# fnothaft/adam

Hardware: AMD Instinct MI355X
Metric: BQSR bases/sec (observe+apply) at 1/2/4/8 MI355X; % HBM roofline (higher is better)
Workload: dtype u8 in, int64 counts, f64 recalibration; 1 GPU; cfg2: synthetic 10M x 100 bp reads, 1 read group, no known sites (per GPU); reads_per_gpu=10000000, bases_per_gpu=1000000000, reads_total=10000000, read_groups=1, known_sites=0, parallelism=dp1: read shards per GPU, RCCL int64 table all-reduce

## Files before the change

adam_amd/csrc/bqsr_capi.cpp:

```cpp
#include <hip/hip_runtime.h>

#include <algorithm>
#include <array>
#include <atomic>
#include <chrono>
#include <cmath>
#include <cstdio>
#include <cstdlib>
#include <cstring>
#include <dlfcn.h>
#include <memory>
#include <mutex>
#include <new>
#include <string>
#include <thread>
#include <vector>

#include <rocprim/rocprim.hpp>

#include "bqsr_internal.h"

using namespace bqsr;

#include "bqsr_kernels.hip"
// ... 129 lines not shown
  return K + 2 * K * cells;
}
TableGeom geom(const bqsr_dims& d) {
  TableGeom g;
  g.K = 60 * (d.n_rg - 1) + 128;
  g.L = d.max_len;
  g.C = 2 * d.max_len + 1;
  g.cells = g.C + kCtxSlots;
  return g;
}

constexpr size_t kLdsMax = 163840;
size_t observe_lds(int qw, int wcells, bool table) {
  return (table ? (size_t)kCtxTabBytes : 0) + (size_t)qw * wcells * 8 + (size_t)qw * 4 + kQBins * 4 +
         (size_t)kMkWords * 4;
}
int64_t piece_bytes(int qw, int cw) { return ((int64_t)qw * cw * kCtxSlots + 15) & ~(int64_t)15; }
size_t apply_lds(int qw, int cw) { return 16 + (size_t)kMkWords * 4 + kCtxTabBytes + (size_t)piece_bytes(qw, cw); }
int lean_orow(int nc, int cw) {
  int o = nc * (cw + kCtxCells);
  while ((o & 3) != 2) ++o;
  return o;
}
size_t lean_lds(int qw, int orow, int wcells) { return ((size_t)qw * (orow + wcells) + qw + kQBins + 1) * 4; }
constexpr int kLeanCopiesMax = 4;
int observe_rows(int wcells, bool table) {
  int qw = kQBins;
  while (qw > 1 && observe_lds(qw, wcells, table) > kLdsMax) --qw;
  return qw;
}
constexpr bool align_slots() { return true; }
int fronts(int n_base, int n_cu, int64_t n_reads, int forced) {
  if (forced == 0) return 0;
  int f = forced;
  if (f < 0) {
    if (n_base > 4 * n_cu) return 0;
    f = (int)std::min<int64_t>((8 * n_cu + n_base - 1) / n_base, n_reads / (8192 * (int64_t)n_base));
    if ((int64_t)std::max(f, 1) * n_base < n_cu) return 0;
    f = std::max(f, 1);
  }
  while (f > 1 && (int64_t)f * n_base > 4096) --f;
  return f;
}
int apply_rows(int cw) {
  int qw = kQBins;
  while (qw > 1 && apply_lds(qw, cw) > kLdsMax) --qw;
  return qw;
}

}


struct bqsr_context {
  int device = 0;
  int n_cu = 256;
  double* d_pow10 = nullptr;
  double* d_thr = nullptr;
  double* d_qbt = nullptr;
  int16_t* d_qbq = nullptr;
  std::mutex stage_mu;
  uint8_t* stage[2] = {nullptr, nullptr};
  hipEvent_t stage_ev[2] = {nullptr, nullptr};
  int tune_order = -1;
  int tune_fronts = -1;
  int tune_keymajor = 0;
  int tune_bgzf = 1;
  int tune_flagstat_grid = 0;
  int tune_pileup_grid = 0;
  std::mutex flagstat_mu;
  unsigned long long* d_flagstat = nullptr;
};

namespace {
constexpr size_t kStageChunk = 64ull << 20;
bqsr_status stage_ring(bqsr_context* ctx) {
  for (int i = 0; i < 2; ++i) {
    if (!ctx->stage[i]) HIP_TRY(hipHostMalloc((void**)&ctx->stage[i], kStageChunk, hipHostMallocDefault));
    if (!ctx->stage_ev[i]) HIP_TRY(hipEventCreateWithFlags(&ctx->stage_ev[i], hipEventDisableTiming));
  }
  return BQSR_OK;
}
bqsr_status upload_staged(bqsr_context* ctx, void* dst, const void* src, size_t n, hipStream_t s) {
  hipPointerAttribute_t attr{};
  const bool pinned = hipPointerGetAttributes(&attr, src) == hipSuccess && attr.type == hipMemoryTypeHost;
  (void)hipGetLastError();
  if (pinned || n < 2 * kStageChunk) {
    HIP_TRY(hipMemcpyAsync(dst, src, n, hipMemcpyHostToDevice, s));
    HIP_TRY(hipStreamSynchronize(s));
    return BQSR_OK;
  }
  std::lock_guard<std::mutex> lock(ctx->stage_mu);
  bqsr_status st = stage_ring(ctx);
  if (st != BQSR_OK) return st;
  const int nth = (int)std::max(1u, std::min(8u, std::thread::hardware_concurrency()));
  const uint8_t* p = (const uint8_t*)src;
  uint8_t* d = (uint8_t*)dst;
  int k = 0;
  for (size_t off = 0; off < n; off += kStageChunk, k ^= 1) {
    const size_t len = std::min(kStageChunk, n - off);
    HIP_TRY(hipEventSynchronize(ctx->stage_ev[k]));
    std::vector<std::thread> th;
    for (int t = 0; t < nth; ++t)
      th.emplace_back([&, t] {
        const size_t a = len * (size_t)t / (size_t)nth, b = len * (size_t)(t + 1) / (size_t)nth;
        memcpy(ctx->stage[k] + a, p + off + a, b - a);
      });
    for (auto& x : th) x.join();
    HIP_TRY(hipMemcpyAsync(d + off, ctx->stage[k], len, hipMemcpyHostToDevice, s));
    HIP_TRY(hipEventRecord(ctx->stage_ev[k], s));
  }
  HIP_TRY(hipStreamSynchronize(s));
  return BQSR_OK;
}
}

struct bqsr_sites {
  bqsr_context* ctx = nullptr;
  std::vector<std::string> names;
  int64_t* pos = nullptr;
  uint64_t* off = nullptr;
  uint32_t* bucket = nullptr;
  uint64_t* bucket_off = nullptr;
  int64_t* bucket_base = nullptr;
  uint64_t* bm = nullptr;
  uint64_t* bm_off = nullptr;
  int64_t* bm_base = nullptr;
  int32_t n = 0;
  int32_t shift = 8;
  SitesDev dev() const { return SitesDev{pos, off, bucket, bucket_off, bucket_base, bm, bm_off, bm_base, n, shift}; }
};

struct bqsr_batch {
  bqsr_context* ctx = nullptr;
  bool owned = false;
  ReadsDev rd{};
  bqsr_dims dims{1, 1};
  int64_t n_slots = 0;
  int64_t n_bases = 0;
  int32_t q_lo = 0, rg_lo = 0;
  bool have_qhist = false;
  int64_t qhist[kQBins] = {0};
  int64_t qhigh = 0;
  std::vector<void*> allocs;
  std::vector<size_t> staged_cnt;
  const bqsr_staged* staged_src = nullptr;
  uint8_t* d_bases2 = nullptr;
  uint64_t* d_bexc = nullptr;
  uint64_t* d_qcodes = nullptr;
  uint8_t* d_qbase = nullptr;
  uint64_t* d_qexc = nullptr;
  ReadInfo* d_info = nullptr;
  uint64_t* d_sbits = nullptr;
  uint32_t* d_work = nullptr;
  uint64_t* d_bnd = nullptr;
  int64_t sbits_words = 0;
  bool err_fresh = false;
  bool prepped = false;
  const bqsr_sites* prep_sites = nullptr;
  uint32_t* d_hq = nullptr;
  uint32_t* d_qmask = nullptr;
  bool hq_valid = false;
  FoldParams fold{};
  uint32_t* d_part = nullptr;
  size_t part_words = 0;
  uint8_t* d_chars = nullptr;
  const bqsr_lut* chars_lut = nullptr;
  uint64_t* d_off64 = nullptr;
  int64_t off64_n = -1;
  size_t chars_bytes = 0;
  unsigned long long* d_err = nullptr;
  double* d_em = nullptr;
  int32_t n_blocks = 0;
  bool bucketed = false;
  int32_t n_keys = 1;
  int32_t n_base = 1;
  int32_t fronts = 0;
  uint32_t* d_perm = nullptr;
  int64_t* d_key_off = nullptr;
  uint32_t* d_key_cnt = nullptr;
  uint32_t* d_cursor = nullptr;
  uint8_t *k_qual = nullptr, *k_bases = nullptr;
  uint64_t* d_kslot = nullptr;
  uint64_t* d_kspan = nullptr;
  void* d_ktemp = nullptr;
  size_t ktemp_bytes = 0;
  bool km_ready = false;
  double km_alloc_ms = -1.0, km_build_ms = -1.0;
  bool perm_static = false;
  OrderDev order() const {
    return bucketed ? OrderDev{d_perm, d_key_off, n_keys, fronts > 0 ? n_base : 0, km_ready ? d_kslot : nullptr}
                    : OrderDev{nullptr, nullptr, 1};
  }
  ReadsDev pass_rd() const {
    ReadsDev r = rd;
    if (bucketed && km_ready) {
      r.qual = k_qual;
      r.bases = k_bases;
    }
    return r;
  }
  int32_t pass_blocks() const { return bucketed && fronts > 0 ? n_keys : n_blocks; }
  uint64_t* h_status = nullptr;
  hipStream_t side = nullptr;
  hipEvent_t ev_obs = nullptr, ev_fold = nullptr;
  bool obs_pending = false;
  ~bqsr_batch() {
    if (side) (void)hipStreamDestroy(side);
    for (hipEvent_t e : {ev_obs, ev_fold})
      if (e) (void)hipEventDestroy(e);
    if (d_part) (void)hipFree(d_part);
    if (d_off64) (void)hipFree(d_off64);
    if (d_chars) (void)hipFree(d_chars);
    if (h_status) (void)hipHostFree(h_status);
    for (void* p : allocs) (void)hipFree(p);
  }
};

struct bqsr_table {
  bqsr_context* ctx = nullptr;
  bqsr_dims dims{1, 1};
  int64_t* words = nullptr;
  bool owned = false;
  ~bqsr_table() {
    if (owned && words) (void)hipFree(words);
  }
  TableGeom g() const { return geom(dims); }
  int64_t* touched() const { return words; }
  int64_t* obs() const { return words + g().K; }
  int64_t* mm() const { return words + g().K + (int64_t)g().K * g().cells; }
};

struct bqsr_lut {
  bqsr_context* ctx = nullptr;
  bqsr_dims dims{1, 1};
  int32_t n_groups = 0;
  std::vector<void*> allocs;
  int64_t *qk_obs = nullptr, *qk_mm = nullptr, *grp_obs = nullptr, *grp_mm = nullptr;
  uint8_t *grp_ok = nullptr, *key_ok = nullptr, *rq_ok = nullptr;
  double *a2 = nullptr, *s1 = nullptr, *d2 = nullptr;
  FinalOut* d_out = nullptr;
  FinalOut out{};
  bool out_pending = false;
  bool host_ready = false;
  std::vector<int64_t> h_words, h_qk_obs, h_qk_mm, h_grp_obs, h_grp_mm;
  std::vector<uint8_t> h_grp_ok;
  const bqsr_table* src = nullptr;
  ~bqsr_lut() {
    for (void* p : allocs) (void)hipFree(p);
  }
};

namespace {
template <class T>
bqsr_status dalloc(std::vector<void*>& v, T** p, size_t n) {
  void* q = nullptr;
  HIP_TRY(hipMalloc(&q, std::max<size_t>(n, 1) * sizeof(T)));
  v.push_back(q);
  *p = (T*)q;
  return BQSR_OK;
}
}


extern "C" {

int bqsr_abi_version(void) { return BQSR_ABI_VERSION; }
const char* bqsr_last_error(void) { return g_err.c_str(); }
int64_t bqsr_last_error_read(void) { return g_err_read; }
const char* bqsr_status_name(bqsr_status s) {
  if ((int)s < 0 || (int)s > 16) return "UNKNOWN";
  return kStatusNames[(int)s];
}

bqsr_status bqsr_context_tune(bqsr_context* ctx, int knob, int64_t value) {
  if (!ctx) return fail(BQSR_ERR_INVALID_ARG, "bqsr_context_tune: null context");
  switch (knob) {
    case BQSR_TUNE_ORDER:
      if (value < -1 || value > 1) break;
      ctx->tune_order = (int)value;
      return BQSR_OK;
    case BQSR_TUNE_FRONTS:
      if (value < -1 || value > 4096) break;
      ctx->tune_fronts = (int)value;
      return BQSR_OK;
    case BQSR_TUNE_KEYMAJOR:
      if (value < 0 || value > 1) break;
      ctx->tune_keymajor = (int)value;
      return BQSR_OK;
    case BQSR_TUNE_FUSED_PREP:
      if (value != 0) break;
      return BQSR_OK;
    case BQSR_TUNE_BGZF:
      if (value < 0 || value > 1) break;
      ctx->tune_bgzf = (int)value;
      return BQSR_OK;
    case BQSR_TUNE_FLAGSTAT_GRID:
      if (value < 0 || value > (1 << 20)) break;
      ctx->tune_flagstat_grid = (int)value;
      return BQSR_OK;
    case BQSR_TUNE_PILEUP_GRID:
      if (value < 0 || value > (1 << 20)) break;
      ctx->tune_pileup_grid = (int)value;
      return BQSR_OK;
    default:
      return fail(BQSR_ERR_INVALID_ARG, "bqsr_context_tune: unknown knob");
  }
  return fail(BQSR_ERR_INVALID_ARG, "bqsr_context_tune: value out of range");
}

bqsr_status bqsr_context_create(int device, bqsr_context** out) {
  if (!out) return fail(BQSR_ERR_INVALID_ARG, "null out");
  HIP_TRY(hipSetDevice(device));
  hipDeviceProp_t prop;
  HIP_TRY(hipGetDeviceProperties(&prop, device));
  bqsr_context* c = new bqsr_context;
  c->device = device;
  c->n_cu = prop.multiProcessorCount;
  hipError_t e = hipMalloc(&c->d_pow10, 256 * sizeof(double));
  if (e == hipSuccess) e = hipMalloc(&c->d_thr, kThrN * sizeof(double));
  if (e == hipSuccess) e = hipMemcpy(c->d_pow10, pow10tab().v, 256 * sizeof(double), hipMemcpyHostToDevice);
  if (e == hipSuccess) e = hipMemcpy(c->d_thr, thresholds().thr.data(), kThrN * sizeof(double), hipMemcpyHostToDevice);
  if (e == hipSuccess) e = hipMalloc(&c->d_qbt, kQbN * sizeof(double));
  if (e == hipSuccess) e = hipMalloc(&c->d_qbq, kQbN * sizeof(int16_t));
  if (e == hipSuccess) e = hipMemcpy(c->d_qbt, buckets().thr.data(), kQbN * sizeof(double), hipMemcpyHostToDevice);
  if (e == hipSuccess) e = hipMemcpy(c->d_qbq, buckets().q.data(), kQbN * sizeof(int16_t), hipMemcpyHostToDevice);
  for (const void* f : {(const void*)bqsr_apply_kernel, (const void*)bqsr_observe_chunks,
                        (const void*)bqsr_observe_lean<true>})
    if (e == hipSuccess) e = hipFuncSetAttribute(f, hipFuncAttributeMaxDynamicSharedMemorySize, (int)kLdsMax);
  if (e == hipSuccess)
    e = hipFuncSetAttribute((const void*)bqsr_fold_hist, hipFuncAttributeMaxDynamicSharedMemorySize, (int)fold_hist_lds());
  if (e == hipSuccess)
    e = hipFuncSetAttribute((const void*)bqsr_fold_chain, hipFuncAttributeMaxDynamicSharedMemorySize,
                            (int)chain_lds(kMaxFoldBlocks));
  if (e != hipSuccess) {
    bqsr_context_destroy(c);
    return fail(BQSR_ERR_DEVICE, std::string("context: ") + hipGetErrorString(e));
  }
  *out = c;
  return ok();
}

void bqsr_context_destroy(bqsr_context* c) {
  if (!c) return;
  if (c->d_pow10) (void)hipFree(c->d_pow10);
  if (c->d_thr) (void)hipFree(c->d_thr);
  if (c->d_qbt) (void)hipFree(c->d_qbt);
  if (c->d_qbq) (void)hipFree(c->d_qbq);
  if (c->d_flagstat) (void)hipFree(c->d_flagstat);
  for (int i = 0; i < 2; ++i) {
    if (c->stage[i]) (void)hipHostFree(c->stage[i]);
    if (c->stage_ev[i]) (void)hipEventDestroy(c->stage_ev[i]);
  }
  delete c;
}


bqsr_status bqsr_sites_create(bqsr_context* ctx, const char* const* contigs, const int64_t* const* pos,
                              const uint64_t* n, int32_t n_contigs, bqsr_sites** out) {
  if (!ctx || !out || n_contigs < 0 || (n_contigs > 0 && (!contigs || !pos || !n)))
    return fail(BQSR_ERR_INVALID_ARG, "bqsr_sites_create: bad arguments");
  HIP_TRY(hipSetDevice(ctx->device));
  bqsr_sites* s = new bqsr_sites;
  s->ctx = ctx;
  s->n = n_contigs;
  std::vector<int64_t> all;
  std::vector<uint64_t> off(1, 0);
  std::vector<uint32_t> bucket;
  std::vector<uint64_t> boff(1, 0);
  std::vector<int64_t> bbase;
  std::vector<uint64_t> bm, bmoff(1, 0);
  std::vector<int64_t> bmbase;
  for (int32_t c = 0; c < n_contigs; ++c) {
    s->names.emplace_back(contigs[c] ? contigs[c] : "");
    std::vector<int64_t> v(pos[c], pos[c] + n[c]);
    std::sort(v.begin(), v.end());
    v.erase(std::unique(v.begin(), v.end()), v.end());
    const int64_t base = v.empty() ? 0 : v.front();
    const int64_t nb = v.empty() ? 0 : ((v.back() - base) >> s->shift) + 1;
    size_t j = 0;
    for (int64_t b = 0; b < nb; ++b) {
      const int64_t lo = base + (b << s->shift);
      while (j < v.size() && v[j] < lo) ++j;
      bucket.push_back((uint32_t)j);
    }
    bbase.push_back(base);
    boff.push_back(bucket.size());
    const int64_t b0 = v.empty() ? 0 : (int64_t)((uint64_t)base & ~(uint64_t)63);
    const int64_t nw = v.empty() ? 0 : ((v.back() - b0) >> 6) + 1;
    const bool dense = nw > 0 && nw <= 64 * (int64_t)v.size() + 64 && nw <= (int64_t(1) << 28);
    if (dense) {
      const size_t w0 = bm.size();
      bm.resize(w0 + (size_t)nw, 0ull);
      for (const int64_t p : v) bm[w0 + (size_t)((p - b0) >> 6)] |= 1ull << ((p - b0) & 63);
    }
    bmbase.push_back(dense ? b0 : 0);
    bmoff.push_back(bm.size());
    all.insert(all.end(), v.begin(), v.end());
    off.push_back(all.size());
  }
  std::vector<void*> keep;
  auto up = [&](auto** dst, const auto& src) -> hipError_t {
    using T = typename std::remove_reference<decltype(src[0])>::type;
    hipError_t e = hipMalloc((void**)dst, std::max<size_t>(src.size(), 1) * sizeof(T));
    if (e != hipSuccess) return e;
    if (!src.empty()) e = hipMemcpy(*dst, src.data(), src.size() * sizeof(T), hipMemcpyHostToDevice);
    return e;
  };
  hipError_t e = up(&s->pos, all);
  if (e == hipSuccess) e = up(&s->off, off);
  if (e == hipSuccess) e = up(&s->bucket, bucket);
  if (e == hipSuccess) e = up(&s->bucket_off, boff);
  if (e == hipSuccess) e = up(&s->bucket_base, bbase);
  if (e == hipSuccess) e = up(&s->bm, bm);
  if (e == hipSuccess) e = up(&s->bm_off, bmoff);
  if (e == hipSuccess) e = up(&s->bm_base, bmbase);
  if (e != hipSuccess) {
    bqsr_sites_destroy(s);
    return fail(BQSR_ERR_DEVICE, std::string("sites upload: ") + hipGetErrorString(e));
  }
  *out = s;
  return ok();
}

void bqsr_sites_destroy(bqsr_sites* s) {
  if (!s) return;
  for (void* p : {(void*)s->pos, (void*)s->off, (void*)s->bucket, (void*)s->bucket_off, (void*)s->bucket_base,
                  (void*)s->bm, (void*)s->bm_off, (void*)s->bm_base})
    if (p) (void)hipFree(p);
  delete s;
}


namespace {

inline uint8_t code_of(uint8_t c) {
  switch (c) {
    case 'A': return kCodeA;
    case 'C': return kCodeC;
    case 'G': return kCodeG;
    case 'T': return kCodeT;
    case 'N': return kCodeN;
    default: return kCodeOther;
  }
}

Window window_rows(const bqsr_batch* b, int max_rows);

bqsr_status finish_batch(bqsr_batch* b, int64_t max_slot_len) {
  if (max_slot_len > kMaxReadLen)
    return fail(BQSR_ERR_UNSUPPORTED, "reads longer than " + std::to_string(kMaxReadLen) + " bases are not supported");
  const int64_t n = b->rd.n_reads;
  b->rd.reads_per_tile = (int32_t)std::max<int64_t>(1, std::min<int64_t>(kMaxTileReads, kTileSlots / std::max<int64_t>(1, max_slot_len)));
  b->rd.n_tiles = (n + b->rd.reads_per_tile - 1) / b->rd.reads_per_tile;
  b->n_blocks = std::min(b->ctx->n_cu, kMaxFoldBlocks);
  bqsr_status st;
  if ((st = dalloc(b->allocs, &b->d_hq, (size_t)b->n_blocks * kQBins)) != BQSR_OK) return st;
  if ((st = dalloc(b->allocs, &b->d_qmask, 4)) != BQSR_OK) return st;
  {
    FoldParams& F = b->fold;
    const size_t nt = (size_t)std::max<int64_t>(1, b->rd.n_tiles), nbk = (size_t)b->n_blocks;
    F.stream_cap = std::max<int64_t>(1 << 20, std::min<int64_t>(16 << 20, b->rd.n_slots));
    if ((st = dalloc(b->allocs, &F.blk, nbk)) != BQSR_OK || (st = dalloc(b->allocs, &F.cand_list, nbk)) != BQSR_OK ||
        (st = dalloc(b->allocs, &F.n_cand, 1)) != BQSR_OK || (st = dalloc(b->allocs, &F.delta, 1)) != BQSR_OK ||
        (st = dalloc(b->allocs, &F.rtile, nt)) != BQSR_OK || (st = dalloc(b->allocs, &F.ntile, nt)) != BQSR_OK ||
        (st = dalloc(b->allocs, &F.dtile, nt * kSegBinades)) != BQSR_OK ||
        (st = dalloc(b->allocs, &F.seg, nbk * kFoldMaxSegs)) != BQSR_OK ||
        (st = dalloc(b->allocs, &F.seg_base, nbk)) != BQSR_OK || (st = dalloc(b->allocs, &F.nseg, nbk)) != BQSR_OK ||
        (st = dalloc(b->allocs, &F.seg_used, 1)) != BQSR_OK ||
        (st = dalloc(b->allocs, &F.streams, (size_t)F.stream_cap + 64)) != BQSR_OK ||
        (st = dalloc(b->allocs, &F.csum, (size_t)F.stream_cap / 64 * 2 + 2)) != BQSR_OK ||
        (st = dalloc(b->allocs, &F.stream_used, 1)) != BQSR_OK)
      return st;
  }
  if ((st = dalloc(b->allocs, &b->d_err, kErrWords)) != BQSR_OK) return st;
  if ((st = dalloc(b->allocs, &b->d_info, (size_t)std::max<int64_t>(1, n))) != BQSR_OK) return st;
  b->sbits_words = (b->rd.n_slots / 32 + 5) & ~(int64_t)1;
  if ((st = dalloc(b->allocs, &b->d_sbits, (size_t)b->sbits_words)) != BQSR_OK) return st;
  if ((st = dalloc(b->allocs, &b->d_em, 2)) != BQSR_OK) return st;
  if ((st = dalloc(b->allocs, &b->d_bnd, (size_t)2 * (size_t)(n / 64 + kPrepChunk / 64 + 1))) != BQSR_OK) return st;
  if ((st = dalloc(b->allocs, &b->d_work,
                   (size_t)(n + kPrepChunk) + (size_t)std::max<int64_t>(n / kPrepChunk + 1, kMaxFoldBlocks))) != BQSR_OK)
    return st;
  if (b->ctx->tune_order >= 0) {
    b->bucketed = b->ctx->tune_order == 1;
  } else {
    b->bucketed = b->dims.n_rg > 1;
    if (!b->bucketed && b->have_qhist) {
      const int cw = geom(b->dims).C;
      const Window w = window_rows(b, apply_rows(cw));
      int64_t in = 0, all = 0;
      for (int q = 0; q < kQBins; ++q) {
        all += b->qhist[q];
        if (q >= w.q_lo && q < w.q_lo + w.qw) in += b->qhist[q];
      }
      b->bucketed = (double)(all - in) > 1e-3 * (double)all;
    }
  }
  if (b->bucketed) {
    b->n_base = 2 * std::max<int32_t>(1, b->dims.n_rg);
    b->fronts = fronts(b->n_base, b->ctx->n_cu, n, b->ctx->tune_fronts);
    b->n_keys = b->n_base * std::max(1, b->fronts);
    if ((st = dalloc(b->allocs, &b->d_perm, (size_t)std::max<int64_t>(1, n))) != BQSR_OK) return st;
    if ((st = dalloc(b->allocs, &b->d_key_off, (size_t)b->n_keys + 1)) != BQSR_OK) return st;
    if ((st = dalloc(b->allocs, &b->d_key_cnt, (size_t)b->n_keys)) != BQSR_OK) return st;
    if ((st = dalloc(b->allocs, &b->d_cursor, (size_t)b->n_keys)) != BQSR_OK) return st;
  }
  return BQSR_OK;
}

bool layout_wanted(const bqsr_batch* b) { return b->bucketed && b->rd.slots_aligned && b->rd.n_reads > 0; }
bool key_major_wanted(const bqsr_batch* b) { return layout_wanted(b) && b->ctx->tune_keymajor; }
bqsr_status key_major_alloc(bqsr_batch* b) {
  if (b->k_qual) return BQSR_OK;
  const int64_t n = b->rd.n_reads;
  bqsr_status st;
  size_t tb = 0;
  HIP_TRY(rocprim::exclusive_scan(nullptr, tb, (const uint64_t*)nullptr, (uint64_t*)nullptr, (uint64_t)0, (size_t)n + 1,
                                  rocprim::plus<uint64_t>(), (hipStream_t)0));
  b->ktemp_bytes = std::max<size_t>(tb, 1);
  if ((st = dalloc(b->allocs, &b->d_kslot, (size_t)(n + 1))) != BQSR_OK ||
      (st = dalloc(b->allocs, &b->d_kspan, (size_t)(n + 1))) != BQSR_OK ||
      (st = dalloc(b->allocs, (uint8_t**)&b->d_ktemp, b->ktemp_bytes)) != BQSR_OK ||
      (st = dalloc(b->allocs, &b->k_qual, (size_t)b->rd.n_slots + kColumnPad)) != BQSR_OK ||
      (st = dalloc(b->allocs, &b->k_bases, (size_t)b->rd.n_slots / 2 + 1 + kColumnPad)) != BQSR_OK)
    return st;
  return BQSR_OK;
}
void launch_key_sort(bqsr_batch* b, uint64_t* span, hipStream_t s) {
  const int64_t n = b->rd.n_reads;
  const int n_cu = b->ctx->n_cu;
  (void)hipMemsetAsync(b->d_key_cnt, 0, (size_t)b->n_keys * 4, s);
  const unsigned cb = (unsigned)std::min<int64_t>((n + 255) / 256, (int64_t)n_cu * 4);
  hipLaunchKernelGGL(bqsr_key_count, dim3(cb), dim3(256), 0, s, (const ReadMeta*)b->rd.meta, n, b->n_keys, b->n_base,
                     std::max(1, b->fronts), b->d_key_cnt);
  hipLaunchKernelGGL(bqsr_key_scan, dim3(1), dim3(1024), 0, s, (const uint32_t*)b->d_key_cnt, b->n_keys, b->d_key_off,
                     b->d_cursor);
  const unsigned sb = (unsigned)std::min<int64_t>((n + 4095) / 4096, (int64_t)n_cu * 8);
  hipLaunchKernelGGL(bqsr_key_scatter, dim3(sb), dim3(256), 0, s, (const ReadMeta*)b->rd.meta, n, b->n_keys, b->n_base,
                     std::max(1, b->fronts), b->d_cursor, b->d_perm, span);
}
bqsr_status layout_build(bqsr_batch* b, hipStream_t s) {
  if (!layout_wanted(b)) return BQSR_OK;
  const int64_t n = b->rd.n_reads;
  bqsr_context* ctx = b->ctx;
  const bool km = key_major_wanted(b);
  b->km_ready = false;
  const auto t0 = std::chrono::steady_clock::now();
  bqsr_status st = km ? key_major_alloc(b) : BQSR_OK;
  if (st != BQSR_OK) return st;
  const auto t1 = std::chrono::steady_clock::now();
  if (km) HIP_TRY(hipMemsetAsync(b->d_kspan + n, 0, 8, s));
  launch_key_sort(b, km ? b->d_kspan : nullptr, s);
  HIP_TRY(hipGetLastError());
  if (km) {
    size_t tb = b->ktemp_bytes;
    HIP_TRY(rocprim::exclusive_scan(b->d_ktemp, tb, b->d_kspan, b->d_kslot, (uint64_t)0, (size_t)n + 1,
                                    rocprim::plus<uint64_t>(), s));
    HIP_TRY(hipMemsetAsync(b->k_qual + b->rd.n_slots, 0, kColumnPad, s));
    HIP_TRY(hipMemsetAsync(b->k_bases + b->rd.n_slots / 2, 0, 1 + kColumnPad, s));
    const unsigned gw = (unsigned)std::min<int64_t>((n + 16 * kKmPer - 1) / (16 * kKmPer), (int64_t)ctx->n_cu * 64 / kKmPer);
    hipLaunchKernelGGL(bqsr_km_gather, dim3(gw), dim3(256), 0, s, b->rd, (const uint32_t*)b->d_perm,
                       (const uint64_t*)b->d_kslot, b->k_qual, b->k_bases);
    HIP_TRY(hipGetLastError());
  }
  HIP_TRY(hipStreamSynchronize(s));
  const auto t2 = std::chrono::steady_clock::now();
  b->km_alloc_ms = std::chrono::duration<double, std::milli>(t1 - t0).count();
  b->km_build_ms = std::chrono::duration<double, std::milli>(t2 - t1).count();
  b->km_ready = km;
  b->perm_static = true;
  return BQSR_OK;
}

struct Packed {
  std::vector<ReadMeta> meta;
  std::vector<ReadAlign> align;
  std::vector<uint8_t> qual, bases, md;
  std::vector<uint32_t> cigar;
  int64_t n_slots = 0, n_bases = 0, max_slot = 0;
  int32_t n_rg = 1, max_len = 1;
  int64_t qhist[256] = {0};
  std::vector<int64_t> rghist;
};

bqsr_status pack(const bqsr_records* R, Packed& P) {
  const int64_t n = R->n_reads;
  P.meta.resize((size_t)n);
  P.align.resize((size_t)n);
  uint64_t slot = 0, md_tot = 0, cig_tot = 0;
  for (int64_t r = 0; r < n; ++r) {
    const uint32_t f = R->flags[r];
    const uint64_t lq = (f & BQSR_F_HAS_QUAL) ? R->qual_offset[r + 1] - R->qual_offset[r] : 0;
    const uint64_t ls = (f & BQSR_F_HAS_SEQ) ? R->seq_offset[r + 1] - R->seq_offset[r] : 0;
    const uint64_t nmd = (f & BQSR_F_HAS_MD) ? R->md_offset[r + 1] - R->md_offset[r] : 0;
    const uint64_t ncig = (f & BQSR_F_HAS_CIGAR) ? R->cigar_offset[r + 1] - R->cigar_offset[r] : 0;
    if (lq > 65535 || ls > 65535 || nmd > 65535 || ncig > 65535)
      return fail(BQSR_ERR_UNSUPPORTED, "read field longer than 65535", r);
    if ((f & BQSR_F_HAS_RG) && (R->rg_id[r] < 0 || R->rg_id[r] > 65535))
      return fail(BQSR_ERR_UNSUPPORTED, "recordGroupId outside [0, 65535]", r);
    ReadMeta& m = P.meta[(size_t)r];
    m.slot = slot;
    m.lq = (uint16_t)lq;
    m.ls = (uint16_t)ls;
    m.flags = (uint16_t)(f & 0x7FFF);
    m.rg = (f & BQSR_F_HAS_RG) ? (uint16_t)R->rg_id[r] : 0;
    ReadAlign& a = P.align[(size_t)r];
    a.start = R->start[r];
    a.cigar_off = (uint32_t)cig_tot;
    a.md_off = (uint32_t)md_tot;
    a.contig = R->contig_id[r];
    a.n_cigar = (uint16_t)ncig;
    a.md_len = (uint16_t)nmd;
    const uint64_t sl = align_slots() ? slot_span(lq, ls) : std::max(lq, ls);
    slot += sl;
    P.max_slot = std::max<int64_t>(P.max_slot, (int64_t)sl);
    md_tot += nmd;
    cig_tot += ncig;
    P.n_bases += (int64_t)(R->seq_offset[r + 1] - R->seq_offset[r]);
    if (f & BQSR_F_HAS_RG) P.n_rg = std::max<int32_t>(P.n_rg, R->rg_id[r] + 1);
    P.max_len = std::max<int32_t>(P.max_len, (int32_t)ls);
  }
  if (md_tot > 0xFFFFFFFFull || cig_tot > 0xFFFFFFFFull)
    return fail(BQSR_ERR_UNSUPPORTED, "partition MD / CIGAR columns exceed 4 GiB");
  P.n_slots = (int64_t)slot;
  P.qual.assign((size_t)slot + kColumnPad, 0);
  P.bases.assign((size_t)slot / 2 + 1 + kColumnPad, 0);
  P.md.resize(md_tot + kColumnPad);
  P.cigar.resize(cig_tot + kColumnPad / 4);
  P.rghist.assign((size_t)P.n_rg, 0);
  const int nth = (int)std::max<int64_t>(1, std::min<int64_t>(16, n / 65536));
  std::vector<std::thread> th;
  std::vector<std::array<int64_t, 256>> qh((size_t)nth);
// ... 350 lines not shown
  }
  *out = b;
  return ok();
}

void bqsr_batch_destroy(bqsr_batch* b) { delete b; }
int64_t bqsr_batch_reads(const bqsr_batch* b) { return b ? b->rd.n_reads : -1; }
int64_t bqsr_batch_bases(const bqsr_batch* b) { return b ? b->n_bases : -1; }
int64_t bqsr_batch_slots(const bqsr_batch* b) { return b ? b->n_slots : -1; }
bqsr_dims bqsr_batch_dims(const bqsr_batch* b) { return b ? b->dims : bqsr_dims{0, 0}; }

bqsr_status bqsr_batch_relayout(bqsr_batch* b, void* stream, double* ms) {
  if (!b) return fail(BQSR_ERR_INVALID_ARG, "bqsr_batch_relayout: null batch");
  hipStream_t s = (hipStream_t)stream;
  HIP_TRY(hipStreamSynchronize(s));
  const auto t0 = std::chrono::steady_clock::now();
  const bool has = b->perm_static;
  if (has) {
    b->perm_static = false;
    bqsr_status st = layout_build(b, s);
    if (st != BQSR_OK) return st;
  }
  HIP_TRY(hipStreamSynchronize(s));
  if (ms) *ms = has ? std::chrono::duration<double, std::milli>(std::chrono::steady_clock::now() - t0).count() : -1.0;
  return ok();
}

bqsr_status bqsr_batch_layout_times(const bqsr_batch* b, double* alloc_ms, double* build_ms) {
  if (!b) return fail(BQSR_ERR_INVALID_ARG, "bqsr_batch_layout_times: null batch");
  if (alloc_ms) *alloc_ms = b->km_alloc_ms;
  if (build_ms) *build_ms = b->km_build_ms;
  return ok();
}

bqsr_status bqsr_batch_set_window(bqsr_batch* b, int32_t q_lo, int32_t rg_lo) {
  if (!b || q_lo < 0 || q_lo >= kQBins || rg_lo < 0) return fail(BQSR_ERR_INVALID_ARG, "bad window");
  b->q_lo = q_lo;
  b->rg_lo = rg_lo;
  b->have_qhist = false;
  return ok();
}
int32_t bqsr_batch_reads_per_tile(const bqsr_batch* b) { return b ? b->rd.reads_per_tile : -1; }


int64_t bqsr_table_words(bqsr_dims d) { return (d.n_rg < 1 || d.max_len < 1) ? -1 : table_words(d); }

bqsr_status bqsr_table_create(bqsr_context* ctx, bqsr_dims d, void* device_words, bqsr_table** out) {
  if (!ctx || !out || d.n_rg < 1 || d.max_len < 1 || d.max_len > 65535)
    return fail(BQSR_ERR_INVALID_ARG, "bqsr_table_create: bad arguments");
  HIP_TRY(hipSetDevice(ctx->device));
  bqsr_table* t = new bqsr_table;
  t->ctx = ctx;
  t->dims = d;
  const size_t bytes = (size_t)table_words(d) * 8;
  if (device_words) {
    t->words = (int64_t*)device_words;
  } else {
    hipError_t e = hipMalloc((void**)&t->words, bytes);
    if (e != hipSuccess) {
      delete t;
      return fail(BQSR_ERR_DEVICE, hipGetErrorString(e));
    }
    t->owned = true;
  }
  hipError_t e = hipMemset(t->words, 0, bytes);
  if (e != hipSuccess) {
    delete t;
    return fail(BQSR_ERR_DEVICE, hipGetErrorString(e));
  }
  *out = t;
  return ok();
}
void bqsr_table_destroy(bqsr_table* t) { delete t; }
bqsr_dims bqsr_table_dims(const bqsr_table* t) { return t ? t->dims : bqsr_dims{0, 0}; }
void* bqsr_table_device_ptr(bqsr_table* t) { return t ? t->words : nullptr; }

bqsr_status bqsr_table_download(const bqsr_table* t, int64_t* host) {
  if (!t || !host) return fail(BQSR_ERR_INVALID_ARG, "null");
  HIP_TRY(hipSetDevice(t->ctx->device));
  HIP_TRY(hipMemcpy(host, t->words, (size_t)table_words(t->dims) * 8, hipMemcpyDeviceToHost));
  return ok();
}
bqsr_status bqsr_table_upload(bqsr_table* t, const int64_t* host) {
  if (!t || !host) return fail(BQSR_ERR_INVALID_ARG, "null");
  HIP_TRY(hipSetDevice(t->ctx->device));
  HIP_TRY(hipMemcpy(t->words, host, (size_t)table_words(t->dims) * 8, hipMemcpyHostToDevice));
  return ok();
}

bqsr_status bqsr_table_merge(bqsr_table* acc, const bqsr_table* part, double* acc_em, double part_em) {
  if (!acc || !part || !acc_em) return fail(BQSR_ERR_INVALID_ARG, "null");
  if (acc->dims.n_rg != part->dims.n_rg || acc->dims.max_len != part->dims.max_len)
    return fail(BQSR_ERR_INVALID_ARG, "table dims differ");
  HIP_TRY(hipSetDevice(acc->ctx->device));
  const int64_t n = table_words(acc->dims);
  hipLaunchKernelGGL(bqsr_table_add, dim3((unsigned)std::min<int64_t>(4096, (n + 255) / 256)), dim3(256), 0,
                     hipStreamPerThread, acc->words, part->words, n);
  HIP_TRY(hipGetLastError());
  HIP_TRY(hipStreamSynchronize(hipStreamPerThread));
  *acc_em = *acc_em + part_em;
  return ok();
}


namespace {
Window window_rows(const bqsr_batch* b, int max_rows) {
  Window w{max_rows, std::min(b->q_lo, kQBins - 1), b->rg_lo};
  if (!b->have_qhist) {
    w.qw = std::min(w.qw, kQBins - w.q_lo);
    return w;
  }
  int lo = 0, hi = kQBins - 1;
  while (lo < kQBins - 1 && b->qhist[lo] == 0) ++lo;
  while (hi > lo && b->qhist[hi] == 0) --hi;
  if (hi - lo + 1 <= max_rows) {
    w.q_lo = lo;
    w.qw = hi - lo + 1;
  } else {
    w.q_lo = best_q_lo(b->qhist, max_rows);
  }
  w.qw = std::min(w.qw, kQBins - w.q_lo);
  return w;
}
int window_cw(const bqsr_batch* b, const TableGeom& g) { return b->bucketed ? g.L : g.C; }
int qual_span(const bqsr_batch* b) {
  if (!b->have_qhist) return kQBins;
  int lo = 0, hi = kQBins - 1;
  while (lo < kQBins - 1 && b->qhist[lo] == 0) ++lo;
  while (hi > lo && b->qhist[hi] == 0) --hi;
  return hi - lo + 1;
}
int lane_shift(const bqsr_batch* b) {
  const int c = (b->dims.max_len + kSuper - 1) / kSuper;
  int s = 0;
  while ((1 << s) < c && s < 6) ++s;
  return s;
}
bqsr_status check_dims(const bqsr_batch* b, const bqsr_table* t) {
  if (b->dims.n_rg > t->dims.n_rg || b->dims.max_len > t->dims.max_len)
    return fail(BQSR_ERR_INVALID_ARG, "table dims smaller than the batch's (n_rg / max_len)");
  return BQSR_OK;
}
}

namespace {
bqsr_status launch_prep(bqsr_context* ctx, bqsr_batch* b, const bqsr_sites* sites, hipStream_t s) {
  if (!b->err_fresh) HIP_TRY(hipMemsetAsync(b->d_err + kErrAppPrep, 0xFF, 8, s));
  b->err_fresh = false;
  b->hq_valid = false;
  if (b->rd.n_reads > 0) {
    PrepParams P{};
    P.rd = b->rd;
    if (sites) P.sites = sites->dev();
    P.store_words = b->dims.max_len <= 128 && P.sites.n_contigs > 0;
    P.bnd = b->d_bnd;
    P.info = b->d_info;
    P.sbits = b->d_sbits;
    P.err = b->d_err;
    P.work = b->d_work;
    P.n_work = b->d_work + b->rd.n_reads + kPrepChunk;
    const int64_t blocks = (b->rd.n_reads + kPrepChunk - 1) / kPrepChunk;
    if (P.store_words) {
      hipLaunchKernelGGL(bqsr_prep_kernel<true>, dim3((unsigned)blocks), dim3(kPrepThreads), 0, s, P);
      hipLaunchKernelGGL(bqsr_prep_complex, dim3((unsigned)blocks), dim3(kComplexThreads), 0, s, P);
    } else {
      hipLaunchKernelGGL(bqsr_prep_kernel<false>, dim3((unsigned)blocks), dim3(kPrepThreads), 0, s, P);
    }
    HIP_TRY(hipGetLastError());
    if (b->bucketed && !b->perm_static) {
      launch_key_sort(b, nullptr, s);
      HIP_TRY(hipGetLastError());
    }
  }
  b->prepped = true;
  b->prep_sites = sites;
  return BQSR_OK;
}
}

bqsr_status bqsr_observe_stage(bqsr_context* ctx, bqsr_batch* b, const bqsr_sites* sites, bqsr_table* t,
                               int32_t stages, void* stream) {
  if (!ctx || !b || !t) return fail(BQSR_ERR_INVALID_ARG, "null");
  bqsr_status st = check_dims(b, t);
  if (st != BQSR_OK) return st;
  HIP_TRY(hipSetDevice(ctx->device));
  hipStream_t s = S(stream);
  if (stages & BQSR_STAGE_RESET) HIP_TRY(hipMemsetAsync(b->d_err + kErrObs, 0xFF, 8, s));
  if (stages & BQSR_STAGE_PREP) {
    if ((st = launch_prep(ctx, b, sites, s)) != BQSR_OK) return st;
  }
  if (b->rd.n_reads == 0) {
    if (stages & BQSR_STAGE_FOLD) HIP_TRY(hipMemsetAsync(b->d_em, 0, 8, s));
    return ok();
  }
  if ((stages & BQSR_STAGE_KERNEL) && (!b->prepped || b->prep_sites != sites))
    return fail(BQSR_ERR_INVALID_ARG, "observe kernel before the prep stage (or with other known sites)");
  if (stages & BQSR_STAGE_KERNEL) {
    ObserveParams P{};
    P.rd = b->pass_rd();
    P.ord = b->order();
    P.info = b->d_info;
    P.sbits = b->d_sbits;
    P.g = geom(t->dims);
    const bool lean = !b->bucketed;
    P.wcells = window_cw(b, P.g) + (lean ? kCtxCells : kCtxSlots);
    while ((P.wcells & 3) != 2) ++P.wcells;
    if (lean) {
      const int cw = window_cw(b, P.g), span = qual_span(b);
      int best_rows = 0;
      for (int nc = kLeanCopiesMax; nc >= 1 && best_rows < span; --nc) {
        const int orow = lean_orow(nc, cw);
        int qw = kQBins;
        while (qw > 1 && lean_lds(qw, orow, P.wcells) > kLdsMax) --qw;
        if (qw > best_rows) {
          best_rows = qw;
          P.nc = nc;
          P.orow = orow;
        }
      }
      P.w = window_rows(b, best_rows);
      P.rows_all = b->have_qhist && b->qhigh == 0;
      for (int q = 0; q < kQBins && P.rows_all; ++q)
        if (b->qhist[q] && (q < P.w.q_lo || q >= P.w.q_lo + P.w.qw)) P.rows_all = 0;
    } else {
      P.w = window_rows(b, observe_rows(P.wcells, true));
    }
    P.touched = t->touched();
    P.obs = t->obs();
    P.mm = t->mm();
    P.part_stride = 2 * P.w.qw * P.wcells + P.w.qw;
    if (!lean) {
      if (!b->side) {
        HIP_TRY(hipStreamCreateWithFlags(&b->side, hipStreamNonBlocking));
        HIP_TRY(hipEventCreateWithFlags(&b->ev_obs, hipEventDisableTiming));
        HIP_TRY(hipEventCreateWithFlags(&b->ev_fold, hipEventDisableTiming));
      }
      HIP_TRY(hipEventRecord(b->ev_obs, s));
      b->obs_pending = true;
    }
    const size_t need = (size_t)P.part_stride * (b->pass_blocks() + b->n_keys - 1);
    if (b->part_words < need) {
      if (b->d_part) {
        HIP_TRY(hipStreamSynchronize(s));
        (void)hipFree(b->d_part);
        b->d_part = nullptr;
        b->part_words = 0;
      }
      HIP_TRY(hipMalloc((void**)&b->d_part, need * sizeof(uint32_t)));
      b->part_words = need;
    }
    P.part = b->d_part;
    P.hq_block = b->d_hq;
    P.err = b->d_err + kErrObs;
    P.n_blocks = lean ? b->n_blocks : b->pass_blocks();
    const size_t lds = lean ? lean_lds(P.w.qw, P.orow, P.wcells) : observe_lds(P.w.qw, P.wcells, true);
    if (lean) {
      hipLaunchKernelGGL((bqsr_observe_lean<true>), dim3(P.n_blocks), dim3(kBlockThreads), lds, s, P);
    } else {
      hipLaunchKernelGGL(bqsr_observe_chunks, dim3(P.n_blocks), dim3(kBlockThreads), lds, s, P);
    }
    HIP_TRY(hipGetLastError());
    const int rb = (int)std::min<int64_t>(4096, ((int64_t)P.part_stride * (b->bucketed ? b->n_base : 1) + 255) / 256);
    const unsigned ry = b->bucketed ? 1u : (unsigned)((b->n_blocks + kRedSlabs - 1) / kRedSlabs);
    hipLaunchKernelGGL(bqsr_window_reduce, dim3(rb, ry), dim3(256), 0, s, (const uint32_t*)b->d_part, b->rd, P.ord,
                       P.n_blocks, P.part_stride, P.wcells, P.w, P.g, P.touched, P.obs, P.mm, lean ? kCtxJunk : 0);
    HIP_TRY(hipGetLastError());
  }
  if (stages & BQSR_STAGE_FOLD) {
    const hipStream_t caller = s;
    const bool fork = b->obs_pending;
    if (fork) {
      HIP_TRY(hipStreamWaitEvent(b->side, b->ev_obs, 0));
      s = b->side;
      b->obs_pending = false;
    }
    if (b->bucketed) {
      HIP_TRY(hipMemsetAsync(b->d_hq, 0, (size_t)b->n_blocks * kQBins * 4, s));
      hipLaunchKernelGGL(bqsr_fold_hist, dim3(b->n_blocks * kFhSplit), dim3(kFhWaves * 64), fold_hist_lds(), s, b->rd, (const ReadInfo*)b->d_info,
                         b->n_blocks, lane_shift(b), b->d_hq);
      HIP_TRY(hipGetLastError());
    }
    FoldParams F = b->fold;
    F.rd = b->rd;
    F.info = b->d_info;
    F.hq_block = b->d_hq;
    F.pow10 = ctx->d_pow10;
    F.n_blocks = b->n_blocks;
    F.em_out = b->d_em;
    F.qmask = b->d_qmask;
    hipLaunchKernelGGL(bqsr_fold_plan, dim3(1), dim3(1024), 0, s, F);
    const int64_t max_tpb = (b->rd.n_tiles + b->n_blocks - 1) / b->n_blocks + 1;
    hipLaunchKernelGGL(bqsr_fold_tiles, dim3(ctx->n_cu * 4), dim3(kFtWaves * 64), 0, s, F, max_tpb);
    hipLaunchKernelGGL(bqsr_fold_segs, dim3(b->n_blocks), dim3(kSegThreads), 0, s, F);
    hipLaunchKernelGGL(bqsr_fold_chain, dim3(1), dim3(1024), chain_lds(b->n_blocks), s, F);
    HIP_TRY(hipGetLastError());
    b->hq_valid = true;
    if (fork) {
      HIP_TRY(hipEventRecord(b->ev_fold, s));
      HIP_TRY(hipStreamWaitEvent(caller, b->ev_fold, 0));
    }
  }
  return ok();
}

bqsr_status bqsr_observe_async(bqsr_context* ctx, bqsr_batch* b, const bqsr_sites* sites, bqsr_table* t, void* stream) {
  return bqsr_observe_stage(ctx, b, sites, t, BQSR_STAGE_RESET | BQSR_STAGE_PREP | BQSR_STAGE_KERNEL | BQSR_STAGE_FOLD,
                            stream);
}

bqsr_status bqsr_table_zero_async(bqsr_table* t, void* stream) {
  if (!t) return fail(BQSR_ERR_INVALID_ARG, "null");
  HIP_TRY(hipSetDevice(t->ctx->device));
  HIP_TRY(hipMemsetAsync(t->words, 0, (size_t)table_words(t->dims) * 8, S(stream)));
  return ok();
}

void* bqsr_batch_em_device_ptr(bqsr_batch* b) { return b ? (void*)b->d_em : nullptr; }

bqsr_status bqsr_observe_result(bqsr_batch* b, double* em, void* stream) {
  HIP_TRY(hipSetDevice(b->ctx->device));
  hipStream_t s = S(stream);
  unsigned long long err = 0;
  double e = 0;
  HIP_TRY(hipMemcpyAsync(&err, b->d_err + kErrObs, 8, hipMemcpyDeviceToHost, s));
  HIP_TRY(hipMemcpyAsync(&e, b->d_em, 8, hipMemcpyDeviceToHost, s));
  HIP_TRY(hipStreamSynchronize(s));
  if (em) *em = e;
  return from_err_key(err, 0);
}

bqsr_status bqsr_observe(bqsr_context* ctx, bqsr_batch* b, const bqsr_sites* sites, bqsr_table* t,
                         double* expected_mismatch, void* stream) {
  bqsr_status st = bqsr_observe_async(ctx, b, sites, t, stream);
  if (st != BQSR_OK) return st;
  return bqsr_observe_result(b, expected_mismatch, stream);
}

bqsr_status bqsr_observe_records(bqsr_context* ctx, const bqsr_records* recs, const bqsr_sites* sites, bqsr_dims dims,
                                 bqsr_table** out_partial, double* out_em) {
  if (!out_partial || !out_em) return fail(BQSR_ERR_INVALID_ARG, "null out");
  bqsr_batch* b = nullptr;
  bqsr_status st = bqsr_batch_create(ctx, recs, nullptr, &b);
  if (st != BQSR_OK) return st;
  bqsr_table* t = nullptr;
  st = bqsr_table_create(ctx, dims, nullptr, &t);
  if (st == BQSR_OK) st = bqsr_observe(ctx, b, sites, t, out_em, nullptr);
  bqsr_batch_destroy(b);
  if (st != BQSR_OK) {
    bqsr_table_destroy(t);
    return st;
  }
  *out_partial = t;
  return ok();
}


namespace {
bqsr_status finalize_impl(bqsr_context* ctx, const bqsr_table* t, double em, const double* em_dev, bqsr_lut** out,
                          void* stream) {
  if (!ctx || !t || !out) return fail(BQSR_ERR_INVALID_ARG, "null");
  HIP_TRY(hipSetDevice(ctx->device));
  hipStream_t s = S(stream);
  const TableGeom g = geom(t->dims);
  const int n_rg = t->dims.n_rg;
  bqsr_lut* L = *out;
  const bool reuse = L && L->ctx == ctx && L->dims.n_rg == t->dims.n_rg && L->dims.max_len == t->dims.max_len;
  if (L && !reuse) {
    (void)hipStreamSynchronize(s);
    delete L;
    *out = nullptr;
  }
  if (!reuse) L = new bqsr_lut;
  L->ctx = ctx;
  L->dims = t->dims;
  L->src = t;
  L->host_ready = false;
  L->n_groups = (g.K - 1) / kMaxQ + 2;
  bqsr_status st;
  if (!reuse && ((st = dalloc(L->allocs, &L->qk_obs, g.K)) != BQSR_OK || (st = dalloc(L->allocs, &L->qk_mm, g.K)) != BQSR_OK ||
      (st = dalloc(L->allocs, &L->grp_obs, L->n_groups)) != BQSR_OK ||
      (st = dalloc(L->allocs, &L->grp_mm, L->n_groups)) != BQSR_OK ||
      (st = dalloc(L->allocs, &L->grp_ok, L->n_groups)) != BQSR_OK || (st = dalloc(L->allocs, &L->key_ok, g.K)) != BQSR_OK ||
      (st = dalloc(L->allocs, &L->rq_ok, (size_t)n_rg * kQBins)) != BQSR_OK ||
      (st = dalloc(L->allocs, &L->a2, (size_t)n_rg * kQBins)) != BQSR_OK ||
      (st = dalloc(L->allocs, &L->s1, (size_t)n_rg * kQBins * g.C)) != BQSR_OK ||
      (st = dalloc(L->allocs, &L->d2, (size_t)n_rg * kQBins * kCtxSlots)) != BQSR_OK ||
      (st = dalloc(L->allocs, &L->d_out, 1)) != BQSR_OK)) {
    delete L;
    return st;
  }
  hipLaunchKernelGGL(bqsr_final_keys, dim3((g.K + 3) / 4), dim3(256), 0, s, t->touched(), t->obs(), t->mm(), g, L->qk_obs,
                     L->qk_mm);
  hipLaunchKernelGGL(bqsr_final_groups, dim3(1), dim3(256), 0, s, t->touched(), L->qk_obs, L->qk_mm, g, n_rg, em,
                     em_dev, ctx->d_pow10, L->n_groups, L->grp_obs, L->grp_mm, L->grp_ok, L->key_ok, L->a2, L->rq_ok, L->d_out);
  const int64_t ncell = (int64_t)n_rg * kQBins * (g.C + kCtxSlots);
  hipLaunchKernelGGL(bqsr_final_tables, dim3((unsigned)std::min<int64_t>(8192, (ncell + 255) / 256)), dim3(256), 0, s,
                     t->obs(), t->mm(), g, n_rg, L->a2, L->rq_ok, pow10tab().v[kMaxQ], L->s1, L->d2);
  hipError_t e = hipGetLastError();
  L->out_pending = em_dev != nullptr;
  if (e == hipSuccess && !em_dev) e = hipMemcpyAsync(&L->out, L->d_out, sizeof(FinalOut), hipMemcpyDeviceToHost, s);
  if (e != hipSuccess) {
    if (!reuse) delete L;
    return fail(BQSR_ERR_DEVICE, hipGetErrorString(e));
  }
  *out = L;
  return ok();
}
}

bqsr_status bqsr_finalize_async(bqsr_context* ctx, const bqsr_table* t, double em, bqsr_lut** out, void* stream) {
// ... 492 lines not shown
```

adam_amd/csrc/bqsr_internal.h:

```cpp
#pragma once
#include <hip/hip_runtime.h>
#include <stdint.h>

#include "../../include/adam_bqsr.h"

namespace bqsr {

struct ReadMeta {
  uint64_t slot;
  uint16_t lq;
  uint16_t ls;
  uint16_t flags;
  uint16_t rg;
};
static_assert(sizeof(ReadMeta) == 16, "ReadMeta must be 16 B");

struct ReadAlign {
  int64_t start;
  uint32_t cigar_off;
  uint32_t md_off;
  int32_t contig;
  uint16_t n_cigar;
  uint16_t md_len;
};
static_assert(sizeof(ReadAlign) == 24, "ReadAlign must be 24 B");

struct alignas(8) ReadInfo {
  uint16_t st;
  uint16_t en;
  uint16_t fl;
  uint16_t pad;
};
static_assert(sizeof(ReadInfo) == 8 && alignof(ReadInfo) == 8, "ReadInfo must be one aligned 8-B word");
__device__ __forceinline__ ReadInfo info_load(const ReadInfo* p) {
  const uint64_t v = __hip_atomic_load((const uint64_t*)p, __ATOMIC_RELAXED, __HIP_MEMORY_SCOPE_WORKGROUP);
  return ReadInfo{(uint16_t)v, (uint16_t)(v >> 16), (uint16_t)(v >> 32), (uint16_t)(v >> 48)};
}
__device__ __forceinline__ void info_store(ReadInfo* p, ReadInfo x) {
  const uint64_t v = (uint64_t)x.st | ((uint64_t)x.en << 16) | ((uint64_t)x.fl << 32) | ((uint64_t)x.pad << 48);
  __hip_atomic_store((uint64_t*)p, v, __ATOMIC_RELAXED, __HIP_MEMORY_SCOPE_WORKGROUP);
}
constexpr uint16_t kInfoObs = 1;
constexpr uint16_t kInfoObsCheck = 2;
constexpr uint16_t kInfoApp = 4;
constexpr uint16_t kInfoAppCheck = 8;
constexpr uint16_t kInfoNeg = 16;
constexpr uint16_t kInfoSecond = 32;
constexpr uint16_t kInfoPass = 64;
constexpr uint16_t kInfoCycNeg = 128;
constexpr uint16_t kInfoTrim = 256;
constexpr uint16_t kInfoNoBits = 512;

constexpr uint16_t kSeqOther = 1u << 15;

constexpr uint8_t kCodeA = 0, kCodeC = 1, kCodeG = 2, kCodeT = 3, kCodeN = 4, kCodeOther = 5;

constexpr int kMaxQ = 60;
constexpr int kCtxSlots = 21;
constexpr uint32_t kCtxTab = 4096;
constexpr int kCtxTabBytes = 2 * kCtxTab * 2;
constexpr int kQBins = 128;

constexpr int kTileSlots = 4096;
constexpr int kMaxTileReads = 64;
constexpr int kMaxFoldBlocks = 1024;
constexpr int kWaves = 16;
constexpr int kBlockThreads = 64 * kWaves;
constexpr int kMkWords = kWaves * 64;
constexpr int kMaxReadLen = 4096;
constexpr int kColumnPad = 32;
constexpr int kRedSlabs = 16;

constexpr uint64_t kNoError = ~0ull;
__host__ __device__ inline uint64_t err_key(uint64_t read, uint32_t o, uint32_t rank, uint32_t code) {
  return (read << 28) | ((uint64_t)(o & 0xFFFFF) << 8) | ((uint64_t)(rank & 0xF) << 4) | (code & 0xF);
}
enum : uint32_t {
  kRankCtor = 0,
  kRankCigar = 1,
  kRankMd = 2,
  kRankSnp = 3,
  kRankCov = 4,
  kRankTable = 5
};
enum { kErrObs = 0, kErrAppPrep = 1, kErrAppKern = 2, kNExc = 3, kErrWords = 4 };
constexpr int kJobStatusWords = 16;
constexpr int kStatusSlots = 4;

struct SitesDev {
  const int64_t* pos;
  const uint64_t* off;
  const uint32_t* bucket;
  const uint64_t* bucket_off;
  const int64_t* bucket_base;
  const uint64_t* bm;
  const uint64_t* bm_off;
  const int64_t* bm_base;
  int32_t n_contigs;
  int32_t shift;
};

struct TableGeom {
  int32_t K;
  int32_t C;
  int32_t L;
  int32_t cells;
};

struct Window {
  int32_t qw;
  int32_t q_lo;
  int32_t rg_lo;
};

struct ReadsDev {
  const ReadMeta* meta;
  const ReadAlign* align;
  const uint8_t* qual;
  const uint8_t* bases;
  const uint32_t* cigar;
  const uint8_t* md;
  int64_t n_reads;
  int64_t n_slots;
  int32_t reads_per_tile;
  int64_t n_tiles;
  int32_t slots_aligned;
};
__host__ __device__ inline uint64_t slot_span(uint64_t lq, uint64_t ls) {
  const uint64_t sl = lq > ls ? lq : ls;
  return (sl + 15) & ~(uint64_t)15;
}

struct PrepParams {
  ReadsDev rd;
  SitesDev sites;
  ReadInfo* info;
  uint64_t* sbits;
  int32_t store_words;
  uint64_t* bnd;
  unsigned long long* err;
  uint32_t* work;
  uint32_t* n_work;
};

struct OrderDev {
  const uint32_t* perm;
  const int64_t* key_off;
  int32_t n_keys;
  int32_t n_base = 0;
  const uint64_t* kslot = nullptr;
};

struct ObserveParams {
  ReadsDev rd;
  OrderDev ord;
  ReadInfo* info;
  const uint64_t* sbits;
  TableGeom g;
  Window w;
  int64_t* touched;
  int64_t* obs;
  int64_t* mm;
  uint32_t* part;
  int32_t part_stride;
  uint32_t* hq_block;
  unsigned long long* err;
  int32_t n_blocks;
  int32_t wcells;
  int32_t lane_shift;
  int32_t orow;
  int32_t nc;
  int32_t rows_all;
};

constexpr int32_t kFoldNoBase = INT32_MIN;
constexpr int kSegBinades = 32;
constexpr double kFoldTie = -1.0, kFoldUnknown = -2.0;
constexpr int kFoldMaxSegs = 64;
enum : int32_t { kSegRun = 0, kSegEvent = 1, kSegGlobal = 2 };

struct FoldBlock {
  double r0, r1;
  double inc;
  int32_t e;
  int32_t cidx;
};
static_assert(sizeof(FoldBlock) == 32, "FoldBlock is 4 words");

struct FoldSeg {
  int64_t inc;
  int32_t t0, t1;
  int32_t e;
  int32_t kind;
  int64_t off;
};
static_assert(sizeof(FoldSeg) == 32, "FoldSeg is 4 words");

struct FoldParams {
  ReadsDev rd;
  const ReadInfo* info;
  const uint32_t* hq_block;
  const double* pow10;
  int32_t n_blocks;
  FoldBlock* blk;
  int32_t* cand_list;
  int32_t* n_cand;
  double* delta;
  double* rtile;
  int32_t* ntile;
  double* dtile;
  FoldSeg* seg;
  int32_t* seg_base;
  int32_t* nseg;
  uint32_t* seg_used;
  uint8_t* streams;
  double* csum;
  int64_t stream_cap;
  unsigned long long* stream_used;
  double* em_out;
  uint32_t* qmask;
};

constexpr int kQbElo = -48;
constexpr int kQbEhi = 3;
constexpr int kQbBits = 5;
constexpr int kQbN = (kQbEhi - kQbElo + 1) << kQbBits;

struct ApplyParams {
  ReadsDev rd;
  OrderDev ord;
  const ReadInfo* info;
  TableGeom g;
  Window w;
  int32_t n_rg;
  const double* s1;
  const double* d2;
  const uint8_t* rq_ok;
  const uint8_t* key_ok;
  const uint8_t* grp_ok;
  int32_t n_groups;
  const double* thr;
  int32_t thr_qmin;
  int32_t thr_n;
  const double* qb_thr;
  const int16_t* qb_q;
  uint8_t* out_qual;
  uint32_t* out_start;
  uint32_t* out_len;
  unsigned long long* exc;
  int64_t max_exc;
  unsigned long long* n_exc;
  unsigned long long* err;
  int32_t lane_shift;
  int32_t outs_apart;
  const uint8_t* chars;
  int64_t piece_stride;
  uint32_t* rowbad;
  const uint32_t* qmask;
};

struct FinalOut {
  int64_t g_obs, g_mm;
  double avg, global_error;
  int32_t any_key;
  int32_t pad;
};
static_assert(kErrWords + 1 + sizeof(FinalOut) / 8 <= (size_t)kJobStatusWords, "job status words overflow");
static_assert(sizeof(FinalOut) % 8 == 0, "FinalOut is whole words");

constexpr int kThrQmin = -3100;
constexpr int kThrQmax = 3300;
constexpr int kThrN = kThrQmax - kThrQmin + 1;

}
```

adam_amd/csrc/bqsr_kernels.hip:

```cpp
#include <hip/hip_runtime.h>

#include "bqsr_internal.h"

namespace bqsr {


__device__ __forceinline__ void wave_sync() {
  __builtin_amdgcn_fence(__ATOMIC_SEQ_CST, "workgroup");
  __builtin_amdgcn_wave_barrier();
}

__device__ __forceinline__ bool usable_read(uint16_t f) {
  return (f & BQSR_F_MAPPED) && (f & BQSR_F_PRIMARY) && !(f & BQSR_F_DUPLICATE) && (f & BQSR_F_HAS_MD);
}
__device__ __forceinline__ bool eligible_read(uint16_t f) {
  return (f & BQSR_F_MAPPED) && (f & BQSR_F_PRIMARY) && !(f & BQSR_F_DUPLICATE);
}

__device__ __forceinline__ void report(unsigned long long* err, uint64_t key) { atomicMin(err, (unsigned long long)key); }

__device__ __forceinline__ uint32_t cig_op(uint32_t e) { return e & 0xFu; }
__device__ __forceinline__ uint32_t cig_len(uint32_t e) { return e >> 4; }
__device__ __forceinline__ bool is_seg_op(uint32_t op) {
  return op == BQSR_CIGAR_M || op == BQSR_CIGAR_X || op == BQSR_CIGAR_EQ || op == BQSR_CIGAR_S;
}
__device__ __forceinline__ bool consumes_ref(uint32_t op) {
  return op == BQSR_CIGAR_M || op == BQSR_CIGAR_D || op == BQSR_CIGAR_N || op == BQSR_CIGAR_EQ || op == BQSR_CIGAR_X;
}

__device__ __forceinline__ bool md_base(uint8_t c) {
  if (c >= 'a' && c <= 'z') c = (uint8_t)(c - 32);
  switch (c) {
    case 'A': case 'G': case 'C': case 'T': case 'N': case 'U': case 'K': case 'M': case 'R':
    case 'S': case 'W': case 'B': case 'V': case 'H': case 'D': case 'X': case 'Y':
      return true;
    default:
      return false;
  }
}

template <class MdPtr, class F>
__device__ bool md_scan(MdPtr md, int n, int64_t* total, F&& nonmatch) {
  int off = 0;
  int64_t pos = 0;
  *total = 0;
  if (n == 0) return true;
  auto digits = [&]() -> bool {
    int b = off;
    int64_t v = 0;
    while (off < n && md[off] >= '0' && md[off] <= '9') {
      v = v * 10 + (md[off] - '0');
      if (v > 2147483647LL) return false;
      ++off;
    }
    if (off == b) return false;
    pos += v;
    return true;
  };
  if (!digits()) return false;
  while (off < n) {
    if (md[off] == '^') ++off;
    int b = off;
    while (off < n && md_base(md[off])) {
      nonmatch(pos + (off - b));
      ++off;
    }
    if (off == b) return false;
    pos += off - b;
    if (!digits()) return false;
  }
  *total = pos;
  return true;
}

template <class CigPtr>
__device__ int refpos_to_offset(CigPtr cig, int ncig, int64_t unclipped, int64_t p) {
  int ro = 0;
  int64_t pos = unclipped;
  for (int i = 0; i < ncig; ++i) {
    uint32_t e = cig[i], op = cig_op(e), len = cig_len(e);
    if (is_seg_op(op)) {
      if (p < pos) return -1;
      if (p < pos + (int64_t)len) return ro + (int)(p - pos);
      ro += len;
      pos += len;
    } else if (op == BQSR_CIGAR_I) {
      ro += len;
    } else if (op != BQSR_CIGAR_H) {
      pos += len;
    }
  }
  return -1;
}

__device__ void set_sbits(uint64_t* sb, uint64_t lo, uint64_t hi, int half) {
  while (lo < hi) {
    const uint64_t i = lo >> 5;
    const int b = (int)(lo & 31);
    const int n = (int)min((uint64_t)(32 - b), hi - lo);
    const uint32_t m = (n == 32) ? 0xFFFFFFFFu : (((1u << n) - 1u) << b);
    atomicOr((unsigned long long*)&sb[i], (unsigned long long)m << half);
    lo += (uint64_t)n;
  }
}

__device__ __forceinline__ int first_good(const uint4 v, int n, bool rev) {
  const uint32_t w[4] = {v.x, v.y, v.z, v.w};
  uint32_t g[4];
#pragma unroll
  for (int i = 0; i < 4; ++i) g[i] = ((w[i] & 0x7F7F7F7Fu) + 0x7D7D7D7Du) & ~w[i] & 0x80808080u;
  uint64_t lo = ((uint64_t)g[1] << 32) | g[0], hi = ((uint64_t)g[3] << 32) | g[2];
  if (n < 16) {
    const int keep = n <= 0 ? 0 : n;
    if (!rev) {
      lo &= keep >= 8 ? ~0ull : ((1ull << (8 * keep)) - 1ull);
      hi &= keep <= 8 ? 0ull : ((1ull << (8 * (keep - 8))) - 1ull);
    } else {
      hi &= keep >= 8 ? ~0ull : ~((1ull << (8 * (8 - keep))) - 1ull);
      lo &= keep <= 8 ? 0ull : ~((1ull << (8 * (16 - keep))) - 1ull);
    }
  }
  if (!rev) return lo ? (__builtin_ctzll(lo) >> 3) : hi ? 8 + (__builtin_ctzll(hi) >> 3) : 16;
  return hi ? (__builtin_clzll(hi) >> 3) : lo ? 8 + (__builtin_clzll(lo) >> 3) : 16;
}

__device__ __forceinline__ void trim_quals(const uint8_t* q, int lq, int& st, int& en) {
  int s = 0, tail = 0;
  bool more_st = true, more_tail = true;
  if (lq >= 16) {
    const uint4 head = *(const uint4*)q, back = *(const uint4*)(q + lq - 16);
    s = first_good(head, 16, false);
    tail = first_good(back, 16, true);
    more_st = s == 16;
    more_tail = tail == 16;
  }
  if (more_st)
    while (s < lq && (int8_t)q[s] <= 2) ++s;
  if (more_tail)
    while (tail < lq && (int8_t)q[lq - 1 - tail] <= 2) ++tail;
  st = s;
  en = lq - tail;
}

__device__ __forceinline__ ReadInfo resolve_info(const ReadsDev& rd, ReadInfo inf, uint64_t slot, int lq) {
  if (inf.fl & kInfoTrim) {
    int st, en;
    trim_quals(rd.qual + slot, lq, st, en);
    inf.st = (uint16_t)st;
    if (st >= en) {
      inf.en = 0;
      inf.fl = 0;
    } else {
      inf.en = (uint16_t)en;
      inf.fl &= (uint16_t)~kInfoTrim;
    }
  }
  return inf;
}

constexpr int kPrepThreads = 256;
constexpr int kComplexThreads = 128;
constexpr int kPrepCig = 4, kPrepCigStride = 5;
constexpr int kPrepMd = 32, kPrepMdStride = 9;
constexpr int kPrepChunk = 2048;

template <class CigPtr, class MdPtr>
__device__ void prep_one_rest(const PrepParams& P, int64_t r, const ReadMeta& m, const ReadAlign& a, ReadInfo inf,
                              int st, int en, bool usable, CigPtr cig, MdPtr md);

__device__ __forceinline__ void prep_one(const PrepParams& P, int64_t r, uint32_t* s_cig, uint32_t* s_md) {
  const ReadMeta m = P.rd.meta[r];
  const ReadAlign a = P.rd.align[r];
  ReadInfo inf{0, 0, 0, 0};
  const uint16_t f = m.flags;
  if (!eligible_read(f)) {
    inf.fl = kInfoPass;
    P.info[r] = inf;
    return;
  }
  const bool usable = usable_read(f);
  auto fail = [&](uint64_t key) {
    if (usable) report(&P.err[kErrObs], key);
    report(&P.err[kErrAppPrep], key);
  };
  if (!(f & BQSR_F_HAS_QUAL)) {
    fail(err_key(r, 0, kRankCtor, BQSR_ERR_NULL_FIELD));
    P.info[r] = inf;
    return;
  }
  int st, en;
  trim_quals(P.rd.qual + m.slot, m.lq, st, en);
  inf.st = (uint16_t)min(st, 0xFFFF);
  if (!(f & BQSR_F_HAS_RG)) {
    fail(err_key(r, 0, kRankCtor, BQSR_ERR_NULL_RG));
    P.info[r] = inf;
    return;
  }
  if (!(f & BQSR_F_HAS_SEQ)) {
    fail(err_key(r, 0, kRankCtor, BQSR_ERR_NULL_FIELD));
    P.info[r] = inf;
    return;
  }
  if ((f & BQSR_F_NEG_STRAND) && (f & kSeqOther)) {
    fail(err_key(r, 0, kRankCtor, BQSR_ERR_BAD_REVCOMP_BASE));
    P.info[r] = inf;
    return;
  }
  if (st >= en) {
    P.info[r] = inf;
    return;
  }
  const uint16_t check_fl = (usable ? kInfoObsCheck : 0) | kInfoAppCheck;
  if (!(f & BQSR_F_HAS_CIGAR) || !(f & BQSR_F_HAS_START)) {
    fail(err_key(r, st, kRankCigar, BQSR_ERR_NULL_FIELD));
    inf.en = (uint16_t)st;
    inf.fl = check_fl;
    P.info[r] = inf;
    return;
  }
  const uint32_t* gcig = P.rd.cigar + a.cigar_off;
  const uint8_t* gmd = P.rd.md + a.md_off;
  const bool sc = a.n_cigar <= kPrepCig, sm = !(f & BQSR_F_HAS_MD) || a.md_len <= kPrepMd;
  typedef __attribute__((address_space(3))) uint32_t* LdsW;
  typedef const __attribute__((address_space(3))) uint32_t* LdsCW;
  typedef const __attribute__((address_space(3))) uint8_t* LdsCB;
  if (sc && sm) {
    const uint4 c4 = *(const uint4*)gcig;
    uint4 m0 = make_uint4(0, 0, 0, 0), m1 = m0;
    if (f & BQSR_F_HAS_MD) {
      m0 = *(const uint4*)gmd;
      m1 = *(const uint4*)(gmd + 16);
    }
    LdsW lc = (LdsW)s_cig, lm = (LdsW)s_md;
    lc[0] = c4.x;
    lc[1] = c4.y;
    lc[2] = c4.z;
    lc[3] = c4.w;
    lm[0] = m0.x;
    lm[1] = m0.y;
    lm[2] = m0.z;
    lm[3] = m0.w;
    lm[4] = m1.x;
    lm[5] = m1.y;
    lm[6] = m1.z;
    lm[7] = m1.w;
    prep_one_rest(P, r, m, a, inf, st, en, usable, (LdsCW)lc, (LdsCB)lm);
  } else {
    prep_one_rest(P, r, m, a, inf, st, en, usable, gcig, gmd);
  }
}

template <class CigPtr, class MdPtr>
__device__ void prep_one_rest(const PrepParams& P, int64_t r, const ReadMeta& m, const ReadAlign& a, ReadInfo inf,
                              int st, int en, bool usable, CigPtr cig, MdPtr md) {
  const uint16_t f = m.flags;
  auto fail = [&](uint64_t key) {
    if (usable) report(&P.err[kErrObs], key);
    report(&P.err[kErrAppPrep], key);
  };
  const uint16_t check_fl = (usable ? kInfoObsCheck : 0) | kInfoAppCheck;
  const int ncig = a.n_cigar;
  int64_t lead = 0, rp_len = 0, ref_len = 0;
  bool leading = true, zero = false;
  for (int i = 0; i < ncig; ++i) {
    uint32_t e = cig[i], op = cig_op(e), len = cig_len(e);
    if (leading && (op == BQSR_CIGAR_S || op == BQSR_CIGAR_H)) lead += len; else leading = false;
    if (is_seg_op(op) || op == BQSR_CIGAR_I) rp_len += len;
    if (is_seg_op(op) && len == 0) zero = true;
    if (consumes_ref(op)) ref_len += len;
  }
  const int64_t start = a.start;
  const int64_t unclipped = start - lead;
  const int64_t ref_end = start + ref_len;
  uint64_t best = kNoError;
  if (zero) {
    best = err_key(r, st, kRankCigar, BQSR_ERR_CIGAR_INVALID);
  } else if (unclipped < -2147483648LL || unclipped + rp_len + ref_len > 2147483647LL) {
    best = err_key(r, st, kRankCigar, BQSR_ERR_UNSUPPORTED);
  } else {
    const int e1 = (int)min((int64_t)en, rp_len);
    int o_first = -1;
    {
      int ro = 0;
      for (int i = 0; i < ncig && o_first < 0; ++i) {
        uint32_t e = cig[i], op = cig_op(e), len = cig_len(e);
        if (is_seg_op(op)) {
          int lo = max(ro, st), hi = min(ro + (int)len, e1);
          if (lo < hi) o_first = lo;
          ro += len;
        } else if (op == BQSR_CIGAR_I) {
          ro += len;
        }
      }
    }
    if (o_first >= 0) {
      int64_t tot;
      if ((f & BQSR_F_HAS_MD) && !md_scan(md, a.md_len, &tot, [](int64_t) {}))
        best = min(best, err_key(r, o_first, kRankMd, BQSR_ERR_MD_PARSE));
      if (!(f & BQSR_F_HAS_REFNAME)) best = min(best, err_key(r, o_first, kRankSnp, BQSR_ERR_NULL_FIELD));
    }
    if ((int64_t)en > rp_len)
      best = min(best, err_key(r, (uint32_t)max((int64_t)st, rp_len), kRankCigar, BQSR_ERR_CIGAR_SHORT));
    if (en > (int)m.ls) best = min(best, err_key(r, (uint32_t)max(st, (int)m.ls), kRankCov, BQSR_ERR_SEQ_SHORT));
  }
  if (best != kNoError) {
    fail(best);
    inf.en = (uint16_t)((best >> 8) & 0xFFFFF);
    inf.fl = check_fl;
    P.info[r] = inf;
    return;
  }
  inf.en = (uint16_t)en;
  inf.fl = kInfoApp | (usable ? kInfoObs : 0) | ((f & BQSR_F_NEG_STRAND) ? kInfoNeg : 0) |
           (((f & BQSR_F_PAIRED) && (f & BQSR_F_SECOND_OF_PAIR)) ? kInfoSecond : 0);
  P.info[r] = inf;
  if (!usable) return;

  uint64_t* bw = P.sbits;
  const uint64_t rs = m.slot;
  {
    int ro = 0;
    int64_t pos = unclipped;
    for (int i = 0; i < ncig; ++i) {
      uint32_t e = cig[i], op = cig_op(e), len = cig_len(e);
      if (is_seg_op(op)) {
        int lo = max(ro, st), hi = min(ro + (int)len, en);
        if (lo < hi) {
          int64_t w0 = (int64_t)ro + (start - pos), w1 = (int64_t)ro + (ref_end - pos);
          int a0 = (int)min(max(w0, (int64_t)lo), (int64_t)hi);
          int a1 = (int)min(max(w1, (int64_t)lo), (int64_t)hi);
          set_sbits(bw, rs + (uint64_t)(lo), rs + (uint64_t)(a0), 0);
          set_sbits(bw, rs + (uint64_t)(max(a1, a0)), rs + (uint64_t)(hi), 0);
        }
        ro += len;
        pos += len;
      } else if (op == BQSR_CIGAR_I) {
        int lo = max(ro, st), hi = min(ro + (int)len, en);
        set_sbits(bw, rs + (uint64_t)(lo), rs + (uint64_t)(max(lo, hi)), 0);
        ro += len;
      } else if (op != BQSR_CIGAR_H) {
        pos += len;
      }
    }
  }
  int64_t md_total = 0;
  md_scan(md, a.md_len, &md_total, [&](int64_t prel) {
    int64_t p = start + prel;
    if (p >= ref_end) return;
    int o = refpos_to_offset(cig, ncig, unclipped, p);
    if (o >= st && o < en) set_sbits(bw, rs + (uint64_t)(o), rs + (uint64_t)(o + 1), 32);
  });
  if (start + md_total < ref_end) {
    int ro = 0;
    int64_t pos = unclipped;
    const int64_t t0 = start + md_total;
    for (int i = 0; i < ncig; ++i) {
      uint32_t e = cig[i], op = cig_op(e), len = cig_len(e);
      if (is_seg_op(op)) {
        int64_t p0 = max(pos, t0), p1 = min(pos + (int64_t)len, ref_end);
        if (p0 < p1) {
          int lo = max(ro + (int)(p0 - pos), st), hi = min(ro + (int)(p1 - pos), en);
          if (lo < hi) set_sbits(bw, rs + (uint64_t)(lo), rs + (uint64_t)(hi), 32);
        }
        ro += len;
        pos += len;
      } else if (op == BQSR_CIGAR_I) {
        ro += len;
      } else if (op != BQSR_CIGAR_H) {
        pos += len;
      }
    }
  }
  if (a.contig >= 0 && a.contig < P.sites.n_contigs) {
    const SitesDev& S = P.sites;
    const int64_t* sp = S.pos + S.off[a.contig];
    const int64_t ns = (int64_t)(S.off[a.contig + 1] - S.off[a.contig]);
    if (ns > 0) {
      const int64_t lo_p = unclipped, hi_p = unclipped + rp_len + ref_len;
      const uint32_t* bk = S.bucket + S.bucket_off[a.contig];
      const int64_t nb = (int64_t)(S.bucket_off[a.contig + 1] - S.bucket_off[a.contig]);
      const int64_t base = S.bucket_base[a.contig];
      int64_t j;
      const int64_t bi = (lo_p - base) >> S.shift;
      if (bi < 0) j = 0;
      else if (bi >= nb) j = ns;
      else j = bk[bi];
      while (j < ns && sp[j] < lo_p) ++j;
      for (; j < ns && sp[j] < hi_p; ++j) {
        int o = refpos_to_offset(cig, ncig, unclipped, sp[j]);
        if (o >= st && o < en) set_sbits(bw, rs + (uint64_t)(o), rs + (uint64_t)(o + 1), 0);
      }
    }
  }
}

__device__ void mask_sites_linear(const PrepParams& P, int32_t contig, int64_t unclipped, int st, int en,
                                  uint64_t rs) {
  if (contig < 0 || contig >= P.sites.n_contigs) return;
  const SitesDev& S = P.sites;
  const int64_t* sp = S.pos + S.off[contig];
  const int64_t ns = (int64_t)(S.off[contig + 1] - S.off[contig]);
  if (ns == 0) return;
  const int64_t lo_p = unclipped + st, hi_p = unclipped + en;
  const uint32_t* bk = S.bucket + S.bucket_off[contig];
  const int64_t nb = (int64_t)(S.bucket_off[contig + 1] - S.bucket_off[contig]);
  const int64_t bi = (lo_p - S.bucket_base[contig]) >> S.shift;
  int64_t j = bi < 0 ? 0 : (bi >= nb ? ns : (int64_t)bk[bi]);
  while (j < ns && sp[j] < lo_p) ++j;
  for (; j < ns && sp[j] < hi_p; ++j) {
    const uint64_t o = (uint64_t)(sp[j] - unclipped);
    set_sbits(P.sbits, rs + o, rs + o + 1, 0);
  }
}

__device__ __forceinline__ bool mask_sites_bitmap(const PrepParams& P, int32_t contig, int64_t unclipped, int lq,
                                                  uint64_t rs) {
  const SitesDev& S = P.sites;
  const int64_t nw = (int64_t)(S.bm_off[contig + 1] - S.bm_off[contig]);
  if (nw == 0) return false;
  const uint64_t* w = S.bm + S.bm_off[contig];
  const int64_t b0 = unclipped - S.bm_base[contig];
  int64_t wi = b0 >> 6;
  const uint32_t sh = (uint32_t)(b0 & 63);
  uint64_t lo = (wi >= 0 && wi < nw) ? w[wi] : 0ull;
  for (int o = 0; o < lq; o += 64) {
    ++wi;
    const uint64_t hi = (wi >= 0 && wi < nw) ? w[wi] : 0ull;
    uint64_t m = sh ? (lo >> sh) | (hi << (64 - sh)) : lo;
    lo = hi;
    if (lq - o < 64) m &= (1ull << (lq - o)) - 1ull;
    if (!m) continue;
    const uint64_t s = rs + (uint64_t)o;
    const uint32_t sb = (uint32_t)(s & 31);
    const uint64_t lo64 = m << sb, hi64 = sb ? m >> (64 - sb) : 0ull;
    const uint32_t p0 = (uint32_t)lo64, p1 = (uint32_t)(lo64 >> 32), p2 = (uint32_t)hi64;
    unsigned long long* sw = (unsigned long long*)&P.sbits[s >> 5];
    if (p0) atomicOr(sw, (unsigned long long)p0);
    if (p1) atomicOr(sw + 1, (unsigned long long)p1);
    if (p2) atomicOr(sw + 2, (unsigned long long)p2);
  }
  return true;
}

constexpr int kFastCigOps = 5;
struct PrepRec {
  ReadMeta m;
  ReadAlign a;
  uint64_t nslot;
};
struct PrepCols {
  uint4 c4, md4;
  uint32_t c5;
};
constexpr int kAccWords = 5;
__device__ __forceinline__ void acc_range(uint64_t acc[kAccWords], uint32_t lo, uint32_t hi, int half) {
#pragma unroll
  for (int j = 0; j < kAccWords; ++j) {
    const uint32_t a = max(lo, 32u * j), b = min(hi, 32u * j + 32u);
    const uint32_t n = b > a ? b - a : 0u;
    const uint32_t m = n >= 32u ? 0xFFFFFFFFu : (((1u << n) - 1u) << (a - 32u * j));
    acc[j] |= n ? (uint64_t)m << half : 0ull;
  }
}
__device__ __forceinline__ void acc_bit(uint64_t acc[kAccWords], uint32_t b, int half) {
#pragma unroll
  for (int j = 0; j < kAccWords; ++j) acc[j] |= (b >> 5) == (uint32_t)j ? 1ull << ((b & 31) + half) : 0ull;
}
__device__ __forceinline__ bool sites_bitmap_acc(const SitesDev& S, int32_t contig, int64_t unclipped, int lq,
                                                 uint32_t r0, uint64_t acc[kAccWords]) {
  const int64_t nw = (int64_t)(S.bm_off[contig + 1] - S.bm_off[contig]);
  if (nw == 0) return false;
  const uint64_t* w = S.bm + S.bm_off[contig];
  const int64_t b0 = unclipped - S.bm_base[contig];
  int64_t wi = b0 >> 6;
  const uint32_t sh = (uint32_t)(b0 & 63);
  uint64_t lo = (wi >= 0 && wi < nw) ? w[wi] : 0ull;
#pragma unroll
  for (int step = 0; step < 2; ++step) {
    const int o = 64 * step;
    if (o >= lq) break;
    ++wi;
    const uint64_t hi = (wi >= 0 && wi < nw) ? w[wi] : 0ull;
    uint64_t m = sh ? (lo >> sh) | (hi << (64 - sh)) : lo;
    lo = hi;
    if (lq - o < 64) m &= (1ull << (lq - o)) - 1ull;
    const uint64_t lo64 = m << r0, hi64 = r0 ? m >> (64 - r0) : 0ull;
    acc[2 * step] |= (uint64_t)(uint32_t)lo64;
    acc[2 * step + 1] |= (uint64_t)(uint32_t)(lo64 >> 32);
    if (2 * step + 2 < kAccWords) acc[2 * step + 2] |= (uint64_t)(uint32_t)hi64;
  }
  if (lq > 128) {
    ++wi;
    const uint64_t hi = (wi >= 0 && wi < nw) ? w[wi] : 0ull;
    uint64_t m = sh ? (lo >> sh) | (hi << (64 - sh)) : lo;
    m &= (1ull << (lq - 128)) - 1ull;
    const uint64_t lo64 = m << r0;
    acc[4] |= (uint64_t)(uint32_t)lo64;
  }
  return true;
}

__device__ __forceinline__ PrepRec prep_rec(const PrepParams& P, int64_t r) {
  PrepRec x{};
  if (r < P.rd.n_reads) {
    x.m = P.rd.meta[r];
    x.a = P.rd.align[r];
  }
  if (P.store_words && (threadIdx.x & 63) == 63)
    x.nslot = r + 1 < P.rd.n_reads ? P.rd.meta[r + 1].slot : (uint64_t)P.rd.n_slots;
  return x;
}
__device__ __forceinline__ PrepCols prep_cols(const ReadsDev& rd, const ReadMeta& m, const ReadAlign& a) {
  PrepCols c{make_uint4(0, 0, 0, 0), make_uint4(0, 0, 0, 0), 0u};
  const uint16_t f = m.flags;
  if (eligible_read(f) && a.n_cigar > 0 && a.n_cigar <= kFastCigOps) {
    c.c4 = *(const uint4*)(rd.cigar + a.cigar_off);
    if (a.n_cigar > 4) c.c5 = rd.cigar[a.cigar_off + 4];
    if (usable_read(f) && a.md_len > 0 && a.md_len <= 16) c.md4 = *(const uint4*)(rd.md + a.md_off);
  }
  return c;
}
__device__ __forceinline__ PrepCols prep_cols(const PrepParams& P, const PrepRec& x) { return prep_cols(P.rd, x.m, x.a); }


struct FastCig {
  int32_t lead, m1, x, m2;
  bool del;
  int32_t span;
  int32_t o_end;
  int64_t unclipped;
};
__device__ __forceinline__ bool fast_cigar(const uint32_t cw[kFastCigOps], int nc, const ReadMeta& m, int64_t start,
                                           FastCig& c) {
  int i = 0;
  int64_t trail = 0;
  c.lead = c.m1 = c.x = c.m2 = 0;
  c.del = false;
  bool ok = nc >= 1 && nc <= kFastCigOps;
  auto op = [&](int k) { return cig_op(k == 0 ? cw[0] : k == 1 ? cw[1] : k == 2 ? cw[2] : k == 3 ? cw[3] : cw[4]); };
  auto len = [&](int k) {
    return (int64_t)cig_len(k == 0 ? cw[0] : k == 1 ? cw[1] : k == 2 ? cw[2] : k == 3 ? cw[3] : cw[4]);
  };
  int64_t lead = 0, m1 = 0, x = 0, m2 = 0;
  if (ok && op(0) == BQSR_CIGAR_S) {
    lead = len(0);
    i = 1;
  }
  ok &= i < nc && op(i) == BQSR_CIGAR_M;
  if (ok) m1 = len(i++);
  if (ok && i < nc && (op(i) == BQSR_CIGAR_I || op(i) == BQSR_CIGAR_D)) {
    c.del = op(i) == BQSR_CIGAR_D;
    x = len(i++);
    ok &= x > 0 && i < nc && op(i) == BQSR_CIGAR_M;
    if (ok) m2 = len(i++);
    ok &= m2 > 0;
  }
  if (ok && i < nc && op(i) == BQSR_CIGAR_S) {
    trail = len(i++);
    ok &= trail > 0;
  }
  ok &= i == nc && m1 > 0 && (lead > 0 || op(0) != BQSR_CIGAR_S);
  if (!ok) return false;
  const int64_t rp_len = lead + m1 + (c.del ? 0 : x) + m2 + trail;
  const int64_t ref_len = m1 + (c.del ? x : 0) + m2;
  if (rp_len < m.lq || m.ls < m.lq) return false;
  const int64_t unclipped = start - lead;
  if (unclipped < 0 || unclipped + rp_len + ref_len > 2147483647LL || rp_len > 65535 || ref_len > 65535) return false;
  c.lead = (int32_t)lead;
  c.m1 = (int32_t)m1;
  c.x = (int32_t)x;
  c.m2 = (int32_t)m2;
  c.span = (int32_t)ref_len;
  c.o_end = (int32_t)(lead + m1 + (c.del ? 0 : x) + m2);
  c.unclipped = unclipped;
  return true;
}
__device__ __forceinline__ int32_t fc_offset(const FastCig& c, int32_t rel) {
  if (rel < c.m1) return c.lead + rel;
  if (c.del) return rel < c.m1 + c.x ? -1 : c.lead + rel - c.x;
  return c.lead + rel + c.x;
}

struct FastMd {
  bool ok, listed;
  uint64_t lst;
  int64_t md_total;
};
template <int kN>
__device__ __forceinline__ FastMd fast_md_n(const uint32_t (&w)[kN / 4], int n, const FastCig& cg, int st, int en) {
  uint32_t num = 0, pos = 0;
  bool over = false;
  int prev = 0;
  FastMd r{n > 0, en < 256, 0ull, 0};
  uint32_t lsh = 0;
#pragma unroll
  for (int i = 0; i < kN; ++i) {
    const uint32_t c = __builtin_amdgcn_ubfe(w[i >> 2], 8 * (i & 3), 8);
    if (i < n) {
      const uint32_t d = c - '0';
      if (d < 10u) {
        r.ok &= prev != 3;
        over |= num > 214748364u;
        num = num * 10u + d;
        over |= num > 0x7FFFFFFFu;
        prev = 1;
      } else {
        if (prev == 1) {
          r.ok &= !over;
          pos = min(pos + num, 0x7FFFFFFFu);
          num = 0;
          over = false;
        }
        if (c == '^') {
          r.ok &= prev == 1;
          prev = 3;
        } else {
          r.ok &= md_base((uint8_t)c) && prev != 0;
          if (pos < (uint32_t)cg.span) {
            const int32_t o = fc_offset(cg, (int32_t)pos);
            if (o >= st && o < en) {
              r.listed &= lsh < 64;
              r.lst |= lsh < 64 ? (uint64_t)(o + 1) << lsh : 0ull;
              lsh += 8;
            }
          }
          pos = min(pos + 1u, 0x7FFFFFFFu);
          prev = 2;
        }
      }
    }
  }
  r.ok &= prev == 1 && !over;
  r.md_total = (int64_t)min(pos + num, 0x7FFFFFFFu);
  return r;
}
__device__ __forceinline__ FastMd fast_md(const uint4 md4, int n, const FastCig& cg, int st, int en) {
  const uint32_t w[4] = {md4.x, md4.y, md4.z, md4.w};
  return fast_md_n<16>(w, n, cg, st, en);
}

template <class Emit>
__device__ __forceinline__ void fast_emit(const FastCig& c, const FastMd& md, int st, int en, Emit&& emit) {
  if (c.lead > st) emit(st, min(c.lead, en), 0);
  if (!c.del && c.x > 0) {
    const int lo = max(st, c.lead + c.m1), hi = min(en, c.lead + c.m1 + c.x);
    if (lo < hi) emit(lo, hi, 0);
  }
  if (c.o_end < en) emit(max(st, c.o_end), en, 0);
  for (uint64_t l = md.lst; l; l >>= 8) {
    const int o = (int)(l & 0xFFu) - 1;
    emit(o, o + 1, 32);
  }
  if (md.md_total < c.span) {
    const int32_t t = (int32_t)md.md_total;
    if (t < c.m1) {
      const int lo = max(st, c.lead + t), hi = min(en, c.lead + c.m1);
      if (lo < hi) emit(lo, hi, 32);
    }
    const int32_t r2 = max(t, c.m1 + (c.del ? c.x : 0));
    if (c.x > 0 && r2 < c.span) {
      const int lo = max(st, fc_offset(c, r2)), hi = min(en, c.o_end);
      if (lo < hi) emit(lo, hi, 32);
    }
  }
}

__device__ __forceinline__ void acc_or64(uint64_t acc[kAccWords], uint64_t m, uint32_t b) {
  const uint32_t wi = b >> 5, sh = b & 31;
  const uint64_t lo64 = m << sh;
  const uint32_t w0 = (uint32_t)lo64, w1 = (uint32_t)(lo64 >> 32), w2 = sh ? (uint32_t)(m >> (64 - sh)) : 0u;
#pragma unroll
  for (int j = 0; j < kAccWords; ++j)
    acc[j] |= (uint64_t)(((uint32_t)j == wi ? w0 : 0u) | ((uint32_t)j == wi + 1 ? w1 : 0u) |
                         ((uint32_t)j == wi + 2 ? w2 : 0u));
}
__device__ __forceinline__ void sites_seg_acc(const SitesDev& S, int32_t contig, int64_t u, int o_lo, int o_hi,
                                              uint32_t r0, uint64_t acc[kAccWords]) {
  const int64_t nw = (int64_t)(S.bm_off[contig + 1] - S.bm_off[contig]);
  const uint64_t* w = S.bm + S.bm_off[contig];
  for (int o = o_lo; o < o_hi; o += 64) {
    const int64_t b0 = u + o - S.bm_base[contig];
    const int64_t wi = b0 >> 6;
    const uint32_t sh = (uint32_t)(b0 & 63);
    const uint64_t lo = (wi >= 0 && wi < nw) ? w[wi] : 0ull, hi = (wi + 1 >= 0 && wi + 1 < nw) ? w[wi + 1] : 0ull;
    uint64_t m = sh ? (lo >> sh) | (hi << (64 - sh)) : lo;
    if (o_hi - o < 64) m &= (1ull << (o_hi - o)) - 1ull;
    if (m) acc_or64(acc, m, r0 + (uint32_t)o);
  }
}

__device__ __forceinline__ void fast_bits(const SitesDev& S, int32_t contig, const FastCig& c, const FastMd& md,
                                          int st, int en, uint32_t r0, uint64_t acc[kAccWords], bool* linear) {
  fast_emit(c, md, st, en, [&](int lo, int hi, int half) { acc_range(acc, r0 + (uint32_t)lo, r0 + (uint32_t)hi, half); });
  *linear = false;
  if (contig < 0 || contig >= S.n_contigs) return;
  if (S.bm_off[contig + 1] == S.bm_off[contig]) {
    *linear = true;
  } else if (c.x == 0) {
    sites_bitmap_acc(S, contig, c.unclipped, en, r0, acc);
  } else {
    sites_seg_acc(S, contig, c.unclipped, 0, min(en, c.lead + c.m1), r0, acc);
    const int ob = c.lead + c.m1 + (c.del ? 0 : c.x);
    sites_seg_acc(S, contig, c.unclipped + (c.del ? c.x : -c.x), ob, en, r0, acc);
  }
}

__device__ __forceinline__ uint16_t valid_flags(uint16_t f) {
  return (uint16_t)(kInfoApp | (usable_read(f) ? kInfoObs : 0) | ((f & BQSR_F_NEG_STRAND) ? kInfoNeg : 0) |
                    (((f & BQSR_F_PAIRED) && (f & BQSR_F_SECOND_OF_PAIR)) ? kInfoSecond : 0));
}
constexpr uint16_t kFastNeed = BQSR_F_HAS_QUAL | BQSR_F_HAS_RG | BQSR_F_HAS_SEQ | BQSR_F_HAS_CIGAR | BQSR_F_HAS_START |
                               BQSR_F_HAS_REFNAME;

template <bool kStore, bool kLong = false>
__device__ __forceinline__ bool prep_fast(const PrepParams& P, int64_t r, const PrepRec& x, const PrepCols& cols,
                          uint64_t acc_out[kAccWords], uint4 md4b = make_uint4(0, 0, 0, 0)) {
  const ReadMeta m = x.m;
  const ReadAlign a = x.a;
  const uint16_t f = m.flags;
  if (!eligible_read(f)) {
    P.info[r] = ReadInfo{0, 0, kInfoPass, 0};
    return true;
  }
  if ((f & kFastNeed) != kFastNeed || ((f & BQSR_F_NEG_STRAND) && (f & kSeqOther)) || m.lq == 0 || a.n_cigar == 0 ||
      a.n_cigar > kFastCigOps)
    return false;
  const bool usable = usable_read(f);
  if (usable && (a.md_len == 0 || a.md_len > (kLong ? 32 : 16))) return false;
  int st = 0, en = m.lq;
  if (kLong) {
    trim_quals(P.rd.qual + m.slot, m.lq, st, en);
    if (st >= en) return false;
  }
  const uint32_t cw[kFastCigOps] = {cols.c4.x, cols.c4.y, cols.c4.z, cols.c4.w, cols.c5};
  FastCig c;
  if (!fast_cigar(cw, a.n_cigar, m, a.start, c)) return false;
  const uint64_t rs = m.slot;
  bool nobits = false;
  if (usable) {
    FastMd md;
    if (kLong) {
      const uint32_t w[8] = {cols.md4.x, cols.md4.y, cols.md4.z, cols.md4.w, md4b.x, md4b.y, md4b.z, md4b.w};
      md = fast_md_n<32>(w, a.md_len, c, st, en);
    } else {
      md = fast_md(cols.md4, a.md_len, c, st, en);
    }
    if (!md.ok) return false;
    if (kStore && (int64_t)(rs & 31) + en > 32 * kAccWords) return false;
    if ((kStore || P.sites.n_contigs > 0) && (int64_t)(rs & 31) + en <= 32 * kAccWords) {
      if (!md.listed) return false;
      uint64_t acc[kAccWords] = {0, 0, 0, 0, 0};
      const uint32_t r0 = (uint32_t)(rs & 31);
      bool linear;
      fast_bits(P.sites, a.contig, c, md, st, en, r0, acc, &linear);
      if (kStore) {
        if (linear) return false;
#pragma unroll
        for (int j = 0; j < kAccWords; ++j) acc_out[j] = acc[j];
      } else {
        if (linear && c.x > 0) return false;
        nobits = !linear && !(acc[0] | acc[1] | acc[2] | acc[3] | acc[4]);
        const uint64_t wb = rs >> 5;
#pragma unroll
        for (int j = 0; j < kAccWords; ++j) {
          if (!acc[j]) continue;
          const uint64_t wi = wb + (uint64_t)j;
          atomicOr((unsigned long long*)&P.sbits[wi], (unsigned long long)acc[j]);
        }
        if (linear) mask_sites_linear(P, a.contig, c.unclipped, st, en, rs);
      }
    } else {
      if (a.contig >= 0 && a.contig < P.sites.n_contigs && c.x > 0) return false;
      nobits = c.lead <= st && (c.del || c.x == 0) && c.o_end >= en && md.listed && md.lst == 0 &&
               md.md_total >= c.span && !(a.contig >= 0 && a.contig < P.sites.n_contigs);
      if (!md.listed) {
        if (kLong || c.x > 0) return false;
        const uint32_t w[4] = {cols.md4.x, cols.md4.y, cols.md4.z, cols.md4.w};
        int64_t num = 0, pos = 0;
#pragma unroll
        for (int i = 0; i < 16; ++i) {
          const uint32_t ch = (w[i >> 2] >> (8 * (i & 3))) & 0xFFu;
          if (i < a.md_len) {
            if (ch >= '0' && ch <= '9') {
              num = num * 10 + (int64_t)(ch - '0');
            } else if (ch != '^') {
              pos += num;
              num = 0;
              const int64_t o = c.lead + pos;
              if (pos < c.m1 && o >= st && o < en) set_sbits(P.sbits, rs + (uint64_t)o, rs + (uint64_t)o + 1, 32);
              pos += 1;
            }
          }
        }
      }
      FastMd me = md;
      if (!md.listed) me.lst = 0;
      fast_emit(c, me, st, en,
                [&](int lo, int hi, int half) { set_sbits(P.sbits, rs + (uint64_t)lo, rs + (uint64_t)hi, half); });
      if (a.contig >= 0 && a.contig < P.sites.n_contigs && !mask_sites_bitmap(P, a.contig, c.unclipped, en, rs))
        mask_sites_linear(P, a.contig, c.unclipped, st, en, rs);
    }
  }
  const uint16_t nb = nobits ? kInfoNoBits : 0;
  P.info[r] = kLong ? ReadInfo{(uint16_t)st, (uint16_t)en, (uint16_t)(valid_flags(f) | nb), 0}
                    : ReadInfo{0, 0, (uint16_t)(kInfoTrim | valid_flags(f) | nb), 0};
  return true;
}

__device__ __forceinline__ bool prep_long(const PrepParams& P, int64_t r) {
  PrepRec x{};
  x.m = P.rd.meta[r];
  x.a = P.rd.align[r];
  const uint16_t f = x.m.flags;
  if (!eligible_read(f) || x.a.n_cigar == 0 || x.a.n_cigar > kFastCigOps || x.a.md_len > 32) return false;
  PrepCols c{*(const uint4*)(P.rd.cigar + x.a.cigar_off), make_uint4(0, 0, 0, 0), P.rd.cigar[x.a.cigar_off + 4]};
  uint4 md4b = make_uint4(0, 0, 0, 0);
  if (usable_read(f) && x.a.md_len > 0) {
    c.md4 = *(const uint4*)(P.rd.md + x.a.md_off);
    md4b = *(const uint4*)(P.rd.md + x.a.md_off + 16);
  }
  uint64_t acc[kAccWords] = {0, 0, 0, 0, 0};
  return prep_fast<false, true>(P, r, x, c, acc, md4b);
}

__device__ __forceinline__ uint64_t shfl_down_u64(uint64_t v, int d) {
  const uint32_t lo = (uint32_t)__shfl_down((int)(uint32_t)v, d), hi = (uint32_t)__shfl_down((int)(uint32_t)(v >> 32), d);
  return ((uint64_t)hi << 32) | lo;
}
__device__ __forceinline__ void prep_store_words(const PrepParams& P, int64_t r, const PrepRec& x,
                                                 const uint64_t acc[kAccWords]) {
  const int lane = threadIdx.x & 63;
  const int64_t n = P.rd.n_reads;
  const uint64_t slot = r < n ? x.m.slot : (uint64_t)P.rd.n_slots;
  uint64_t nslot = shfl_down_u64(slot, 1);
  if (lane == 63) nslot = r < n ? x.nslot : (uint64_t)P.rd.n_slots;
  const uint64_t fw = slot >> 5;
  const bool mid = (slot & 31) != 0 && r != 0;
  const uint64_t own_lo = mid ? fw + 1 : fw, own_hi = (nslot + 31) >> 5;
  uint64_t S = mid ? acc[0] : 0ull;
  const uint32_t key = (uint32_t)fw;
#pragma unroll
  for (int d = 1; d < 64; d <<= 1) {
    const uint64_t So = shfl_down_u64(S, d);
    const uint32_t ko = (uint32_t)__shfl_down((int)key, d);
    if (lane + d < 64 && ko == key) S |= So;
  }
  const uint64_t Sn = shfl_down_u64(S, 1);
  const uint32_t kn = (uint32_t)__shfl_down((int)key, 1);
  const uint64_t extra = (lane < 63 && own_hi > own_lo && kn == (uint32_t)(own_hi - 1)) ? Sn : 0ull;
  for (uint64_t w = own_lo; w < own_hi; ++w) {
    const uint64_t j = w - fw;
    uint64_t v = 0;
#pragma unroll
    for (int k = 0; k < kAccWords; ++k) v = j == (uint64_t)k ? acc[k] : v;
    P.sbits[w] = v | (w + 1 == own_hi ? extra : 0ull);
  }
  if (lane == 0) {
    const int64_t g = r >> 6;
    P.bnd[2 * g] = mid ? S : 0ull;
    P.bnd[2 * g + 1] = fw;
  }
}

template <bool kStore>
__global__ void __launch_bounds__(kPrepThreads, kStore ? 1 : 5) bqsr_prep_kernel(PrepParams P) {
  __shared__ uint32_t list[kPrepChunk];
  __shared__ uint32_t cnt;
  __shared__ uint32_t s_cig[kStore ? 1 : kPrepThreads * kPrepCigStride];
  __shared__ uint32_t s_md[kStore ? 1 : kPrepThreads * kPrepMdStride];
  __shared__ uint64_t s_rng[2];
  const int64_t n = P.rd.n_reads;
  const int64_t c0 = (int64_t)blockIdx.x * kPrepChunk;
  if (threadIdx.x == 0) {
    cnt = 0;
    if (!kStore) {
      s_rng[0] = c0 < n ? P.rd.meta[c0].slot : P.rd.n_slots;
      s_rng[1] = c0 + kPrepChunk < n ? P.rd.meta[c0 + kPrepChunk].slot : P.rd.n_slots;
    }
  }
  __syncthreads();
  const int lane = threadIdx.x & 63;
  const int64_t rt = c0 + threadIdx.x;
  PrepRec x0 = prep_rec(P, rt), x1 = prep_rec(P, rt + kPrepThreads);
  PrepCols k0 = prep_cols(P, x0);
  if (!kStore) {
    const uint64_t sa = s_rng[0], sb = s_rng[1];
    const uint64_t wa = (sa + 31) >> 5, wb = sb >> 5;
    for (uint64_t w = wa + threadIdx.x; w < wb; w += kPrepThreads) P.sbits[w] = 0ull;
    if (threadIdx.x < 2 && sa < sb) {
      const uint64_t w = threadIdx.x == 0 ? sa >> 5 : (sb - 1) >> 5;
      const uint64_t lo = max(sa, w << 5) - (w << 5), hi = min(sb, (w << 5) + 32) - (w << 5);
      const bool part = lo > 0 || hi < 32;
      const bool mine = threadIdx.x == 0 || (sb - 1) >> 5 != sa >> 5;
      if (part && mine) {
        const uint64_t m = (uint64_t)((hi >= 32 ? 0xFFFFFFFFu : ((1u << hi) - 1u)) & ~((1u << lo) - 1u));
        atomicAnd((unsigned long long*)&P.sbits[w], (unsigned long long)~(m | (m << 32)));
      }
    }
    __syncthreads();
  }
  for (int i = 0; i < kPrepChunk; i += kPrepThreads) {
    const int64_t r = rt + i;
    const PrepRec x2 = i + 2 * kPrepThreads < kPrepChunk ? prep_rec(P, r + 2 * kPrepThreads) : PrepRec{};
    const PrepCols k1 = i + kPrepThreads < kPrepChunk ? prep_cols(P, x1) : PrepCols{};
    uint64_t acc[kAccWords] = {0, 0, 0, 0, 0};
    const bool todo = r < n && !prep_fast<kStore>(P, r, x0, k0, acc);
    if (kStore) {
      if (todo) {
#pragma unroll
        for (int k = 0; k < kAccWords; ++k) acc[k] = 0;
      }
      prep_store_words(P, r, x0, acc);
    }
    x0 = x1;
    x1 = x2;
    k0 = k1;
    const uint64_t mask = __builtin_amdgcn_ballot_w64(todo);
    if (mask) {
      uint32_t base = 0;
      if (lane == (int)__builtin_ctzll(mask)) base = atomicAdd(&cnt, (uint32_t)__popcll(mask));
      base = __shfl(base, (int)__builtin_ctzll(mask));
      if (todo) list[base + (uint32_t)__popcll(mask & ((1ull << lane) - 1ull))] = (uint32_t)r;
    }
  }
  __syncthreads();
  const uint32_t k = cnt;
  if (!kStore) {
    for (uint32_t i = threadIdx.x; i < k; i += kPrepThreads)
      if (!prep_long(P, (int64_t)list[i]))
        prep_one(P, (int64_t)list[i], &s_cig[threadIdx.x * kPrepCigStride], &s_md[threadIdx.x * kPrepMdStride]);
    return;
  }
  for (uint32_t i = threadIdx.x; i < k; i += kPrepThreads) P.work[c0 + i] = list[i];
  if (threadIdx.x == 0) P.n_work[blockIdx.x] = k;
}

extern "C" __global__ void __launch_bounds__(kComplexThreads) bqsr_prep_complex(PrepParams P) {
  __shared__ uint32_t s_cig[kComplexThreads * kPrepCigStride];
  __shared__ uint32_t s_md[kComplexThreads * kPrepMdStride];
  const uint32_t k = P.n_work[blockIdx.x];
  const int64_t c0 = (int64_t)blockIdx.x * kPrepChunk;
  if (P.store_words && threadIdx.x < kPrepChunk / 64) {
    const int64_t g = (c0 >> 6) + threadIdx.x;
    if (g * 64 < P.rd.n_reads && P.bnd[2 * g])
      atomicOr((unsigned long long*)&P.sbits[P.bnd[2 * g + 1]], (unsigned long long)P.bnd[2 * g]);
  }
  for (uint32_t i = threadIdx.x; i < k; i += kComplexThreads)
    if (!prep_long(P, (int64_t)P.work[c0 + i]))
      prep_one(P, (int64_t)P.work[c0 + i], &s_cig[threadIdx.x * kPrepCigStride], &s_md[threadIdx.x * kPrepMdStride]);
}


constexpr int kChunk = 16;

__device__ __forceinline__ uint32_t wave_sum(uint32_t v) {
  for (int off = 32; off > 0; off >>= 1) v += __shfl_xor(v, off);
  return v;
}



__device__ __forceinline__ void load_window_head(const uint8_t* bases, int64_t n0, int64_t n_slots, uint64_t& lo,
                                              uint32_t& hi) {
  lo = 0;
  hi = 0;
  for (int k = 0; k <= 16; ++k) {
    const int64_t n = n0 + k;
    if (n < 0 || n >= n_slots) continue;
    const uint64_t c = (bases[n >> 1] >> ((n & 1) * 4)) & 0xFu;
    if (k < 16) lo |= c << (4 * k); else hi = (uint32_t)c;
  }
}

struct LaneRead {
  int64_t r;
  int64_t ro;
  uint64_t slot;
  uint64_t oslot;
  int st, en;
  int fl;
  bool trimmed;
  ReadInfo inf;
  int rg;
  int lq, ls;
  int cell0, dir;
  int aux;
};

__device__ __forceinline__ LaneRead lane_decode(int64_t r, const ReadMeta& m, const ReadInfo& inf, uint64_t qs, int L) {
  LaneRead x;
  x.r = r;
  x.ro = r;
  x.aux = 0;
  x.trimmed = false;
  x.inf = inf;
  x.slot = qs;
  x.oslot = m.slot;
  x.fl = inf.fl;
  x.rg = m.rg;
  x.lq = m.lq;
  x.ls = m.ls;
  const bool pass = inf.fl & kInfoPass;
  x.st = pass ? 0 : inf.st;
  x.en = pass ? ((m.flags & BQSR_F_HAS_QUAL) ? m.lq : 0) : inf.en;
  const bool neg = inf.fl & kInfoNeg, sec = inf.fl & kInfoSecond;
  if (!neg) {
    x.cell0 = sec ? L - 1 : L + 1;
    x.dir = sec ? -1 : 1;
  } else {
    x.cell0 = sec ? L - (int)m.ls : L + (int)m.ls;
    x.dir = sec ? 1 : -1;
  }
  return x;
}

__device__ __forceinline__ LaneRead lane_read(const ReadsDev& rd, const ReadInfo* info, int64_t r, bool live, int L,
                                              uint64_t ks = ~0ull) {
  ReadMeta m{0, 0, 0, 0, 0};
  ReadInfo inf{0, 0, 0, 0};
  if (live) {
    m = rd.meta[r];
    inf = info_load(info + r);
  }
  const bool trimmed = inf.fl & kInfoTrim;
  const uint64_t qs = ks == ~0ull ? m.slot : ks;
  inf = resolve_info(rd, inf, qs, m.lq);
  LaneRead x = lane_decode(live ? r : rd.n_reads, m, inf, qs, L);
  x.trimmed = trimmed;
  return x;
}

__device__ __forceinline__ int64_t wg_begin(const ReadsDev& rd, int64_t w, int G) {
  return min(rd.n_tiles * w / G * (int64_t)rd.reads_per_tile, rd.n_reads);
}
__device__ __forceinline__ int64_t wg_of(const ReadsDev& rd, int64_t p, int G) {
  const int64_t t = p / rd.reads_per_tile;
  return min((int64_t)G - 1, ((t + 1) * G - 1) / rd.n_tiles);
}
__device__ __forceinline__ int order_keys(const OrderDev& o) { return o.perm ? o.n_keys : 1; }
__device__ __forceinline__ int64_t key_begin(const OrderDev& o, int64_t n, int g) {
  return o.perm ? o.key_off[g] : (g == 0 ? 0 : n);
}
__device__ __forceinline__ int key_at(const OrderDev& o, int64_t p) {
  if (!o.perm) return 0;
  int lo = 0, hi = o.n_keys - 1;
  while (lo < hi) {
    const int mid = (lo + hi + 1) >> 1;
    if (o.key_off[mid] <= p) lo = mid; else hi = mid - 1;
  }
  return lo;
}
__device__ __forceinline__ int64_t pass_begin(const ReadsDev& rd, const OrderDev& o, int64_t w, int G) {
  return o.n_base ? o.key_off[min((int64_t)o.n_keys, w)] : wg_begin(rd, w, G);
}
__device__ __forceinline__ int64_t order_read(const OrderDev& o, int64_t i) { return o.perm ? (int64_t)o.perm[i] : i; }
__device__ __forceinline__ int key_rg(const OrderDev& o, int key, int rg_lo) {
  return o.perm ? (o.n_base ? key % o.n_base : key) >> 1 : rg_lo;
}
__device__ __forceinline__ int base_key(const OrderDev& o, int key) { return o.n_base ? key % o.n_base : key; }
__device__ __forceinline__ int order_base_keys(const OrderDev& o) { return o.perm ? (o.n_base ? o.n_base : o.n_keys) : 1; }
struct WinGeom {
  int c_lo, cw;
};
__device__ __forceinline__ WinGeom win_geom(const OrderDev& o, const TableGeom& g, int key) {
  if (!o.perm) return WinGeom{0, g.C};
  return (key & 1) ? WinGeom{0, g.L} : WinGeom{g.L + 1, g.L};
}


__device__ __forceinline__ int64_t chunk_n0(const LaneRead& x, int o0) {
  const bool neg = x.fl & kInfoNeg;
  return (int64_t)x.slot + (neg ? (int64_t)(x.en + x.st - o0 - 16) : (int64_t)(o0 - 1));
}
__device__ __forceinline__ uint4 chunk_raw(const ReadsDev& rd, int64_t n0) {
  return n0 >= 0 ? *(const uint4*)(rd.bases + (n0 >> 1)) : make_uint4(0, 0, 0, 0);
}
constexpr int kSub = 4;
constexpr int kSuper = kSub * kChunk;

template <int NW>
__device__ __forceinline__ void sub_bits(const uint64_t* w, uint32_t b0, int i, uint32_t& masked, uint32_t& mism) {
  const uint32_t b = b0 + 16u * (uint32_t)i;
  const uint32_t wi = b >> 5, sh = b & 31;
  uint64_t lo = w[0], hi = w[1];
#pragma unroll
  for (int k = 1; k < NW; ++k) {
    lo = wi == (uint32_t)k ? w[k] : lo;
    hi = wi == (uint32_t)k ? w[k + 1 < NW ? k + 1 : k] : hi;
  }
  masked = __builtin_amdgcn_alignbit((uint32_t)hi, (uint32_t)lo, sh);
  mism = __builtin_amdgcn_alignbit((uint32_t)(hi >> 32), (uint32_t)(lo >> 32), sh);
}

template <int NW>
__device__ __forceinline__ void sub_bits16(const uint64_t* w, uint32_t h, int i, uint32_t& masked, uint32_t& mism) {
  const int a = i >> 1, b = (i + 1) >> 1 < NW ? (i + 1) >> 1 : NW - 1;
  const uint64_t v = (i & 1) ? (h ? w[b] : w[a]) : w[a];
  const uint32_t sh = 16u * ((h + (uint32_t)i) & 1u);
  masked = (uint32_t)v >> sh;
  mism = (uint32_t)(v >> 32) >> sh;
}

__device__ __forceinline__ uint64_t window_first(uint64_t lo, int k) {
  const uint32_t sh = 4u * (uint32_t)k;
  return (lo & ~(0xFull << sh)) | ((uint64_t)kCodeN << sh);
}

__device__ __forceinline__ uint32_t ctx_slot(uint32_t a, uint32_t b) {
  if (a == kCodeN || b == kCodeN) return 4u;
  return 4u * (a < 4u ? a + 1u : 0u) + (b < 4u ? b + 1u : 0u);
}
__device__ __forceinline__ uint32_t comp_code(uint32_t c) { return c < 4u ? c ^ 3u : c; }
__device__ __forceinline__ void ctx_table_fill(uint16_t* t, int tid, int nthreads) {
  for (int i = tid; i < (int)(2 * kCtxTab); i += nthreads) {
    const uint32_t e = (uint32_t)i & (kCtxTab - 1u);
    const uint32_t c0 = e & 15u, c1 = (e >> 4) & 15u, c2 = e >> 8;
    t[i] = (uint16_t)((uint32_t)i < kCtxTab ? ctx_slot(c0, c1) | ctx_slot(c1, c2) << 8
                                  : ctx_slot(comp_code(c1), comp_code(c0)) |
                                        ctx_slot(comp_code(c2), comp_code(c1)) << 8);
  }
}
typedef unsigned short u16x2v __attribute__((ext_vector_type(2)));
typedef __attribute__((address_space(3))) const uint16_t* LdsHalves;
__device__ __forceinline__ uint32_t lshl1_add(uint32_t x, uint32_t tb) {
  uint32_t r;
  asm("v_lshl_add_u32 %0, %1, 1, %2" : "=v"(r) : "v"(x), "v"(tb));
  return r;
}
__device__ __forceinline__ void ctx_lookup(uint64_t lo, uint32_t hi, uint32_t tb, bool neg, uint32_t xo[4]) {
  const uint32_t d0 = (uint32_t)lo, d1 = (uint32_t)(lo >> 32);
  const uint32_t ix[8] = {__builtin_amdgcn_ubfe(d0, 0, 12),  __builtin_amdgcn_ubfe(d0, 8, 12),
                          __builtin_amdgcn_ubfe(d0, 16, 12), __builtin_amdgcn_alignbit(d1, d0, 24) & 0xFFFu,
                          __builtin_amdgcn_ubfe(d1, 0, 12),  __builtin_amdgcn_ubfe(d1, 8, 12),
                          __builtin_amdgcn_ubfe(d1, 16, 12), __builtin_amdgcn_alignbit(hi, d1, 24) & 0xFFFu};
  uint32_t X[4];
#pragma unroll
  for (int w = 0; w < 4; ++w) {
    u16x2v v;
    v.x = *(LdsHalves)(uintptr_t)lshl1_add(ix[2 * w], tb);
    v.y = *(LdsHalves)(uintptr_t)lshl1_add(ix[2 * w + 1], tb);
    X[w] = __builtin_bit_cast(uint32_t, v);
  }
  const uint32_t sel = neg ? 0x04050607u : 0x03020100u;
#pragma unroll
  for (int w = 0; w < 4; ++w) xo[w] = __builtin_amdgcn_perm(X[3 - w], X[w], sel);
}
__device__ __forceinline__ void lean_ctx(uint64_t lo, uint32_t hi, uint32_t u1lo, uint32_t u1hi, uint32_t u2lo,
                                         uint32_t u2hi, uint32_t h[4]) {
  uint32_t s[5];
#pragma unroll
  for (int d = 0; d < 2; ++d) {
    const uint32_t x = (uint32_t)(lo >> (32 * d));
    const uint32_t e = x & 0x07070707u, o = (x >> 4) & 0x07070707u;
    s[2 * d] = __builtin_amdgcn_perm(o, e, 0x05010400u);
    s[2 * d + 1] = __builtin_amdgcn_perm(o, e, 0x07030602u);
  }
  s[4] = hi & 7u;
#pragma unroll
  for (int w = 0; w < 4; ++w) {
    const uint32_t b = __builtin_amdgcn_alignbit(s[w + 1], s[w], 8);
    h[w] = __builtin_amdgcn_perm(u1hi, u1lo, s[w]) + __builtin_amdgcn_perm(u2hi, u2lo, b);
  }
}

constexpr uint32_t kA1lo = 0x100C0804u, kA1hi = 0x00000015u;
constexpr uint32_t kA2lo = 0x04030201u, kA2hi = 0x00000015u;
constexpr uint32_t kA1clo = 0x04080C10u, kA2clo = 0x01020304u;

__device__ __forceinline__ void chunk_ctx(const ReadsDev& rd, bool neg, int64_t n0, uint4 v, int j, uint32_t tb,
                                          uint32_t xo[4]) {
  uint64_t lo;
  uint32_t hi;
  if (__builtin_expect(n0 >= 0, 1)) {
    const uint32_t sh = (uint32_t)(n0 & 1) * 4u;
    lo = ((uint64_t)__builtin_amdgcn_alignbit(v.z, v.y, sh) << 32) | __builtin_amdgcn_alignbit(v.y, v.x, sh);
    hi = __builtin_amdgcn_alignbit(v.w, v.z, sh) & 0xFu;
  } else {
    load_window_head(rd.bases, n0, rd.n_slots, lo, hi);
  }
  if (j <= 0) {
    const int t = neg ? 16 + j : -j;
    if (t < 16) lo = window_first(lo, t); else hi = kCodeN;
  }
  ctx_lookup(lo, hi, neg ? tb + 2u * kCtxTab : tb, neg, xo);
}

__device__ __forceinline__ uint32_t mirror_bits16(uint32_t x, bool rev) {
  return rev ? (__builtin_bitreverse32(x & 0xFFFFu) >> 16) : (x & 0xFFFFu);
}
__device__ __forceinline__ void mirror16(uint32_t x[4], uint32_t sel) {
  const uint32_t y0 = __builtin_amdgcn_perm(x[3], x[0], sel), y1 = __builtin_amdgcn_perm(x[2], x[1], sel);
  const uint32_t y2 = __builtin_amdgcn_perm(x[1], x[2], sel), y3 = __builtin_amdgcn_perm(x[0], x[3], sel);
  x[0] = y0;
  x[1] = y1;
  x[2] = y2;
  x[3] = y3;
}


template <int kCtrl, int kRowMask = 0xF>
__device__ __forceinline__ uint32_t dpp_u32(uint32_t x) {
  return (uint32_t)__builtin_amdgcn_update_dpp(0, (int)x, kCtrl, kRowMask, 0xF, false);
}
__device__ __forceinline__ uint32_t wave_incl_add(uint32_t x) {
  x += dpp_u32<0x111>(x);
  x += dpp_u32<0x112>(x);
  x += dpp_u32<0x114>(x);
  x += dpp_u32<0x118>(x);
  x += dpp_u32<0x142, 0xA>(x);
  x += dpp_u32<0x143, 0xC>(x);
  return x;
}
__device__ __forceinline__ uint32_t wave_incl_max(uint32_t x) {
  x = max(x, dpp_u32<0x111>(x));
  x = max(x, dpp_u32<0x112>(x));
  x = max(x, dpp_u32<0x114>(x));
  x = max(x, dpp_u32<0x118>(x));
  x = max(x, dpp_u32<0x142, 0xA>(x));
  x = max(x, dpp_u32<0x143, 0xC>(x));
  return x;
}
__device__ __forceinline__ uint32_t bperm(int src_lane, uint32_t v) {
  return (uint32_t)__builtin_amdgcn_ds_bpermute(src_lane << 2, (int)v);
}

constexpr uint32_t kPkRev = 0x8000u;

template <uint32_t kAct, int kU, class LD, bool kAux, class FRead, class FLoad, class FChunk>
__device__ __forceinline__ void chunk_walk(const ReadsDev& rd, const ReadInfo* info, const OrderDev& ord, int64_t q0,
                                           int64_t q1, int64_t qstep, int L, int lane, uint32_t* mk, FRead&& fread,
                                           FLoad&& fload, FChunk&& fchunk) {
  for (int64_t wb = q0; wb < q1; wb += qstep) {
    const bool live = wb + lane < q1;
    LaneRead x = lane_read(rd, info, live ? order_read(ord, wb + lane) : 0, live, L,
                           live && ord.kslot ? ord.kslot[wb + lane] : ~0ull);
    fread(x, live);
    const int n = (live && (x.fl & kAct)) ? x.en - x.st : 0;
    const int jb = rd.slots_aligned ? -(x.st & 15) : 0;
    const uint32_t nch = n > 0 ? (uint32_t)((n - jb + 15) >> 4) : 0u;
    const uint32_t pe = wave_incl_add(nch), ps = pe - nch;
    const uint32_t total = __builtin_amdgcn_readlane(pe, 63);
    const uint32_t p_r = (uint32_t)x.r, p_slo = (uint32_t)x.slot, p_shi = (uint32_t)(x.slot >> 32);
    const uint32_t p_olo = (uint32_t)x.oslot, p_ohi = (uint32_t)(x.oslot >> 32);
    const uint32_t p_se = (uint32_t)x.st | ((uint32_t)x.en << 16);
    const uint32_t p_fl = (uint32_t)x.fl | (x.dir < 0 ? kPkRev : 0u) | ((uint32_t)x.cell0 << 16);
    const uint32_t p_rg = (uint32_t)x.rg, p_aux = (uint32_t)x.aux;
    for (uint32_t g00 = 0; g00 < total; g00 += 64 * kU) {
      LaneRead c[kU];
      int jj[kU];
      bool on[kU];
      LD ld[kU];
#pragma unroll
      for (int u = 0; u < kU; ++u) {
        const uint32_t g0 = g00 + 64 * u;
        mk[lane] = 0;
        __builtin_amdgcn_wave_barrier();
        if (nch && ps > g0 && ps < g0 + 64) atomicMax(&mk[ps - g0], (uint32_t)lane);
        __builtin_amdgcn_wave_barrier();
        const uint64_t below = __builtin_amdgcn_ballot_w64(nch && ps <= g0);
        uint32_t v = mk[lane];
        __builtin_amdgcn_wave_barrier();
        if (lane == 0) v = 63u - (uint32_t)__builtin_clzll(below);
        const int ri = (int)wave_incl_max(v);
        c[u].r = bperm(ri, p_r);
        c[u].slot = ((uint64_t)bperm(ri, p_shi) << 32) | bperm(ri, p_slo);
        c[u].ro = c[u].r;
        c[u].oslot = ord.kslot ? ((uint64_t)bperm(ri, p_ohi) << 32) | bperm(ri, p_olo) : c[u].slot;
        const uint32_t se = bperm(ri, p_se), fl = bperm(ri, p_fl);
        c[u].st = (int)(se & 0xFFFFu);
        c[u].en = (int)(se >> 16);
        c[u].fl = (int)(fl & 0x7FFFu);
        c[u].dir = (fl & kPkRev) ? -1 : 1;
        c[u].cell0 = (int)(fl >> 16);
        c[u].rg = (int)bperm(ri, p_rg);
        c[u].aux = kAux ? (int)bperm(ri, p_aux) : 0;
        const uint32_t ps_c = bperm(ri, ps);
        const int jb_c = rd.slots_aligned ? -(c[u].st & 15) : 0;
        jj[u] = jb_c + 16 * (int)(g0 + lane - ps_c);
        on[u] = g0 + lane < total;
        ld[u] = fload(c[u], jj[u], on[u]);
      }
#pragma unroll
      for (int u = 0; u < kU; ++u) fchunk(c[u], jj[u], c[u].en - c[u].st, on[u], ld[u]);
    }
  }
}


typedef __attribute__((address_space(3))) uint32_t* LdsWords;
typedef __attribute__((address_space(3))) const uint8_t* LdsBytes;
__device__ __forceinline__ void lds_add(uint32_t addr, uint32_t v) {
  __hip_atomic_fetch_add((LdsWords)(uintptr_t)addr, v, __ATOMIC_RELAXED, __HIP_MEMORY_SCOPE_WORKGROUP);
}


struct ObsChunkLoads {
  uint4 qs, cr;
  uint64_t bw0, bw1;
};

__device__ __forceinline__ ObsChunkLoads observe_load(const ObserveParams& P, const LaneRead& x, int j, bool on) {
  ObsChunkLoads v{make_uint4(0, 0, 0, 0), make_uint4(0, 0, 0, 0), 0, 0};
  if (!on) return v;
  const int o0 = x.st + j;
  v.qs = *(const uint4*)(P.rd.qual + x.slot + o0);
  if (x.fl & kInfoObs) {
    v.cr = chunk_raw(P.rd, chunk_n0(x, o0));
    const uint64_t s0 = x.oslot + (uint64_t)o0;
    if (!(x.fl & kInfoNoBits)) {
      v.bw0 = P.sbits[s0 >> 5];
      if ((s0 & 31) > 16) v.bw1 = P.sbits[(s0 >> 5) + 1];
    }
  }
  return v;
}

struct ObsPiece {
  uint32_t *w_obs, *w_mm, *w_masked, *blk_hist;
  int rg_w, c_lo, cw, q_lo, qw, wcells;
  bool ident;
  uint32_t tb;
};

__device__ __forceinline__ void observe_chunk(const ObserveParams& P, const ObsPiece& pc, const LaneRead& x, int j,
                                              int n, bool on, const ObsChunkLoads& ld) {
  if (!on) return;
  const bool full = x.fl & kInfoObs;
  const int o0 = x.st + j;
  const int C = P.g.C, cells = P.g.cells;
  const uint32_t qd[4] = {ld.qs.x, ld.qs.y, ld.qs.z, ld.qs.w};
  uint32_t bm = 0, bx = 0;
  uint32_t xo[4] = {4u, 4u, 4u, 4u};
  if (full) {
    const uint32_t sb = (uint32_t)((x.oslot + (uint64_t)o0) & 31);
    bm = __builtin_amdgcn_alignbit((uint32_t)ld.bw1, (uint32_t)ld.bw0, sb);
    bx = __builtin_amdgcn_alignbit((uint32_t)(ld.bw1 >> 32), (uint32_t)(ld.bw0 >> 32), sb);
    chunk_ctx(P.rd, x.fl & kInfoNeg, chunk_n0(x, o0), ld.cr, j, pc.tb, xo);
  }
  const int cc0 = x.cell0 + __mul24(x.dir, o0);
  const int wc0 = cc0 - pc.c_lo;
  const uint32_t nv = (uint32_t)min(kChunk, n - j);
  const int klo = j < 0 ? -j : 0;
  const bool cok = full && x.rg == pc.rg_w && (unsigned)(wc0 + __mul24(klo, x.dir)) < (unsigned)pc.cw &&
                   (unsigned)(wc0 + __mul24((int)nv - 1, x.dir)) < (unsigned)pc.cw;
  const uint32_t vmask = (nv >= 16u ? 0xFFFFu : ((1u << nv) - 1u)) & (0xFFFFu << klo);
  uint32_t fastm = 0;
  if (cok) {
#pragma unroll
    for (int k = 0; k < kChunk; ++k) {
      const int q = (int)__builtin_amdgcn_ubfe(qd[k >> 2], 8 * (k & 3), 8);
      const int row = q - pc.q_lo;
      const bool f = (unsigned)row < (unsigned)pc.qw && ((vmask >> k) & 1u);
      const bool m = (bm >> k) & 1u;
      const int base = __mul24(row, pc.wcells);
      if (f) {
        atomicAdd(m ? &pc.w_masked[row] : &pc.w_obs[base + wc0 + x.dir * k], 1u);
        if (!m) atomicAdd(&pc.w_obs[base + pc.cw + (int)__builtin_amdgcn_ubfe(xo[k >> 2], 8 * (k & 3), 8)], 1u);
      }
      fastm |= (uint32_t)f << k;
    }
  }
  uint32_t slow = vmask & ~fastm;
  uint32_t mmk = fastm & ~bm & bx;
  if (__builtin_amdgcn_ballot_w64(mmk != 0)) {
    const uint64_t x01 = ((uint64_t)xo[1] << 32) | xo[0], x23 = ((uint64_t)xo[3] << 32) | xo[2];
    while (mmk) {
      const int k = __builtin_ctz(mmk);
      mmk &= mmk - 1;
      const int q = (int)__builtin_amdgcn_ubfe(qd[k >> 2], 8 * (k & 3), 8);
      const int base = __mul24(q - pc.q_lo, pc.wcells);
      atomicAdd(&pc.w_mm[base + wc0 + __mul24(x.dir, k)], 1u);
      atomicAdd(&pc.w_mm[base + pc.cw + (int)(((k < 8 ? x01 : x23) >> (8 * (k & 7))) & 0xFFu)], 1u);
    }
  }
  if (__builtin_amdgcn_ballot_w64(slow != 0)) {
    const uint64_t x01 = ((uint64_t)xo[1] << 32) | xo[0], x23 = ((uint64_t)xo[3] << 32) | xo[2];
    while (slow) {
      const int k = __builtin_ctz(slow);
      slow &= slow - 1;
      const int o = o0 + k;
      const int q = (int)(int8_t)__builtin_amdgcn_ubfe(qd[k >> 2], 8 * (k & 3), 8);
      if (q < 0) {
        report(P.err, err_key((uint64_t)x.ro, (uint32_t)o, kRankTable, BQSR_ERR_QUAL_RANGE));
      } else if (full) {
        const bool masked = (bm >> k) & 1u, mism = (bx >> k) & 1u;
        const int ccell = cc0 + __mul24(x.dir, k);
        const int xcell = C + (int)(((k < 8 ? x01 : x23) >> (8 * (k & 7))) & 0xFFu);
        if (pc.ident) atomicAdd(&pc.blk_hist[q], 1u);
        const int64_t key = (int64_t)q + (int64_t)kMaxQ * x.rg;
        atomicAdd((unsigned long long*)&P.touched[key], 1ull);
        if (!masked) {
          atomicAdd((unsigned long long*)&P.obs[key * cells + ccell], 1ull);
          atomicAdd((unsigned long long*)&P.obs[key * cells + xcell], 1ull);
          if (mism) {
            atomicAdd((unsigned long long*)&P.mm[key * cells + ccell], 1ull);
            atomicAdd((unsigned long long*)&P.mm[key * cells + xcell], 1ull);
          }
        }
      }
    }
  }
}

constexpr int kObserveU = 2;

extern "C" __global__ void __launch_bounds__(kBlockThreads) bqsr_observe_chunks(ObserveParams P) {
  extern __shared__ __align__(16) unsigned char smem[];
  const int qw = P.w.qw, L = P.g.L;
  const int wcells = P.wcells;
  uint16_t* ctab = (uint16_t*)smem;
  uint32_t* w_obs = (uint32_t*)(smem + kCtxTabBytes);
  uint32_t* w_mm = w_obs + qw * wcells;
  uint32_t* w_masked = w_mm + qw * wcells;
  uint32_t* blk_hist = w_masked + qw;
  uint32_t* mk_all = blk_hist + kQBins;
  const int tid = threadIdx.x, lane = tid & 63;
  const int wave = __builtin_amdgcn_readfirstlane(tid >> 6);
  uint32_t* mk = mk_all + wave * 64;
  const int G = P.n_blocks;
  const bool ident = P.ord.perm == nullptr;
  for (int i = tid; i < kQBins; i += blockDim.x) blk_hist[i] = 0;
  ctx_table_fill(ctab, tid, blockDim.x);
  const int64_t wa = pass_begin(P.rd, P.ord, blockIdx.x, G), wb = pass_begin(P.rd, P.ord, blockIdx.x + 1, G);
  const int nk = order_keys(P.ord);
  for (int key = wa < wb ? key_at(P.ord, wa) : nk; key < nk; ++key) {
    const int64_t p0 = max(wa, key_begin(P.ord, P.rd.n_reads, key));
    const int64_t p1 = min(wb, key_begin(P.ord, P.rd.n_reads, key + 1));
    if (p0 >= wb) break;
    if (p0 >= p1) continue;
    const WinGeom gm = win_geom(P.ord, P.g, key);
    const ObsPiece pc{w_obs, w_mm, w_masked, blk_hist, key_rg(P.ord, key, P.w.rg_lo), gm.c_lo, gm.cw, P.w.q_lo, qw,
                      wcells, ident, (uint32_t)(uintptr_t)(LdsHalves)ctab};
    for (int i = tid; i < 2 * qw * wcells + qw; i += blockDim.x) w_obs[i] = 0;
    __syncthreads();
    const auto fread = [&](LaneRead& x, bool live) {
      if (live && x.trimmed) info_store(P.info + x.r, x.inf);
    };
    const auto fload = [&](const LaneRead& x, int j, bool on) { return observe_load(P, x, j, on); };
    const auto fchunk = [&](const LaneRead& x, int j, int n, bool on, const ObsChunkLoads& ld) {
      observe_chunk(P, pc, x, j, n, on, ld);
    };
    chunk_walk<kInfoObs | kInfoObsCheck, kObserveU, ObsChunkLoads, false>(P.rd, P.info, P.ord, p0 + 64 * wave, p1,
                                                                          64 * kWaves, L, lane, mk, fread, fload, fchunk);
    __syncthreads();
    uint32_t* pb = P.part + (int64_t)(blockIdx.x + (ident ? 0 : key)) * P.part_stride;
    for (int i = tid; i < 2 * qw * wcells; i += blockDim.x) pb[i] = w_obs[i];
    for (int slot = wave; slot < qw; slot += kWaves) {
      uint32_t v = 0;
      for (int c = lane; c < gm.cw; c += 64) v += w_obs[slot * wcells + c];
      v = wave_sum(v);
      if (lane == 0) {
        const uint32_t tot = v + w_masked[slot];
        pb[2 * qw * wcells + slot] = tot;
        if (ident && tot && P.w.q_lo + slot < kQBins) atomicAdd(&blk_hist[P.w.q_lo + slot], tot);
      }
    }
    __syncthreads();
  }
  if (ident)
    for (int k = tid; k < kQBins; k += blockDim.x) P.hq_block[(int64_t)blockIdx.x * kQBins + k] = blk_hist[k];
}

extern "C" __global__ void bqsr_window_reduce(const uint32_t* part, ReadsDev rd, OrderDev ord, int32_t n_blocks,
                                              int32_t stride, int32_t wcells, Window w, TableGeom g, int64_t* touched,
                                              int64_t* obs, int64_t* mm, int32_t junk) {
  const int nk = order_base_keys(ord);
  const int nc = w.qw * wcells;
  const int64_t total = (int64_t)nk * stride;
  for (int64_t t = blockIdx.x * (int64_t)blockDim.x + threadIdx.x; t < total; t += (int64_t)gridDim.x * blockDim.x) {
    const int key = (int)(t / stride);
    const int i = (int)(t - (int64_t)key * stride);
    uint64_t s = 0;
    if (ord.n_base) {
#pragma unroll 4
      for (int kf = key; kf < ord.n_keys; kf += ord.n_base) {
        const uint32_t v = part[2 * (int64_t)kf * stride + i];
        if (ord.key_off[kf] < ord.key_off[kf + 1]) s += v;
      }
    } else {
      const int64_t k0 = key_begin(ord, rd.n_reads, key), k1 = key_begin(ord, rd.n_reads, key + 1);
      if (k0 >= k1) continue;
      const int64_t wk1 = wg_of(rd, k1 - 1, n_blocks);
      for (int64_t w0 = wg_of(rd, k0, n_blocks) + (int64_t)blockIdx.y * kRedSlabs; w0 <= wk1;
           w0 += (int64_t)gridDim.y * kRedSlabs) {
        const int64_t w1 = min(wk1, w0 + kRedSlabs - 1);
#pragma unroll 8
        for (int64_t b = w0; b <= w1; ++b) {
// ... 736 lines not shown
```

adam_amd/csrc/bqsr_observe_lean.hip:

```cpp

namespace bqsr {

constexpr int kCtxJunk = 22;
constexpr int kCtxCells = kCtxSlots + kCtxJunk;
constexpr int kLeanSub = 8;

constexpr uint32_t kT1lo = 0x40302010u, kT1hi = 0x00000054u;
constexpr uint32_t kT2lo = 0x100C0804u, kT2hi = 0x00000054u;
constexpr uint32_t kT1clo = 0x10203040u, kT2clo = 0x04080C10u;
constexpr uint32_t kPermId = 0x03020100u, kPermRev = 0x04050607u;

__device__ __forceinline__ uint32_t byte_range(int w, int klo, int khi) {
  const int a = min(max(klo - 4 * w, 0), 4), b = min(max(khi - 4 * w, 0), 4);
  const uint32_t lo = a >= 4 ? 0u : (0xFFFFFFFFu << (8 * a));
  const uint32_t hi = b >= 4 ? 0xFFFFFFFFu : ((1u << (8 * b)) - 1u);
  return lo & hi;
}

typedef __attribute__((address_space(3))) uint32_t* LdsU32;

template <bool kPart>
__device__ __forceinline__ void lean_clean(const uint32_t q[4], const uint32_t xo[4], uint32_t a_cyc, uint32_t a_ctx,
                                           uint32_t o4, uint32_t bm, uint32_t bx, uint32_t a_mcyc, uint32_t a_mctx,
                                           uint32_t w4, uint32_t lmasked, int q_lo, uint32_t vp) {
#pragma unroll
  for (int p = 0; p < kChunk; ++p) {
    if (kPart && !((vp >> p) & 1u)) continue;
    const uint32_t qv = __builtin_amdgcn_ubfe(q[p >> 2], 8 * (p & 3), 8);
    const uint32_t xs4 = __builtin_amdgcn_ubfe(xo[p >> 2], 8 * (p & 3), 8);
    const uint32_t rq = __mul24(qv, o4);
    __hip_atomic_fetch_add((LdsU32)(uintptr_t)(rq + a_cyc) + p, 1u, __ATOMIC_RELAXED, __HIP_MEMORY_SCOPE_WORKGROUP);
    __hip_atomic_fetch_add((LdsU32)(uintptr_t)(rq + xs4 + a_ctx), 1u, __ATOMIC_RELAXED, __HIP_MEMORY_SCOPE_WORKGROUP);
  }
  uint32_t mk = bm | bx;
  if (__builtin_amdgcn_ballot_w64(mk != 0)) {
    const uint64_t x01 = ((uint64_t)xo[1] << 32) | xo[0], x23 = ((uint64_t)xo[3] << 32) | xo[2];
    const uint64_t q01 = ((uint64_t)q[1] << 32) | q[0], q23 = ((uint64_t)q[3] << 32) | q[2];
    while (mk) {
      const int p = __builtin_ctz(mk);
      mk &= mk - 1;
      const uint32_t qv = (uint32_t)((p < 8 ? q01 : q23) >> (8 * (p & 7))) & 0xFFu;
      const uint32_t xs4 = (uint32_t)((p < 8 ? x01 : x23) >> (8 * (p & 7))) & 0xFFu;
      const bool masked = (bm >> p) & 1u;
      const uint32_t rq = __mul24(qv, masked ? o4 : w4), val = masked ? ~0u : 1u;
      lds_add(rq + (masked ? a_cyc : a_mcyc) + 4u * (uint32_t)p, val);
      lds_add(rq + (masked ? a_ctx : a_mctx) + xs4, val);
      if (masked) lds_add(lmasked + 4u * (qv - (uint32_t)q_lo), 1u);
    }
  }
}

template <bool kIdent>
__global__ void __launch_bounds__(kBlockThreads) bqsr_observe_lean(ObserveParams P) {
  extern __shared__ __align__(16) unsigned char smem[];
  const int qw = P.w.qw, cells = P.g.cells, C = P.g.C, L = P.g.L;
  const int wcells = P.wcells, orow = P.orow, nc = P.nc;
  uint32_t* w_obs = (uint32_t*)smem;
  uint32_t* w_mm = w_obs + qw * orow;
  uint32_t* w_masked = w_mm + qw * wcells;
  uint32_t* blk_hist = w_masked + qw;
  const uint32_t lds_obs = (uint32_t)(uintptr_t)(LdsWords)w_obs, lds_masked = (uint32_t)(uintptr_t)(LdsWords)w_masked;
  const int tid = threadIdx.x, lane = tid & 63;
  const int wave = __builtin_amdgcn_readfirstlane(tid >> 6);
  const int G = P.n_blocks;
  const int q_lo = P.w.q_lo;
  const uint32_t w4 = 4u * (uint32_t)wcells, o4 = 4u * (uint32_t)orow;
  const uint32_t copy = (uint32_t)(lane % nc);
  const uint32_t qoff = (uint32_t)q_lo * o4;
  const uint32_t lds_mm = (uint32_t)(uintptr_t)(LdsWords)w_mm;
  const uint32_t lo4 = (uint32_t)q_lo * 0x01010101u, hi4 = (uint32_t)(q_lo + qw) * 0x01010101u;
  constexpr int kSup = kLeanSub * kChunk;
  constexpr int NW = (kSup + 31) / 32 + 1;
  constexpr bool ident = kIdent;
  const int nk = kIdent ? 1 : order_keys(P.ord);
  const int64_t wa = pass_begin(P.rd, P.ord, blockIdx.x, G), wb = pass_begin(P.rd, P.ord, blockIdx.x + 1, G);
  for (int i = tid; i < kQBins; i += blockDim.x) blk_hist[i] = 0;

  for (int key = kIdent ? 0 : (wa < wb ? key_at(P.ord, wa) : nk); key < nk; ++key) {
  const int64_t p0 = kIdent ? wa : max(wa, key_begin(P.ord, P.rd.n_reads, key));
  const int64_t p1 = kIdent ? wb : min(wb, key_begin(P.ord, P.rd.n_reads, key + 1));
  if (!kIdent && p0 >= wb) break;
  if (!kIdent && p0 >= p1) continue;
  const int rg_w = kIdent ? P.w.rg_lo : key_rg(P.ord, key, P.w.rg_lo);
  const WinGeom gm = kIdent ? WinGeom{0, C} : win_geom(P.ord, P.g, key);
  const int c_lo = gm.c_lo, cw = gm.cw;
  const uint32_t a_ctx = lds_obs + 4u * ((uint32_t)(nc * cw) + copy * kCtxCells) - qoff;
  const uint32_t a_mctx = lds_mm + 4u * (uint32_t)cw - (uint32_t)q_lo * w4;
  for (int i = tid; i < qw * (orow + wcells) + qw; i += blockDim.x) w_obs[i] = 0;
  __syncthreads();

  for (int64_t g0 = p0 + 64 * wave; g0 < p1; g0 += 64 * kWaves) {
    const bool live = g0 + lane < p1;
    LaneRead x;
    {
      const int64_t r = !live ? 0 : (kIdent ? g0 + lane : order_read(P.ord, g0 + lane));
      x = lane_read(P.rd, P.info, r, live, L);
      if (x.trimmed) info_store(P.info + x.r, x.inf);
    }
    const bool act = x.fl & (kInfoObs | kInfoObsCheck);
    const bool full = x.fl & kInfoObs;
    const int n = act ? x.en - x.st : 0;
    const bool clean_rd = full && x.rg == rg_w;
    const bool neg = x.fl & kInfoNeg, sec = x.fl & kInfoSecond;
    const bool rev = x.dir < 0;
    const uint32_t u1lo = neg ? kT2clo : kT1lo, u2lo = neg ? kT1clo : kT2lo;
    const uint32_t sel_q = rev ? kPermRev : kPermId, sel_x = sec ? kPermRev : kPermId;
    const int jb = P.rd.slots_aligned ? -(x.st & 15) : 0;
    const uint8_t* qp = P.rd.qual + x.slot;
    for (int j0 = jb; __builtin_amdgcn_ballot_w64(j0 < n); j0 += kSup) {
      if (j0 >= n) continue;
      uint4 qs[kLeanSub];
      uint3 cr[kLeanSub];
      uint64_t bw[NW];
      const uint64_t s0 = x.slot + (uint64_t)(x.st + j0);
#pragma unroll
      for (int i = 0; i < kLeanSub; ++i) {
        const bool lv = j0 + kChunk * i < n;
        const int o0 = x.st + j0 + kChunk * i;
        qs[i] = lv ? *(const uint4*)(qp + o0) : make_uint4(0, 0, 0, 0);
        const int64_t n0 = chunk_n0(x, o0);
        cr[i] = (lv && full && n0 >= 0) ? *(const uint3*)(P.rd.bases + ((n0 >> 3) << 2)) : make_uint3(0, 0, 0);
      }
#pragma unroll
      for (int w = 0; w < NW; ++w)
        bw[w] = !(full && !(x.fl & kInfoNoBits) && (w == 0 || 32 * w - 32 < n - j0)) ? 0ull : P.sbits[(s0 >> 5) + w];
#pragma clang loop unroll(full)
      for (int i = 0; i < kLeanSub; ++i) {
        const int j = j0 + kChunk * i;
        if (j >= n) continue;
        const int o0 = x.st + j;
        const int klo = j < 0 ? -j : 0, khi = min(kChunk, n - j);
        const uint32_t vmask = (0xFFFFu >> (kChunk - khi)) & (0xFFFFu << klo);
        uint32_t bm = 0, bx = 0;
        uint32_t h[4] = {0x10101010u, 0x10101010u, 0x10101010u, 0x10101010u};
        if (full) {
          if (P.rd.slots_aligned)
            sub_bits16<NW>(bw, (uint32_t)(s0 >> 4) & 1u, i, bm, bx);
          else
            sub_bits<NW>(bw, (uint32_t)(s0 & 31), i, bm, bx);
          const int64_t n0 = chunk_n0(x, o0);
          uint64_t clo;
          uint32_t chi;
          if (__builtin_expect(n0 >= 0, 1)) {
            const uint32_t sh = 4u * (uint32_t)(n0 & 7);
            clo = ((uint64_t)__builtin_amdgcn_alignbit(cr[i].z, cr[i].y, sh) << 32) |
                  __builtin_amdgcn_alignbit(cr[i].y, cr[i].x, sh);
            chi = (cr[i].z >> sh) & 0xFu;
          } else {
            load_window_head(P.rd.bases, n0, P.rd.n_slots, clo, chi);
          }
          lean_ctx(clo, chi, u1lo, kT1hi, u2lo, kT2hi, h);
        }
        bm &= vmask;
        bx &= vmask;
        uint32_t qd[4] = {qs[i].x, qs[i].y, qs[i].z, qs[i].w};
        mirror16(qd, sel_q);
        mirror16(h, sel_x);
        if (j <= 0) {
          const int pf = rev ? 15 + j : -j;
#pragma unroll
          for (int w = 0; w < 4; ++w) {
            const uint32_t m = (pf >> 2) == w ? 0xFFu << (8 * (pf & 3)) : 0u;
            h[w] = (h[w] & ~m) | (0x10101010u & m);
          }
        }
        const uint32_t bmp = mirror_bits16(bm, rev), bxp = mirror_bits16(bx, rev);
        const uint32_t vp = mirror_bits16(vmask, rev);
        const int plo = rev ? kChunk - khi : klo, phi = rev ? kChunk - klo : khi;
        const int cc0 = x.cell0 + __mul24(x.dir, o0);
        const int cb = (rev ? cc0 - (kChunk - 1) : cc0) - c_lo;
        const bool part = __builtin_amdgcn_ballot_w64(vp != 0xFFFFu) != 0;
        bool clean = clean_rd;
        if (!P.rows_all) {
          uint32_t bad = 0;
#pragma unroll
          for (int w = 0; w < 4; ++w) {
            uint32_t v = qd[w];
            if (part) {
              const uint32_t vb = byte_range(w, plo, phi);
              v = (v & vb) | (lo4 & ~vb);
            }
            const uint32_t t = v | 0x80808080u;
            bad |= v | ~(t - lo4) | (t - hi4);
          }
          clean = clean && (bad & 0x80808080u) == 0u;
        }
        const uint32_t a_cyc = lds_obs + 4u * (copy * (uint32_t)cw + (uint32_t)cb) - qoff;
        const uint32_t a_mcyc = lds_mm + 4u * (uint32_t)cb - (uint32_t)q_lo * w4;
        uint32_t fastm = 0;
        if (clean) {
          if (part)
            lean_clean<true>(qd, h, a_cyc, a_ctx, o4, bmp, bxp, a_mcyc, a_mctx, w4, lds_masked, q_lo, vp);
          else
            lean_clean<false>(qd, h, a_cyc, a_ctx, o4, bmp, bxp, a_mcyc, a_mctx, w4, lds_masked, q_lo, vp);
          fastm = vp;
        } else {
#pragma unroll
          for (int p = 0; p < kChunk; ++p) {
            const int q = (int)__builtin_amdgcn_ubfe(qd[p >> 2], 8 * (p & 3), 8);
            const int row = q - q_lo;
            const bool f = clean_rd && (unsigned)row < (unsigned)qw && ((vp >> p) & 1u);
            const bool m = (bmp >> p) & 1u;
            if (f) {
              const int ob = __mul24(row, orow);
              atomicAdd(m ? &w_masked[row] : &w_obs[ob + (int)copy * cw + cb + p], 1u);
              if (!m)
                atomicAdd(&w_obs[ob + nc * cw + (int)copy * kCtxCells +
                                 (int)(__builtin_amdgcn_ubfe(h[p >> 2], 8 * (p & 3), 8) >> 2)],
                          1u);
            }
            fastm |= (uint32_t)f << p;
          }
          uint32_t mmk = fastm & ~bmp & bxp;
          if (__builtin_amdgcn_ballot_w64(mmk != 0)) {
            const uint64_t x01 = ((uint64_t)h[1] << 32) | h[0], x23 = ((uint64_t)h[3] << 32) | h[2];
            const uint64_t q01 = ((uint64_t)qd[1] << 32) | qd[0], q23 = ((uint64_t)qd[3] << 32) | qd[2];
            while (mmk) {
              const int p = __builtin_ctz(mmk);
              mmk &= mmk - 1;
              const int q = (int)(((p < 8 ? q01 : q23) >> (8 * (p & 7))) & 0xFFu);
              const int xs = (int)((((p < 8 ? x01 : x23) >> (8 * (p & 7))) & 0xFFu) >> 2);
              const int base = __mul24(q - q_lo, wcells);
              atomicAdd(&w_mm[base + cb + p], 1u);
              atomicAdd(&w_mm[base + cw + xs], 1u);
            }
          }
        }
        uint32_t slow = vp & ~fastm;
        if (__builtin_amdgcn_ballot_w64(slow != 0)) {
          const uint64_t x01 = ((uint64_t)h[1] << 32) | h[0], x23 = ((uint64_t)h[3] << 32) | h[2];
          const uint64_t q01 = ((uint64_t)qd[1] << 32) | qd[0], q23 = ((uint64_t)qd[3] << 32) | qd[2];
          while (slow) {
            const int p = __builtin_ctz(slow);
            slow &= slow - 1;
            const int k = rev ? kChunk - 1 - p : p;
            const int o = o0 + k;
            const int q = (int)(int8_t)(((p < 8 ? q01 : q23) >> (8 * (p & 7))) & 0xFFu);
            if (q < 0) {
              report(P.err, err_key((uint64_t)x.r, (uint32_t)o, kRankTable, BQSR_ERR_QUAL_RANGE));
            } else if (full) {
              const bool masked = (bmp >> p) & 1u, mism = (bxp >> p) & 1u;
              const int ccell = cc0 + __mul24(x.dir, k);
              const int xs = (int)((((p < 8 ? x01 : x23) >> (8 * (p & 7))) & 0xFFu) >> 2);
              const int xcell = C + (xs < kCtxSlots ? xs : 4);
              if (ident) atomicAdd(&blk_hist[q], 1u);
              const int64_t key = (int64_t)q + (int64_t)kMaxQ * x.rg;
              atomicAdd((unsigned long long*)&P.touched[key], 1ull);
              if (!masked) {
                atomicAdd((unsigned long long*)&P.obs[key * cells + ccell], 1ull);
                atomicAdd((unsigned long long*)&P.obs[key * cells + xcell], 1ull);
                if (mism) {
                  atomicAdd((unsigned long long*)&P.mm[key * cells + ccell], 1ull);
                  atomicAdd((unsigned long long*)&P.mm[key * cells + xcell], 1ull);
                }
              }
            }
          }
        }
      }
    }
  }
  __syncthreads();
  uint32_t* pb = P.part + (int64_t)(blockIdx.x + (ident ? 0 : key)) * P.part_stride;
  const int nw = qw * wcells;
  for (int i = tid; i < nw; i += blockDim.x) {
    const int r = i / wcells, c = i - r * wcells;
    const uint32_t* ro = w_obs + r * orow;
    uint32_t v = 0;
    if (c < cw)
      for (int k = 0; k < nc; ++k) v += ro[k * cw + c];
    else if (c < cw + kCtxCells)
      for (int k = 0; k < nc; ++k) v += ro[nc * cw + k * kCtxCells + (c - cw)];
    pb[i] = v;
    pb[nw + i] = w_mm[i];
  }
  for (int slot = wave; slot < qw; slot += kWaves) {
    uint32_t v = 0;
    for (int c = lane; c < nc * cw; c += 64) v += w_obs[slot * orow + c];
    v = wave_sum(v);
    if (lane == 0) {
      const uint32_t tot = v + w_masked[slot];
      pb[2 * nw + slot] = tot;
      if (ident && tot && q_lo + slot < kQBins) atomicAdd(&blk_hist[q_lo + slot], tot);
    }
  }
  __syncthreads();
  }
  if (ident)
    for (int k = tid; k < kQBins; k += blockDim.x) P.hq_block[(int64_t)blockIdx.x * kQBins + k] = blk_hist[k];
}

template __global__ void bqsr_observe_lean<true>(ObserveParams);

}
```

Baseline: 503.3 billion bases/s.

## Store per-slot mask bits as 32-bit words per 16 aligned bases

When read slots are 16-aligned, the skip/mismatch bitmaps are laid out as one 32-bit word per 16 bases (mask in the low half, mismatch in the high half) instead of 64-bit words spanning 32 slots. Each read now clears and writes its own words with plain stores, which removes the boundary-word fixup buffer and the cross-read atomics. The observe kernels can then fetch a chunk's bits with aligned uint4 loads without shift or merge logic. The cost is a new template split for prep and observe kernels and extra code paths with their own correctness risk.

```diff
diff --git a/adam_amd/csrc/bqsr_capi.cpp b/adam_amd/csrc/bqsr_capi.cpp
--- a/adam_amd/csrc/bqsr_capi.cpp
+++ b/adam_amd/csrc/bqsr_capi.cpp
@@ -305,7 +305,6 @@
   ReadInfo* d_info = nullptr;
   uint64_t* d_sbits = nullptr;
   uint32_t* d_work = nullptr;
-  uint64_t* d_bnd = nullptr;
   int64_t sbits_words = 0;
   bool err_fresh = false;
   bool prepped = false;
@@ -478,7 +477,7 @@
   if (e == hipSuccess) e = hipMemcpy(c->d_qbt, buckets().thr.data(), kQbN * sizeof(double), hipMemcpyHostToDevice);
   if (e == hipSuccess) e = hipMemcpy(c->d_qbq, buckets().q.data(), kQbN * sizeof(int16_t), hipMemcpyHostToDevice);
   for (const void* f : {(const void*)bqsr_apply_kernel, (const void*)bqsr_observe_chunks,
-                        (const void*)bqsr_observe_lean<true>})
+                        (const void*)bqsr_observe_lean<true, false>, (const void*)bqsr_observe_lean<true, true>})
     if (e == hipSuccess) e = hipFuncSetAttribute(f, hipFuncAttributeMaxDynamicSharedMemorySize, (int)kLdsMax);
   if (e == hipSuccess)
     e = hipFuncSetAttribute((const void*)bqsr_fold_hist, hipFuncAttributeMaxDynamicSharedMemorySize, (int)fold_hist_lds());
@@ -627,10 +626,9 @@
   }
   if ((st = dalloc(b->allocs, &b->d_err, kErrWords)) != BQSR_OK) return st;
   if ((st = dalloc(b->allocs, &b->d_info, (size_t)std::max<int64_t>(1, n))) != BQSR_OK) return st;
-  b->sbits_words = (b->rd.n_slots / 32 + 5) & ~(int64_t)1;
+  b->sbits_words = b->rd.slots_aligned ? (b->rd.n_slots / 16 + 8 + 1) / 2 : b->rd.n_slots / 32 + 5;
   if ((st = dalloc(b->allocs, &b->d_sbits, (size_t)b->sbits_words)) != BQSR_OK) return st;
   if ((st = dalloc(b->allocs, &b->d_em, 2)) != BQSR_OK) return st;
-  if ((st = dalloc(b->allocs, &b->d_bnd, (size_t)2 * (size_t)(n / 64 + kPrepChunk / 64 + 1))) != BQSR_OK) return st;
   if ((st = dalloc(b->allocs, &b->d_work,
                    (size_t)(n + kPrepChunk) + (size_t)std::max<int64_t>(n / kPrepChunk + 1, kMaxFoldBlocks))) != BQSR_OK)
     return st;
@@ -1287,19 +1285,21 @@
     PrepParams P{};
     P.rd = b->rd;
     if (sites) P.sites = sites->dev();
-    P.store_words = b->dims.max_len <= 128 && P.sites.n_contigs > 0;
-    P.bnd = b->d_bnd;
+    const bool w32 = b->rd.slots_aligned;
+    const bool store = w32 && b->dims.max_len <= 128 && P.sites.n_contigs > 0;
     P.info = b->d_info;
     P.sbits = b->d_sbits;
     P.err = b->d_err;
     P.work = b->d_work;
     P.n_work = b->d_work + b->rd.n_reads + kPrepChunk;
     const int64_t blocks = (b->rd.n_reads + kPrepChunk - 1) / kPrepChunk;
-    if (P.store_words) {
-      hipLaunchKernelGGL(bqsr_prep_kernel<true>, dim3((unsigned)blocks), dim3(kPrepThreads), 0, s, P);
+    if (store) {
+      hipLaunchKernelGGL(bqsr_prep_kernel<kPrepStore>, dim3((unsigned)blocks), dim3(kPrepThreads), 0, s, P);
       hipLaunchKernelGGL(bqsr_prep_complex, dim3((unsigned)blocks), dim3(kComplexThreads), 0, s, P);
+    } else if (w32) {
+      hipLaunchKernelGGL(bqsr_prep_kernel<kPrepW32>, dim3((unsigned)blocks), dim3(kPrepThreads), 0, s, P);
     } else {
-      hipLaunchKernelGGL(bqsr_prep_kernel<false>, dim3((unsigned)blocks), dim3(kPrepThreads), 0, s, P);
+      hipLaunchKernelGGL(bqsr_prep_kernel<kPrepU64>, dim3((unsigned)blocks), dim3(kPrepThreads), 0, s, P);
     }
     HIP_TRY(hipGetLastError());
     if (b->bucketed && !b->perm_static) {
@@ -1390,7 +1390,10 @@
     P.n_blocks = lean ? b->n_blocks : b->pass_blocks();
     const size_t lds = lean ? lean_lds(P.w.qw, P.orow, P.wcells) : observe_lds(P.w.qw, P.wcells, true);
     if (lean) {
-      hipLaunchKernelGGL((bqsr_observe_lean<true>), dim3(P.n_blocks), dim3(kBlockThreads), lds, s, P);
+      if (P.rd.slots_aligned)
+        hipLaunchKernelGGL((bqsr_observe_lean<true, true>), dim3(P.n_blocks), dim3(kBlockThreads), lds, s, P);
+      else
+        hipLaunchKernelGGL((bqsr_observe_lean<true, false>), dim3(P.n_blocks), dim3(kBlockThreads), lds, s, P);
     } else {
       hipLaunchKernelGGL(bqsr_observe_chunks, dim3(P.n_blocks), dim3(kBlockThreads), lds, s, P);
     }
diff --git a/adam_amd/csrc/bqsr_internal.h b/adam_amd/csrc/bqsr_internal.h
--- a/adam_amd/csrc/bqsr_internal.h
+++ b/adam_amd/csrc/bqsr_internal.h
@@ -136,8 +136,6 @@
   SitesDev sites;
   ReadInfo* info;
   uint64_t* sbits;
-  int32_t store_words;
-  uint64_t* bnd;
   unsigned long long* err;
   uint32_t* work;
   uint32_t* n_work;
diff --git a/adam_amd/csrc/bqsr_kernels.hip b/adam_amd/csrc/bqsr_kernels.hip
--- a/adam_amd/csrc/bqsr_kernels.hip
+++ b/adam_amd/csrc/bqsr_kernels.hip
@@ -93,7 +93,18 @@
   return -1;
 }
 
+template <bool kW32>
 __device__ void set_sbits(uint64_t* sb, uint64_t lo, uint64_t hi, int half) {
+  if (kW32) {
+    uint32_t* sw = (uint32_t*)sb;
+    while (lo < hi) {
+      const int b = (int)(lo & 15);
+      const int n = (int)min((uint64_t)(16 - b), hi - lo);
+      atomicOr(&sw[lo >> 4], (((1u << n) - 1u) << b) << (half >> 1));
+      lo += (uint64_t)n;
+    }
+    return;
+  }
   while (lo < hi) {
     const uint64_t i = lo >> 5;
     const int b = (int)(lo & 31);
@@ -102,6 +113,12 @@
     atomicOr((unsigned long long*)&sb[i], (unsigned long long)m << half);
     lo += (uint64_t)n;
   }
+}
+__device__ __forceinline__ void own_words_order() { __builtin_amdgcn_fence(__ATOMIC_SEQ_CST, "workgroup"); }
+__device__ __forceinline__ void own_words_clear(uint64_t* sb, uint64_t rs, int lq) {
+  uint32_t* sw = (uint32_t*)sb + (rs >> 4);
+  for (int k = 0; 16 * k < lq; ++k) sw[k] = 0u;
+  own_words_order();
 }
 
 __device__ __forceinline__ int first_good(const uint4 v, int n, bool rev) {
@@ -164,10 +181,11 @@
 constexpr int kPrepMd = 32, kPrepMdStride = 9;
 constexpr int kPrepChunk = 2048;
 
-template <class CigPtr, class MdPtr>
+template <bool kW32, class CigPtr, class MdPtr>
 __device__ void prep_one_rest(const PrepParams& P, int64_t r, const ReadMeta& m, const ReadAlign& a, ReadInfo inf,
                               int st, int en, bool usable, CigPtr cig, MdPtr md);
 
+template <bool kW32>
 __device__ __forceinline__ void prep_one(const PrepParams& P, int64_t r, uint32_t* s_cig, uint32_t* s_md) {
   const ReadMeta m = P.rd.meta[r];
   const ReadAlign a = P.rd.align[r];
@@ -244,13 +262,13 @@
     lm[5] = m1.y;
     lm[6] = m1.z;
     lm[7] = m1.w;
-    prep_one_rest(P, r, m, a, inf, st, en, usable, (LdsCW)lc, (LdsCB)lm);
+    prep_one_rest<kW32>(P, r, m, a, inf, st, en, usable, (LdsCW)lc, (LdsCB)lm);
   } else {
-    prep_one_rest(P, r, m, a, inf, st, en, usable, gcig, gmd);
-  }
-}
-
-template <class CigPtr, class MdPtr>
+    prep_one_rest<kW32>(P, r, m, a, inf, st, en, usable, gcig, gmd);
+  }
+}
+
+template <bool kW32, class CigPtr, class MdPtr>
 __device__ void prep_one_rest(const PrepParams& P, int64_t r, const ReadMeta& m, const ReadAlign& a, ReadInfo inf,
                               int st, int en, bool usable, CigPtr cig, MdPtr md) {
   const uint16_t f = m.flags;
@@ -318,6 +336,7 @@
 
   uint64_t* bw = P.sbits;
   const uint64_t rs = m.slot;
+  if (kW32) own_words_clear(bw, rs, m.lq);
   {
     int ro = 0;
     int64_t pos = unclipped;
@@ -329,14 +348,14 @@
           int64_t w0 = (int64_t)ro + (start - pos), w1 = (int64_t)ro + (ref_end - pos);
           int a0 = (int)min(max(w0, (int64_t)lo), (int64_t)hi);
           int a1 = (int)min(max(w1, (int64_t)lo), (int64_t)hi);
-          set_sbits(bw, rs + (uint64_t)(lo), rs + (uint64_t)(a0), 0);
-          set_sbits(bw, rs + (uint64_t)(max(a1, a0)), rs + (uint64_t)(hi), 0);
+          set_sbits<kW32>(bw, rs + (uint64_t)(lo), rs + (uint64_t)(a0), 0);
+          set_sbits<kW32>(bw, rs + (uint64_t)(max(a1, a0)), rs + (uint64_t)(hi), 0);
         }
         ro += len;
         pos += len;
       } else if (op == BQSR_CIGAR_I) {
         int lo = max(ro, st), hi = min(ro + (int)len, en);
-        set_sbits(bw, rs + (uint64_t)(lo), rs + (uint64_t)(max(lo, hi)), 0);
+        set_sbits<kW32>(bw, rs + (uint64_t)(lo), rs + (uint64_t)(max(lo, hi)), 0);
         ro += len;
       } else if (op != BQSR_CIGAR_H) {
         pos += len;
@@ -348,7 +367,7 @@
     int64_t p = start + prel;
     if (p >= ref_end) return;
     int o = refpos_to_offset(cig, ncig, unclipped, p);
-    if (o >= st && o < en) set_sbits(bw, rs + (uint64_t)(o), rs + (uint64_t)(o + 1), 32);
+    if (o >= st && o < en) set_sbits<kW32>(bw, rs + (uint64_t)(o), rs + (uint64_t)(o + 1), 32);
   });
   if (start + md_total < ref_end) {
     int ro = 0;
@@ -360,7 +379,7 @@
         int64_t p0 = max(pos, t0), p1 = min(pos + (int64_t)len, ref_end);
         if (p0 < p1) {
           int lo = max(ro + (int)(p0 - pos), st), hi = min(ro + (int)(p1 - pos), en);
-          if (lo < hi) set_sbits(bw, rs + (uint64_t)(lo), rs + (uint64_t)(hi), 32);
+          if (lo < hi) set_sbits<kW32>(bw, rs + (uint64_t)(lo), rs + (uint64_t)(hi), 32);
         }
         ro += len;
         pos += len;
@@ -388,12 +407,13 @@
       while (j < ns && sp[j] < lo_p) ++j;
       for (; j < ns && sp[j] < hi_p; ++j) {
         int o = refpos_to_offset(cig, ncig, unclipped, sp[j]);
-        if (o >= st && o < en) set_sbits(bw, rs + (uint64_t)(o), rs + (uint64_t)(o + 1), 0);
-      }
-    }
-  }
-}
-
+        if (o >= st && o < en) set_sbits<kW32>(bw, rs + (uint64_t)(o), rs + (uint64_t)(o + 1), 0);
+      }
+    }
+  }
+}
+
+template <bool kW32>
 __device__ void mask_sites_linear(const PrepParams& P, int32_t contig, int64_t unclipped, int st, int en,
                                   uint64_t rs) {
   if (contig < 0 || contig >= P.sites.n_contigs) return;
@@ -409,10 +429,11 @@
   while (j < ns && sp[j] < lo_p) ++j;
   for (; j < ns && sp[j] < hi_p; ++j) {
     const uint64_t o = (uint64_t)(sp[j] - unclipped);
-    set_sbits(P.sbits, rs + o, rs + o + 1, 0);
-  }
-}
-
+    set_sbits<kW32>(P.sbits, rs + o, rs + o + 1, 0);
+  }
+}
+
+template <bool kW32>
 __device__ __forceinline__ bool mask_sites_bitmap(const PrepParams& P, int32_t contig, int64_t unclipped, int lq,
                                                   uint64_t rs) {
   const SitesDev& S = P.sites;
@@ -430,6 +451,15 @@
     lo = hi;
     if (lq - o < 64) m &= (1ull << (lq - o)) - 1ull;
     if (!m) continue;
+    if (kW32) {
+      uint32_t* sw = (uint32_t*)P.sbits + ((rs + (uint64_t)o) >> 4);
+#pragma unroll
+      for (int k = 0; k < 4; ++k) {
+        const uint32_t p = (uint32_t)(m >> (16 * k)) & 0xFFFFu;
+        if (p) atomicOr(sw + k, p);
+      }
+      continue;
+    }
     const uint64_t s = rs + (uint64_t)o;
     const uint32_t sb = (uint32_t)(s & 31);
     const uint64_t lo64 = m << sb, hi64 = sb ? m >> (64 - sb) : 0ull;
@@ -446,7 +476,6 @@
 struct PrepRec {
   ReadMeta m;
   ReadAlign a;
-  uint64_t nslot;
 };
 struct PrepCols {
   uint4 c4, md4;
@@ -466,6 +495,39 @@
 #pragma unroll
   for (int j = 0; j < kAccWords; ++j) acc[j] |= (b >> 5) == (uint32_t)j ? 1ull << ((b & 31) + half) : 0ull;
 }
+struct __attribute__((packed, aligned(4))) WordPair {
+  uint32_t a, b;
+};
+__device__ __forceinline__ void store_chunk_words(uint64_t* sb, uint64_t rs, int lq, const uint64_t acc[kAccWords]) {
+  uint32_t* sw = (uint32_t*)sb + (rs >> 4);
+#pragma unroll
+  for (int j = 0; j < kAccWords; ++j) {
+    const uint32_t lo = (uint32_t)acc[j], hi = (uint32_t)(acc[j] >> 32);
+    const uint32_t w0 = (lo & 0xFFFFu) | (hi << 16), w1 = (lo >> 16) | (hi & 0xFFFF0000u);
+    if (32 * j + 16 < lq)
+      *(WordPair*)(sw + 2 * j) = WordPair{w0, w1};
+    else if (32 * j < lq)
+      sw[2 * j] = w0;
+  }
+}
+
+__device__ __forceinline__ uint64_t bits_below(int n) { return n >= 64 ? ~0ull : n <= 0 ? 0ull : (1ull << n) - 1ull; }
+__device__ __forceinline__ uint64_t bits_range(int lo, int hi) { return bits_below(hi) & ~bits_below(lo); }
+template <int N>
+__device__ __forceinline__ void store_chunk_words_lean(uint64_t* sb, uint64_t rs, int lq, const uint64_t m[N],
+                                                       const uint64_t x[N]) {
+  uint32_t* sw = (uint32_t*)sb + (rs >> 4);
+#pragma unroll
+  for (int j = 0; j < 2 * N; ++j) {
+    const uint32_t lo = (uint32_t)(m[j >> 1] >> (32 * (j & 1))), hi = (uint32_t)(x[j >> 1] >> (32 * (j & 1)));
+    const uint32_t w0 = (lo & 0xFFFFu) | (hi << 16), w1 = (lo >> 16) | (hi & 0xFFFF0000u);
+    if (32 * j + 16 < lq)
+      *(WordPair*)(sw + 2 * j) = WordPair{w0, w1};
+    else if (32 * j < lq)
+      sw[2 * j] = w0;
+  }
+}
+
 __device__ __forceinline__ bool sites_bitmap_acc(const SitesDev& S, int32_t contig, int64_t unclipped, int lq,
                                                  uint32_t r0, uint64_t acc[kAccWords]) {
   const int64_t nw = (int64_t)(S.bm_off[contig + 1] - S.bm_off[contig]);
@@ -506,8 +568,6 @@
     x.m = P.rd.meta[r];
     x.a = P.rd.align[r];
   }
-  if (P.store_words && (threadIdx.x & 63) == 63)
-    x.nslot = r + 1 < P.rd.n_reads ? P.rd.meta[r + 1].slot : (uint64_t)P.rd.n_slots;
   return x;
 }
 __device__ __forceinline__ PrepCols prep_cols(const ReadsDev& rd, const ReadMeta& m, const ReadAlign& a) {
@@ -712,9 +772,38 @@
 constexpr uint16_t kFastNeed = BQSR_F_HAS_QUAL | BQSR_F_HAS_RG | BQSR_F_HAS_SEQ | BQSR_F_HAS_CIGAR | BQSR_F_HAS_START |
                                BQSR_F_HAS_REFNAME;
 
-template <bool kStore, bool kLong = false>
+template <int N>
+__device__ __forceinline__ void lean_words(uint64_t* sb, uint64_t rs, const FastCig& c, const FastMd& md, int st,
+                                           int en) {
+  uint64_t am[N], ax[N];
+#pragma unroll
+  for (int j = 0; j < N; ++j) am[j] = ax[j] = 0ull;
+  FastMd me = md;
+  me.lst = 0;
+  fast_emit(c, me, st, en, [&](int lo, int hi, int half) {
+#pragma unroll
+    for (int j = 0; j < N; ++j) {
+      const uint64_t b = bits_range(lo - 64 * j, hi - 64 * j);
+      if (half)
+        ax[j] |= b;
+      else
+        am[j] |= b;
+    }
+  });
+  for (uint64_t l = md.lst; l; l >>= 8) {
+    const uint32_t o = (uint32_t)(l & 0xFFu) - 1u;
+    const uint64_t b = 1ull << (o & 63u);
+#pragma unroll
+    for (int j = 0; j < N; ++j) ax[j] |= (o >> 6) == (uint32_t)j ? b : 0ull;
+  }
+  store_chunk_words_lean<N>(sb, rs, en, am, ax);
+}
+
+enum : int { kPrepU64 = 0, kPrepW32 = 1, kPrepStore = 2 };
+template <int kForm, bool kLong = false>
 __device__ __forceinline__ bool prep_fast(const PrepParams& P, int64_t r, const PrepRec& x, const PrepCols& cols,
-                          uint64_t acc_out[kAccWords], uint4 md4b = make_uint4(0, 0, 0, 0)) {
+                                          uint4 md4b = make_uint4(0, 0, 0, 0)) {
+  constexpr bool kW32 = kForm != kPrepU64;
   const ReadMeta m = x.m;
   const ReadAlign a = x.a;
   const uint16_t f = m.flags;
@@ -746,35 +835,64 @@
       md = fast_md(cols.md4, a.md_len, c, st, en);
     }
     if (!md.ok) return false;
-    if (kStore && (int64_t)(rs & 31) + en > 32 * kAccWords) return false;
-    if ((kStore || P.sites.n_contigs > 0) && (int64_t)(rs & 31) + en <= 32 * kAccWords) {
+    const bool site_contig = a.contig >= 0 && a.contig < P.sites.n_contigs;
+    const bool plain = c.lead <= st && (c.del || c.x == 0) && c.o_end >= en && md.listed && md.lst == 0 &&
+                       md.md_total >= c.span;
+    if (kForm == kPrepStore) {
+      if (en > 32 * kAccWords || !md.listed) return false;
+      uint64_t acc[kAccWords] = {0, 0, 0, 0, 0};
+      bool linear;
+      fast_bits(P.sites, a.contig, c, md, st, en, 0u, acc, &linear);
+      if (linear) return false;
+      store_chunk_words(P.sbits, rs, en, acc);
+    } else if (kW32 && P.sites.n_contigs == 0 && en < 256) {
+      nobits = plain;
+      if (!nobits) {
+        if (!md.listed) return false;
+        if (en <= 128)
+          lean_words<2>(P.sbits, rs, c, md, st, en);
+        else
+          lean_words<4>(P.sbits, rs, c, md, st, en);
+      }
+    } else if (kW32 && en <= 32 * kAccWords) {
+      nobits = P.sites.n_contigs == 0 && plain;
+      if (!nobits) {
+        if (!md.listed) return false;
+        uint64_t acc[kAccWords] = {0, 0, 0, 0, 0};
+        bool linear;
+        fast_bits(P.sites, a.contig, c, md, st, en, 0u, acc, &linear);
+        if (linear && c.x > 0) return false;
+        if (P.sites.n_contigs > 0) nobits = !linear && !(acc[0] | acc[1] | acc[2] | acc[3] | acc[4]);
+        if (!nobits) {
+          store_chunk_words(P.sbits, rs, en, acc);
+          if (linear) {
+            own_words_order();
+            mask_sites_linear<true>(P, a.contig, c.unclipped, st, en, rs);
+          }
+        }
+      }
+    } else if (!kW32 && P.sites.n_contigs > 0 && (int64_t)(rs & 31) + en <= 32 * kAccWords) {
       if (!md.listed) return false;
       uint64_t acc[kAccWords] = {0, 0, 0, 0, 0};
       const uint32_t r0 = (uint32_t)(rs & 31);
       bool linear;
       fast_bits(P.sites, a.contig, c, md, st, en, r0, acc, &linear);
-      if (kStore) {
-        if (linear) return false;
-#pragma unroll
-        for (int j = 0; j < kAccWords; ++j) acc_out[j] = acc[j];
-      } else {
-        if (linear && c.x > 0) return false;
-        nobits = !linear && !(acc[0] | acc[1] | acc[2] | acc[3] | acc[4]);
-        const uint64_t wb = rs >> 5;
-#pragma unroll
-        for (int j = 0; j < kAccWords; ++j) {
-          if (!acc[j]) continue;
-          const uint64_t wi = wb + (uint64_t)j;
-          atomicOr((unsigned long long*)&P.sbits[wi], (unsigned long long)acc[j]);
-        }
-        if (linear) mask_sites_linear(P, a.contig, c.unclipped, st, en, rs);
-      }
+      if (linear && c.x > 0) return false;
+      nobits = !linear && !(acc[0] | acc[1] | acc[2] | acc[3] | acc[4]);
+      const uint64_t wb = rs >> 5;
+#pragma unroll
+      for (int j = 0; j < kAccWords; ++j) {
+        if (!acc[j]) continue;
+        const uint64_t wi = wb + (uint64_t)j;
+        atomicOr((unsigned long long*)&P.sbits[wi], (unsigned long long)acc[j]);
+      }
+      if (linear) mask_sites_linear<false>(P, a.contig, c.unclipped, st, en, rs);
     } else {
-      if (a.contig >= 0 && a.contig < P.sites.n_contigs && c.x > 0) return false;
-      nobits = c.lead <= st && (c.del || c.x == 0) && c.o_end >= en && md.listed && md.lst == 0 &&
-               md.md_total >= c.span && !(a.contig >= 0 && a.contig < P.sites.n_contigs);
+      if (site_contig && c.x > 0) return false;
+      if (!md.listed && (kLong || c.x > 0)) return false;
+      nobits = plain && !site_contig;
+      if (kW32 && !nobits) own_words_clear(P.sbits, rs, en);
       if (!md.listed) {
-        if (kLong || c.x > 0) return false;
         const uint32_t w[4] = {cols.md4.x, cols.md4.y, cols.md4.z, cols.md4.w};
         int64_t num = 0, pos = 0;
 #pragma unroll
@@ -787,7 +905,7 @@
               pos += num;
               num = 0;
               const int64_t o = c.lead + pos;
-              if (pos < c.m1 && o >= st && o < en) set_sbits(P.sbits, rs + (uint64_t)o, rs + (uint64_t)o + 1, 32);
+              if (pos < c.m1 && o >= st && o < en) set_sbits<kW32>(P.sbits, rs + (uint64_t)o, rs + (uint64_t)o + 1, 32);
               pos += 1;
             }
           }
@@ -796,9 +914,9 @@
       FastMd me = md;
       if (!md.listed) me.lst = 0;
       fast_emit(c, me, st, en,
-                [&](int lo, int hi, int half) { set_sbits(P.sbits, rs + (uint64_t)lo, rs + (uint64_t)hi, half); });
-      if (a.contig >= 0 && a.contig < P.sites.n_contigs && !mask_sites_bitmap(P, a.contig, c.unclipped, en, rs))
-        mask_sites_linear(P, a.contig, c.unclipped, st, en, rs);
+                [&](int lo, int hi, int half) { set_sbits<kW32>(P.sbits, rs + (uint64_t)lo, rs + (uint64_t)hi, half); });
+      if (site_contig && !mask_sites_bitmap<kW32>(P, a.contig, c.unclipped, en, rs))
+        mask_sites_linear<kW32>(P, a.contig, c.unclipped, st, en, rs);
     }
   }
   const uint16_t nb = nobits ? kInfoNoBits : 0;
@@ -807,6 +925,7 @@
   return true;
 }
 
+template <bool kW32>
 __device__ __forceinline__ bool prep_long(const PrepParams& P, int64_t r) {
   PrepRec x{};
   x.m = P.rd.meta[r];
@@ -819,51 +938,12 @@
     c.md4 = *(const uint4*)(P.rd.md + x.a.md_off);
     md4b = *(const uint4*)(P.rd.md + x.a.md_off + 16);
   }
-  uint64_t acc[kAccWords] = {0, 0, 0, 0, 0};
-  return prep_fast<false, true>(P, r, x, c, acc, md4b);
-}
-
-__device__ __forceinline__ uint64_t shfl_down_u64(uint64_t v, int d) {
-  const uint32_t lo = (uint32_t)__shfl_down((int)(uint32_t)v, d), hi = (uint32_t)__shfl_down((int)(uint32_t)(v >> 32), d);
-  return ((uint64_t)hi << 32) | lo;
-}
-__device__ __forceinline__ void prep_store_words(const PrepParams& P, int64_t r, const PrepRec& x,
-                                                 const uint64_t acc[kAccWords]) {
-  const int lane = threadIdx.x & 63;
-  const int64_t n = P.rd.n_reads;
-  const uint64_t slot = r < n ? x.m.slot : (uint64_t)P.rd.n_slots;
-  uint64_t nslot = shfl_down_u64(slot, 1);
-  if (lane == 63) nslot = r < n ? x.nslot : (uint64_t)P.rd.n_slots;
-  const uint64_t fw = slot >> 5;
-  const bool mid = (slot & 31) != 0 && r != 0;
-  const uint64_t own_lo = mid ? fw + 1 : fw, own_hi = (nslot + 31) >> 5;
-  uint64_t S = mid ? acc[0] : 0ull;
-  const uint32_t key = (uint32_t)fw;
-#pragma unroll
-  for (int d = 1; d < 64; d <<= 1) {
-    const uint64_t So = shfl_down_u64(S, d);
-    const uint32_t ko = (uint32_t)__shfl_down((int)key, d);
-    if (lane + d < 64 && ko == key) S |= So;
-  }
-  const uint64_t Sn = shfl_down_u64(S, 1);
-  const uint32_t kn = (uint32_t)__shfl_down((int)key, 1);
-  const uint64_t extra = (lane < 63 && own_hi > own_lo && kn == (uint32_t)(own_hi - 1)) ? Sn : 0ull;
-  for (uint64_t w = own_lo; w < own_hi; ++w) {
-    const uint64_t j = w - fw;
-    uint64_t v = 0;
-#pragma unroll
-    for (int k = 0; k < kAccWords; ++k) v = j == (uint64_t)k ? acc[k] : v;
-    P.sbits[w] = v | (w + 1 == own_hi ? extra : 0ull);
-  }
-  if (lane == 0) {
-    const int64_t g = r >> 6;
-    P.bnd[2 * g] = mid ? S : 0ull;
-    P.bnd[2 * g + 1] = fw;
-  }
-}
-
-template <bool kStore>
-__global__ void __launch_bounds__(kPrepThreads, kStore ? 1 : 5) bqsr_prep_kernel(PrepParams P) {
+  return prep_fast<kW32 ? kPrepW32 : kPrepU64, true>(P, r, x, c, md4b);
+}
+
+template <int kForm>
+__global__ void __launch_bounds__(kPrepThreads, kForm == kPrepStore ? 1 : 5) bqsr_prep_kernel(PrepParams P) {
+  constexpr bool kStore = kForm == kPrepStore, kW32 = kForm != kPrepU64;
   __shared__ uint32_t list[kPrepChunk];
   __shared__ uint32_t cnt;
   __shared__ uint32_t s_cig[kStore ? 1 : kPrepThreads * kPrepCigStride];
@@ -873,7 +953,7 @@
   const int64_t c0 = (int64_t)blockIdx.x * kPrepChunk;
   if (threadIdx.x == 0) {
     cnt = 0;
-    if (!kStore) {
+    if (!kW32) {
       s_rng[0] = c0 < n ? P.rd.meta[c0].slot : P.rd.n_slots;
       s_rng[1] = c0 + kPrepChunk < n ? P.rd.meta[c0 + kPrepChunk].slot : P.rd.n_slots;
     }
@@ -883,7 +963,7 @@
   const int64_t rt = c0 + threadIdx.x;
   PrepRec x0 = prep_rec(P, rt), x1 = prep_rec(P, rt + kPrepThreads);
   PrepCols k0 = prep_cols(P, x0);
-  if (!kStore) {
+  if (!kW32) {
     const uint64_t sa = s_rng[0], sb = s_rng[1];
     const uint64_t wa = (sa + 31) >> 5, wb = sb >> 5;
     for (uint64_t w = wa + threadIdx.x; w < wb; w += kPrepThreads) P.sbits[w] = 0ull;
@@ -903,15 +983,7 @@
     const int64_t r = rt + i;
     const PrepRec x2 = i + 2 * kPrepThreads < kPrepChunk ? prep_rec(P, r + 2 * kPrepThreads) : PrepRec{};
     const PrepCols k1 = i + kPrepThreads < kPrepChunk ? prep_cols(P, x1) : PrepCols{};
-    uint64_t acc[kAccWords] = {0, 0, 0, 0, 0};
-    const bool todo = r < n && !prep_fast<kStore>(P, r, x0, k0, acc);
-    if (kStore) {
-      if (todo) {
-#pragma unroll
-        for (int k = 0; k < kAccWords; ++k) acc[k] = 0;
-      }
-      prep_store_words(P, r, x0, acc);
-    }
+    const bool todo = r < n && !prep_fast<kForm>(P, r, x0, k0);
     x0 = x1;
     x1 = x2;
     k0 = k1;
@@ -927,8 +999,8 @@
   const uint32_t k = cnt;
   if (!kStore) {
     for (uint32_t i = threadIdx.x; i < k; i += kPrepThreads)
-      if (!prep_long(P, (int64_t)list[i]))
-        prep_one(P, (int64_t)list[i], &s_cig[threadIdx.x * kPrepCigStride], &s_md[threadIdx.x * kPrepMdStride]);
+      if (!prep_long<kW32>(P, (int64_t)list[i]))
+        prep_one<kW32>(P, (int64_t)list[i], &s_cig[threadIdx.x * kPrepCigStride], &s_md[threadIdx.x * kPrepMdStride]);
     return;
   }
   for (uint32_t i = threadIdx.x; i < k; i += kPrepThreads) P.work[c0 + i] = list[i];
@@ -940,14 +1012,10 @@
   __shared__ uint32_t s_md[kComplexThreads * kPrepMdStride];
   const uint32_t k = P.n_work[blockIdx.x];
   const int64_t c0 = (int64_t)blockIdx.x * kPrepChunk;
-  if (P.store_words && threadIdx.x < kPrepChunk / 64) {
-    const int64_t g = (c0 >> 6) + threadIdx.x;
-    if (g * 64 < P.rd.n_reads && P.bnd[2 * g])
-      atomicOr((unsigned long long*)&P.sbits[P.bnd[2 * g + 1]], (unsigned long long)P.bnd[2 * g]);
-  }
   for (uint32_t i = threadIdx.x; i < k; i += kComplexThreads)
-    if (!prep_long(P, (int64_t)P.work[c0 + i]))
-      prep_one(P, (int64_t)P.work[c0 + i], &s_cig[threadIdx.x * kPrepCigStride], &s_md[threadIdx.x * kPrepMdStride]);
+    if (!prep_long<true>(P, (int64_t)P.work[c0 + i]))
+      prep_one<true>(P, (int64_t)P.work[c0 + i], &s_cig[threadIdx.x * kPrepCigStride],
+                     &s_md[threadIdx.x * kPrepMdStride]);
 }
 
 
@@ -1090,15 +1158,6 @@
   }
   masked = __builtin_amdgcn_alignbit((uint32_t)hi, (uint32_t)lo, sh);
   mism = __builtin_amdgcn_alignbit((uint32_t)(hi >> 32), (uint32_t)(lo >> 32), sh);
-}
-
-template <int NW>
-__device__ __forceinline__ void sub_bits16(const uint64_t* w, uint32_t h, int i, uint32_t& masked, uint32_t& mism) {
-  const int a = i >> 1, b = (i + 1) >> 1 < NW ? (i + 1) >> 1 : NW - 1;
-  const uint64_t v = (i & 1) ? (h ? w[b] : w[a]) : w[a];
-  const uint32_t sh = 16u * ((h + (uint32_t)i) & 1u);
-  masked = (uint32_t)v >> sh;
-  mism = (uint32_t)(v >> 32) >> sh;
 }
 
 __device__ __forceinline__ uint64_t window_first(uint64_t lo, int k) {
@@ -1308,8 +1367,13 @@
     v.cr = chunk_raw(P.rd, chunk_n0(x, o0));
     const uint64_t s0 = x.oslot + (uint64_t)o0;
     if (!(x.fl & kInfoNoBits)) {
-      v.bw0 = P.sbits[s0 >> 5];
-      if ((s0 & 31) > 16) v.bw1 = P.sbits[(s0 >> 5) + 1];
+      if (P.rd.slots_aligned) {
+        const uint32_t w = ((const uint32_t*)P.sbits)[s0 >> 4];
+        v.bw0 = (uint64_t)(w & 0xFFFFu) | ((uint64_t)(w >> 16) << 32);
+      } else {
+        v.bw0 = P.sbits[s0 >> 5];
+        if ((s0 & 31) > 16) v.bw1 = P.sbits[(s0 >> 5) + 1];
+      }
     }
   }
   return v;
@@ -1332,7 +1396,7 @@
   uint32_t bm = 0, bx = 0;
   uint32_t xo[4] = {4u, 4u, 4u, 4u};
   if (full) {
-    const uint32_t sb = (uint32_t)((x.oslot + (uint64_t)o0) & 31);
+    const uint32_t sb = P.rd.slots_aligned ? 0u : (uint32_t)((x.oslot + (uint64_t)o0) & 31);
     bm = __builtin_amdgcn_alignbit((uint32_t)ld.bw1, (uint32_t)ld.bw0, sb);
     bx = __builtin_amdgcn_alignbit((uint32_t)(ld.bw1 >> 32), (uint32_t)(ld.bw0 >> 32), sb);
     chunk_ctx(P.rd, x.fl & kInfoNeg, chunk_n0(x, o0), ld.cr, j, pc.tb, xo);
diff --git a/adam_amd/csrc/bqsr_observe_lean.hip b/adam_amd/csrc/bqsr_observe_lean.hip
--- a/adam_amd/csrc/bqsr_observe_lean.hip
+++ b/adam_amd/csrc/bqsr_observe_lean.hip
@@ -50,7 +50,7 @@
   }
 }
 
-template <bool kIdent>
+template <bool kIdent, bool kW32>
 __global__ void __launch_bounds__(kBlockThreads) bqsr_observe_lean(ObserveParams P) {
   extern __shared__ __align__(16) unsigned char smem[];
   const int qw = P.w.qw, cells = P.g.cells, C = P.g.C, L = P.g.L;
@@ -105,13 +105,14 @@
     const bool rev = x.dir < 0;
     const uint32_t u1lo = neg ? kT2clo : kT1lo, u2lo = neg ? kT1clo : kT2lo;
     const uint32_t sel_q = rev ? kPermRev : kPermId, sel_x = sec ? kPermRev : kPermId;
-    const int jb = P.rd.slots_aligned ? -(x.st & 15) : 0;
+    const int jb = kW32 ? -(x.st & 15) : 0;
     const uint8_t* qp = P.rd.qual + x.slot;
     for (int j0 = jb; __builtin_amdgcn_ballot_w64(j0 < n); j0 += kSup) {
       if (j0 >= n) continue;
       uint4 qs[kLeanSub];
       uint3 cr[kLeanSub];
-      uint64_t bw[NW];
+      uint64_t bw[kW32 ? 1 : NW];
+      uint4 cw0 = make_uint4(0, 0, 0, 0), cw1 = cw0;
       const uint64_t s0 = x.slot + (uint64_t)(x.st + j0);
 #pragma unroll
       for (int i = 0; i < kLeanSub; ++i) {
@@ -121,9 +122,17 @@
         const int64_t n0 = chunk_n0(x, o0);
         cr[i] = (lv && full && n0 >= 0) ? *(const uint3*)(P.rd.bases + ((n0 >> 3) << 2)) : make_uint3(0, 0, 0);
       }
-#pragma unroll
-      for (int w = 0; w < NW; ++w)
-        bw[w] = !(full && !(x.fl & kInfoNoBits) && (w == 0 || 32 * w - 32 < n - j0)) ? 0ull : P.sbits[(s0 >> 5) + w];
+      if constexpr (kW32) {
+        if (full && !(x.fl & kInfoNoBits)) {
+          const uint32_t* cwp = (const uint32_t*)P.sbits + (s0 >> 4);
+          cw0 = *(const uint4*)cwp;
+          if (4 * kChunk < n - j0) cw1 = *(const uint4*)(cwp + 4);
+        }
+      } else {
+#pragma unroll
+        for (int w = 0; w < NW; ++w)
+          bw[w] = !(full && !(x.fl & kInfoNoBits) && (w == 0 || 32 * w - 32 < n - j0)) ? 0ull : P.sbits[(s0 >> 5) + w];
+      }
 #pragma clang loop unroll(full)
       for (int i = 0; i < kLeanSub; ++i) {
         const int j = j0 + kChunk * i;
@@ -134,10 +143,13 @@
         uint32_t bm = 0, bx = 0;
         uint32_t h[4] = {0x10101010u, 0x10101010u, 0x10101010u, 0x10101010u};
         if (full) {
-          if (P.rd.slots_aligned)
-            sub_bits16<NW>(bw, (uint32_t)(s0 >> 4) & 1u, i, bm, bx);
-          else
+          if constexpr (kW32) {
+            const uint32_t cwv[kLeanSub] = {cw0.x, cw0.y, cw0.z, cw0.w, cw1.x, cw1.y, cw1.z, cw1.w};
+            bm = cwv[i] & 0xFFFFu;
+            bx = cwv[i] >> 16;
+          } else {
             sub_bits<NW>(bw, (uint32_t)(s0 & 31), i, bm, bx);
+          }
           const int64_t n0 = chunk_n0(x, o0);
           uint64_t clo;
           uint32_t chi;
@@ -290,6 +302,7 @@
     for (int k = tid; k < kQBins; k += blockDim.x) P.hq_block[(int64_t)blockIdx.x * kQBins + k] = blk_hist[k];
 }
 
-template __global__ void bqsr_observe_lean<true>(ObserveParams);
+template __global__ void bqsr_observe_lean<true, false>(ObserveParams);
+template __global__ void bqsr_observe_lean<true, true>(ObserveParams);
 
 }
```

After: 516.2 billion bases/s, median of 6. +2.6%, better.
